# Daniel-Lin-S/decode_tonal_langauge

Measured on AMD Instinct MI355X. Metric: mel-frames/sec (train step) SynthesisModelCNN, 128ch x 400t batch256, higher is better.
Workload: dtype f32; 1 GPU; SynthesisModelCNN 128ch x 400t -> 80 mel, 4 tones x 2 syllables, L=5, global batch 256 (strong scaling: 256 windows on rank 0), dropout 0.5, NAdam, 1,376,768,720 params; per_gpu_batch=256, global_batch=256, parallelism=dp1, init=drawn on every rank

## Files before the change

decode_tonal_langauge_amd/_conv_stack.py:

```python
from __future__ import annotations

from typing import List

import torch

from . import _kernels, _lib
from ._launch import LaunchTimers, launch_nt, launch_tn, permute_reduce, r4
from ._lib import (EPI_C1WGRAD, EPI_GY, EPI_LRELU, EPI_MASK, EPI_MASKY, EPI_POOL, EPI_POOLV, LOAD_DIRECT, LOAD_UNPOOL, LOAD_V,
                   LOAD_Y, check, ptr)


class _Stage:

    def __init__(self, idx, cin, cout, k, pool, tin, tp_in):
        self.idx, self.cin, self.cout, self.k, self.pool = idx, cin, cout, k, pool
        self.tin, self.tp_in = tin, tp_in
        self.tc = tin - k + 1
        self.tout = self.tc // 2 if pool else self.tc
        self.tp_out = tp_in // 2 if pool else tp_in


class ConvStack(LaunchTimers):
    F63_CAPABLE = True

# ... 150 lines not shown
    def _v_hex_buffer(self, store, idx, rows, cin):
        nh = rows // 6
        nh_pad = (nh + 24 + 127) // 128 * 128
        V = store.get(idx)
        if V is None or V.shape[0] != nh_pad or V.shape[1] != 8 or V.shape[2] != cin:
            V = store[idx] = torch.zeros(nh_pad, 8, cin, dtype=torch.float32, device=self._dev)
        return V

    def _halo_buffer(self, key, ntm, cout):
        halo = self._vhalo.get(key)
        if halo is None or halo.shape[0] != ntm or halo.shape[2] != cout:
            halo = self._vhalo[key] = torch.zeros(ntm, 2, cout, dtype=torch.float32, device=self._dev)
        return halo

    def _pack_wino63(self, w, forward: bool):
        O, I = w.shape[0], w.shape[1]
        dst = torch.empty(8, O, I, dtype=torch.float32, device=w.device) if forward else \
            torch.empty(8, I, O, dtype=torch.float32, device=w.device)
        check(self.lib.tl_wino63_weights(ptr(w), ptr(dst) if forward else None, None if forward else ptr(dst), O, I, I, O,
                                         self._stream()), "tl_wino63_weights")
        return dst

    def f63_issue_factor(self, st) -> float:
        return (st.tp_in // 6) * 8.0 / (st.tc * 3.0)

    def _stage_forward63(self, st, w, bia) -> None:
        S = self.S
        wp = self._pack_wino63(w, True)
        V = self._v_ready[st.idx - 1]
        if st.idx == 2 and self.store_p1 and 2 not in self.P:
            self.P[2] = torch.zeros(S * st.tp_out, st.cout, dtype=torch.float32, device=self._dev)
        Pout = self.P.get(st.idx) if (st.idx != 2 or self.store_p1) else None
        kw = dict(A=ptr(V), A_rows=V.shape[0], lda=V.shape[2], loader=LOAD_V, Bw=ptr(wp), bias=ptr(bia), out=ptr(Pout),
                  M=S * st.tp_in, N=st.cout, K=st.cin, ldb=st.cin, ldo=Pout.shape[1] if Pout is not None else st.cout, J=3,
                  row_shift=0, Tp=st.tp_in, slope=self.slope, obits=ptr(self.bits[st.idx]), osign=ptr(self.sbits[st.idx]),
                  ld_obits=st.cout // 32, Tvalid=2 * st.tout)
        if st.idx == 2:
            rows_out = S * st.tp_out
            Vn = self._v_hex_buffer(self.V, 2, rows_out, st.cout)
            ntm = -(-(S * st.tp_in) // self._nt63_rows())
            halo = self._halo_buffer(2, ntm, st.cout)
            kw.update(epilogue=EPI_POOLV, vout=ptr(Vn), vhalo=ptr(halo), vout_quads=Vn.shape[0], ld_vout=Vn.shape[2])
            self._nt(tag="conv2_fwd", fn="tl_conv3_wino63v_nt", **kw)
            check(self.lib.tl_wino63_v_fixup(ptr(Vn), ptr(halo), rows_out // 6, ntm, st.tp_out, st.cout, Vn.shape[2],
                                             self._stream()), "tl_wino63_v_fixup")
            self._v_ready[2] = Vn
        else:
            if Pout is None:
                raise RuntimeError("F(6,3) stage 3 writes pooled rows: its output buffer was not allocated")
            kw.update(epilogue=EPI_POOL, out_tp=st.tp_out)
            self._nt(tag="conv3_fwd", fn="tl_conv3_wino63v_nt", **kw)

    def _stage_wgrad63(self, st, gw, gb) -> None:
        S = self.S
        f32 = dict(dtype=torch.float32, device=self._dev)
        rows_in = S * st.tp_in
        nd = st.cout
        ldg = nd
        V = self._v_ready[st.idx - 1]
        tiles = (st.cin // 64) * (nd // 64)
        sk = self._splitk(tiles, (rows_in + 35) // 36, 4096)
        slab = torch.empty(sk, 8 * st.cin, ldg, **f32)
        bias_part = torch.empty(sk, nd, **f32)
        if (st.idx == 3 and self.f63_yprod3 and self._y_ready.get(3) != self.generation):
            Gs = self.G[3]
            Y3 = self._v_hex_buffer(self.Yt, 3, rows_in, nd)
            Vd3 = self._v_hex_buffer(self.Vd, 3, rows_in, nd)
            ev = self._tick("conv3_yvd")
            check(self.lib.tl_wino63_unpool_yvd(ptr(Gs), ptr(self.bits[3]), ptr(Y3), ptr(Vd3), rows_in, Gs.shape[0], st.tp_in,
                                                st.tp_out, 2 * st.tout, nd, Gs.shape[1], st.cout // 32, nd, self._stream()),
                  "tl_wino63_unpool_yvd")
            if ev:
                ev[1].record()
            self._y_ready[3] = self.generation
            self._vd_ready[3] = self.generation
        if self._y_ready.get(st.idx) == self.generation:
            Y = self.Yt[st.idx]
            self._y_ready[st.idx] = -1
            self._tn(tag=f"conv{st.idx}_wgrad", fn="tl_conv3_wino63v_tn", A=ptr(V), B=ptr(Y), slab=ptr(slab), Krows=rows_in,
                     A_rows=V.shape[0], B_rows=Y.shape[0], Mdim=st.cin, Ndim=nd, lda=V.shape[2], ldb=Y.shape[2], ldc=ldg, J=3,
                     Tp=st.tp_in, splitk=sk, slab_stride=8 * st.cin * ldg, loader=LOAD_Y, Tvalid=2 * st.tout,
                     colsum=ptr(bias_part))
        else:
            Gs = self.G[st.idx]
            Vd = self._v_hex_buffer(self.Vd, st.idx, rows_in, nd)
            self._tn(tag=f"conv{st.idx}_wgrad", fn="tl_conv3_wino63v_tn", A=ptr(V), B=ptr(Gs), slab=ptr(slab), Krows=rows_in,
                     A_rows=V.shape[0], B_rows=Gs.shape[0], Mdim=st.cin, Ndim=nd, lda=V.shape[2], ldb=Gs.shape[1], ldc=ldg, J=3,
                     Tp=st.tp_in, splitk=sk, slab_stride=8 * st.cin * ldg, loader=LOAD_UNPOOL, bbits=ptr(self.bits[st.idx]),
                     ld_bbits=st.cout // 32, Tvalid=2 * st.tout, colsum=ptr(bias_part), vd=ptr(Vd), ld_vd=nd, g_tp=st.tp_out)
            self._vd_ready[st.idx] = self.generation
        self._wino_wgrad_tail(st, slab, bias_part, 8, "tl_wino63_wgrad_finalize", gw, gb)

    def _wino_wgrad_tail(self, st, slab, bias_part, taps, finalize, gw, gb) -> None:
        sk, rows, ldg = slab.shape
        if sk > 1:
            red = torch.empty(rows, ldg, dtype=torch.float32, device=self._dev)
            n = taps * st.cin * ldg
            self._permute(slab, red, (1, 1, 1, n), (0, 0, 0, 1), nz=sk, zs=n)
        else:
            red = slab
        check(getattr(self.lib, finalize)(ptr(red), ptr(gw), st.cout, st.cin, ldg, self._stream()), finalize)
        self._permute(bias_part, gb, (1, 1, 1, st.cout), (0, 0, 0, 1), nz=sk, zs=bias_part.shape[1])

    def _gy_stage(self, st) -> bool:
        return self.gy4 and st.idx == 4

    def _gy_applies(self) -> bool:
        if not (self.wino63 and self.f63_yprod3 and len(self.stages) >= 3):
            return False
        below, st = self.stages[1], self.stages[2]
        return (_kernels.get("conv4_dgrad") == "nt63" and st.k == 1 and st.pool and self._f63(below)
                and st.cout % 32 == 0 and st.cout >= 40 and st.cin % 32 == 0 and (below.tp_in // 2) % 3 == 0)

    def _stage_dgrad_gy(self, st, w):
        S = self.S
        below = self.stages[1]
        tpg = below.tp_in // 2
        rows = S * tpg
        f32 = dict(dtype=torch.float32, device=self._dev)
        nh = -(-rows // 6)
        nh_pad = (nh + 127) // 128 * 128
        A = self._gy_A
        if A is None or A.shape[0] != nh_pad or A.shape[2] != st.cout:
            A = self._gy_A = torch.zeros(nh_pad, 8, st.cout, **f32)
        Gs = self.G[st.idx]
        ev = self._tick(f"conv{st.idx}_dgrad")
        check(self.lib.tl_wino63_unpool_rows6(ptr(Gs), ptr(self.bits[st.idx]), ptr(A), rows, Gs.shape[0], tpg, st.tp_out,
                                              2 * st.tout, st.cout, Gs.shape[1], st.cout // 32, st.cout, 0, self._stream()),
              "tl_wino63_unpool_rows6")
        taps = torch.empty(st.cout // 8, 8, st.cin, 8, **f32)
        check(self.lib.tl_wino63_weights1(ptr(w), ptr(taps), st.cout, st.cin, st.cout, self._stream()), "tl_wino63_weights1")
        rows3 = S * below.tp_in
        Y3 = self._v_hex_buffer(self.Yt, below.idx, rows3, below.cout)
        Vd3 = self._v_hex_buffer(self.Vd, below.idx, rows3, below.cout)
        ntm = -(-rows // self._nt63_rows())
        halo = self._halo_buffer("d3", ntm, below.cout)
        self._nt(tag=None, fn="tl_conv1_wino63v_dgrad_nt", A=ptr(A), A_rows=A.shape[0], lda=A.shape[2], loader=LOAD_V,
                 Bw=ptr(taps), M=rows, N=st.cin, K=st.cout, ldb=st.cout, ldo=st.cin, J=1, row_shift=0, Tp=tpg, slope=self.slope,
                 auxbits=ptr(self.sbits[below.idx]), ld_auxbits=self.sbits[below.idx].shape[1], abits=ptr(self.bits[below.idx]),
                 ld_abits=below.cout // 32, out_tp=below.tp_out, Tvalid_in=2 * below.tout, epilogue=EPI_GY, out=None,
                 vout=ptr(Y3), vout2=ptr(Vd3), vhalo=ptr(halo), vout_quads=Y3.shape[0], ld_vout=Y3.shape[2])
        check(self.lib.tl_wino63_vd_fixup(ptr(Vd3), ptr(halo), rows // 3, ntm, below.tp_in // 6, below.cout, Vd3.shape[2],
                                          self._stream()), "tl_wino63_vd_fixup")
        if ev:
            ev[1].record()
        self._y_ready[below.idx] = self.generation
        self._vd_ready[below.idx] = self.generation
        return None

    def _stage_dgrad63(self, st, w):
        S = self.S
        rows_in = S * st.tp_in
        if self._vd_ready.get(st.idx) != self.generation:
            raise RuntimeError("F(6,3) input gradient: the stage's weight-gradient pass (which writes Vd) must run first")
        self._vd_ready[st.idx] = -1
        Vd = self.Vd[st.idx]
        wd = self._pack_wino63(w, False)
        kw = dict(A=ptr(Vd), A_rows=Vd.shape[0], lda=Vd.shape[2], loader=LOAD_V, Bw=ptr(wd), M=rows_in, N=st.cin,
                  K=st.cout, ldb=st.cout, ldo=st.cin, J=3, row_shift=-2, Tp=st.tp_in, slope=self.slope,
                  auxbits=ptr(self.sbits[st.idx - 1]), ld_auxbits=self.sbits[st.idx - 1].shape[1])
        if st.idx == 3 and self.f63_yprod:
            below = self.stages[0]
            rows2 = S * below.tp_in
            Y2 = self._v_hex_buffer(self.Yt, 2, rows2, below.cout)
            Vd2 = self._v_hex_buffer(self.Vd, 2, rows2, below.cout)
            ntm = -(-rows_in // self._nt63_rows())
            halo = self._halo_buffer("d2", ntm, below.cout)
            self._nt(tag="conv3_dgrad", fn="tl_conv3_wino63v_nt", epilogue=EPI_MASKY, out=None, vout=ptr(Y2), vout2=ptr(Vd2),
                     vhalo=ptr(halo), vout_quads=Y2.shape[0], ld_vout=Y2.shape[2], abits=ptr(self.bits[2]),
                     ld_abits=below.cout // 32, Tvalid_in=2 * below.tout, **kw)
            check(self.lib.tl_wino63_vd_fixup(ptr(Vd2), ptr(halo), rows_in // 3, ntm, below.tp_in // 6, below.cout, Vd2.shape[2],
                                              self._stream()), "tl_wino63_vd_fixup")
            self._y_ready[2] = self.generation
            self._vd_ready[2] = self.generation
            return None
        if st.idx == 3:
            self._nt(tag="conv3_dgrad", fn="tl_conv3_wino63v_nt", epilogue=EPI_MASK, out=ptr(self.G[2]), **kw)
            return None
        ntm = -(-rows_in // self._nt63_rows())
        part = torch.empty(ntm, (self.k1 + 1) * self.c1, dtype=torch.float32, device=self._dev)
        self._nt(tag="conv2_dgrad", fn="tl_conv3_wino63v_nt", epilogue=EPI_C1WGRAD, out=None, c1x=ptr(self._x),
                 c1bits=ptr(self.bits[1]), c1partial=ptr(part), c1T=self.T, c1kt=self.k1, Tvalid=self.tout1, **kw)
        return part

    def _c1_fusable(self) -> bool:
        return self.k1 <= 3 and self.T >= 2 * self.tout1 + 2

    def _v43(self, st) -> bool:
        return (self.wino43 and st.k == 3 and st.pool and st.cin % 64 == 0 and st.cout % 32 == 0 and st.tp_in % 4 == 0
                and r4(st.cout) % 16 == 0)

    def _tn_bm(self, st) -> int:
        wide = st.cin % 128 == 0
        dma8 = wide and r4(st.cout) % 64 == 0 and (st.cout // 32) % 2 == 0
        if self.tn_bm == 127:
            return 127 if wide else 64
        if self.tn_bm in (0, 128):
            return 128 if dma8 else 64
        return 64

    def _conv1_writes_v(self) -> bool:
        return (self._v43(self.stages[0]) and self.tp1 % 4 == 0 and self.c1 in (128, 256, 512, 1024)
                and (self.fuse_c1 and self._c1_fusable()))

    def _writes_v(self, st) -> bool:
        if not (self.wino_vout and st.pool and st.idx - 1 < len(self.stages)):
            return False
        nxt = self.stages[st.idx - 1]
        return self._v43(st) and self._v43(nxt) and st.tp_in % 8 == 0 and nxt.cin == st.cout

    def _pin(self, st):
        return self.P.get(st.idx - 1)

    def _v_buffer(self, idx, rows, cin, store=None):
        store = self.V if store is None else store
        nq = rows // 4
        nq_pad = (nq + 127) // 128 * 128
        V = store.get(idx)
        if V is None or V.shape[0] != nq_pad or V.shape[2] != cin:
            V = store[idx] = torch.zeros(nq_pad, 6, cin, dtype=torch.float32, device=self._dev)
        return V

    def _input_transform(self, st):
        src = self.P[st.idx - 1]
        V = self._v_buffer(st.idx - 1, src.shape[0], st.cin)
        ev = self._tick(f"conv{st.idx}_xform")
        check(self.lib.tl_wino43_input_transform(ptr(src), ptr(V), src.shape[0], st.tp_in, st.cin, src.shape[1], st.cin,
                                                 self._stream()), "tl_wino43_input_transform")
        if ev:
            ev[1].record()
        return V

    def wgrad_issue_factor(self, st) -> float:
        if self._f63(st):
            return self.f63_issue_factor(st)
        return 0.5 if self._v43(st) else 1.0

    def kernel_families(self):
        if self.wino63:
            self._fam_share = {}
            st2, st3 = self.stages[0], self.stages[1]
            f6 = "Winograd F(6,3) on pre-transformed operands, LDS-DMA"
            tn = "wino63v_tn4_kernel<true>" if st3.cin % 256 == 0 and st3.tp_in >= 12 else "wino63v_tn_kernel<true>"
            tn2 = "wino63v_tn4_kernel<true>" if st2.cin % 256 == 0 else "wino63v_tn_kernel<true>"
            fams = {f"wino63v_nt_kernel<POOLV> (conv2 forward, {f6}; writes V of its pooled output for conv3)": ["conv2_fwd"],
                    f"wino63v_nt_kernel<POOL> (conv3 forward, {f6})": ["conv3_fwd"],
                    f"wino63v_nt_kernel<C1WGRAD> (conv2 input gradient + conv1 weight gradient, {f6})": ["conv2_dgrad"],
                    }
            if self.f63_yprod3:
                gy = self.gy4
                src = "the epilogue of conv4's input gradient" if gy else "wino63_unpool_yvd_kernel"
                fams[f"wino63v_tn4y_kernel (conv3 weight gradient, {f6}: both operands by LDS-DMA, no transform in the kernel; Y3 / Vd3 "
                     f"from {src})"] = ["conv3_wgrad"]
            else:
                fams[f"{tn} (conv3 weight gradient, {f6}; also writes Vd)"] = ["conv3_wgrad"]
            if self.f63_yprod:
                fams[f"wino63v_nt_kernel<MASKY> (conv3 input gradient, {f6}; writes Y and Vd of conv2 instead of the gradient rows)"] = ["conv3_dgrad"]
                fams[f"wino63v_tn4y_kernel (conv2 weight gradient, {f6}: both operands by LDS-DMA, no transform in the kernel)"] = ["conv2_wgrad"]
            else:
                fams[f"wino63v_nt_kernel<MASK> (conv3 input gradient, {f6})"] = ["conv3_dgrad"]
                fams[f"{tn2} (conv2 weight gradient, {f6}; also writes Vd)"] = ["conv2_wgrad"]
            issued = {k: self.f63_issue_factor(st2 if "conv2" in k else st3) for k in fams}
            return fams, issued
        self._fam_share = {}
        if not all(self._v43(st) for st in self.stages[:2]):
            fams = {"nt_window_kernel<128,UNPOOL,MASK> (conv input-gradient)": ["conv2_dgrad", "conv3_dgrad", "conv4_dgrad"],
                    "nt_window_kernel<128,DIRECT,POOL> (conv forward)": ["conv2_fwd", "conv3_fwd", "conv4_fwd"],
                    "tn3_kernel<UNPOOL> (conv weight-gradient)": ["conv2_wgrad", "conv3_wgrad"]}
            return fams, {k: 1.0 for k in fams}
        form = "Winograd F(4,3) on pre-transformed operands, LDS-DMA"
        fused = self.fuse_c1 and self._c1_fusable()
        bm = self._tn_bm(self.stages[0])
        extra = {}
        if bm == 128:
            tn = f"wino43v_tn8_kernel<true> (conv2/conv3 weight gradient, {form}; also writes Vd for the input gradient)"
        else:
            ntm = (self.stages[0].cin + 63) // 64
            tn = f"wino43v_tn_kernel<false, 2> (conv2/conv3 weight gradient, C_in tiles 1..{ntm - 1} of {ntm}, {form})"
            vdn = f"wino43v_tn_kernel<true, 2> (conv2/conv3 weight gradient, C_in tile 0 of {ntm}, {form}, + writes Vd for the input gradient)"
            extra[vdn] = ["conv2_wgrad_vd", "conv3_wgrad_vd"]
            self._fam_share = {tn: (ntm - 1) / ntm, vdn: 1.0 / ntm}
        fams = {tn: ["conv2_wgrad", "conv3_wgrad"]}
        if self._writes_v(self.stages[0]):
            fams[f"wino43v_nt_kernel<POOLV> (conv2 forward, {form}; writes V of its pooled output for conv3 instead of the raw rows)"] = ["conv2_fwd"]
            fams[f"wino43v_nt_kernel<POOL> (conv3 forward, {form})"] = ["conv3_fwd"]
        else:
            fams[f"wino43v_nt_kernel<POOL> (conv2/conv3 forward, {form})"] = ["conv2_fwd", "conv3_fwd"]
        fams.update(extra)
        if fused:
            fams[f"wino43v_nt_kernel<UNPOOL,C1WGRAD> (conv2 input gradient + conv1 weight gradient, {form})"] = ["conv2_dgrad"]
            fams[f"wino43v_nt_kernel<UNPOOL,MASK> (conv3 input gradient, {form})"] = ["conv3_dgrad"]
        else:
            fams[f"wino43v_nt_kernel<UNPOOL,MASK> (conv2/conv3 input gradient, {form})"] = ["conv2_dgrad", "conv3_dgrad"]
        return fams, {k: 0.5 for k in fams}

    def _pack_wino43(self, w, forward: bool):
        O, I = w.shape[0], w.shape[1]
        dst = torch.empty(6, O, I, dtype=torch.float32, device=w.device) if forward else \
            torch.empty(6, I, O, dtype=torch.float32, device=w.device)
        check(self.lib.tl_wino43_weights(ptr(w), ptr(dst) if forward else None, None if forward else ptr(dst), O, I, I, O,
                                         self._stream()), "tl_wino43_weights")
        return dst

    def conv1_forward(self, x, w1, b1) -> None:
        lib, st_ = self.lib, self._stream()
        S, T, dev = self.S, self.T, self._dev
        self._x = x
        self._v_ready = {}
        w1 = w1.reshape(self.c1, self.k1).contiguous()
        sbits = ptr(self.sbits.get(1))
        if self.store_p1 and 1 not in self.P:
            self.P[1] = torch.zeros(S * self.tp1, self.c1, dtype=torch.float32, device=dev)
        P1 = ptr(self.P[1]) if self.store_p1 else None
        geom = (S, T, self.k1, self.c1, self.tp1, self.tout1, self.slope, st_)
        if self.wino63:
            V1 = self._v_hex_buffer(self.V, 1, S * self.tp1, self.c1)
            ev = self._tick("conv1_fwd")
            check(lib.tl_conv1_fwd_v6(ptr(x), ptr(w1), ptr(b1), P1, ptr(V1), ptr(self.bits[1]), sbits, *geom), "tl_conv1_fwd_v6")
            if ev:
                ev[1].record()
            self._v_ready[1] = V1
        elif self._conv1_writes_v():
            V1 = self._v_buffer(1, S * self.tp1, self.c1)
            check(lib.tl_conv1_fwd_v(ptr(x), ptr(w1), ptr(b1), P1, ptr(V1), ptr(self.bits[1]), sbits, *geom), "tl_conv1_fwd_v")
            self._v_ready[1] = V1
        else:
            check(lib.tl_conv1_fwd(ptr(x), ptr(w1), ptr(b1), ptr(self.P[1]), ptr(self.bits[1]), sbits, *geom), "tl_conv1_fwd")

    STAGE_NAMES = {2: "ecog_conv_block.3", 3: "ecog_conv_block.6", 4: "ecog_conv_block.9", 5: "ecog_conv_block.12"}

    def stage_forward(self, st: _Stage, w: torch.Tensor, bia: torch.Tensor) -> None:
        if self._f63(st):
            return self._stage_forward63(st, w, bia)
        S = self.S
        v43 = self._v43(st)
        wp = self._pack_wino43(w, True) if v43 else self._pack_conv(w, st.cin, False)
        src = self._pin(st)
        vout = self._writes_v(st)
        if vout and self.store_p1 and st.idx not in self.P:
            self.P[st.idx] = torch.zeros(S * st.tp_out, st.cout, dtype=torch.float32, device=self._dev)
        Pout = self.P.get(st.idx) if (not vout or self.store_p1) else None
        kw = dict(A=ptr(src), Bw=ptr(wp), bias=ptr(bia), out=ptr(Pout), M=S * st.tp_in,
                  A_rows=S * st.tp_in, N=st.cout, K=st.cin, lda=st.cin, ldb=st.cin,
                  ldo=Pout.shape[1] if Pout is not None else st.cout, J=st.k, row_shift=0, Tp=st.tp_in, slope=self.slope,
                  loader=LOAD_DIRECT)
        if st.pool:
            kw.update(epilogue=EPI_POOL, obits=ptr(self.bits[st.idx]), osign=ptr(self.sbits[st.idx]),
                      ld_obits=st.cout // 32, Tvalid=2 * st.tout)
        else:
            kw.update(epilogue=EPI_LRELU, Tvalid=st.tout)
        if not v43:
            self._nt(tag=f"conv{st.idx}_fwd", fn="tl_gemm_nt_window", **kw)
            return
        V = self._v_ready.get(st.idx - 1)
        if V is None:
            V = self._v_ready[st.idx - 1] = self._input_transform(st)
        kw.update(A=ptr(V), A_rows=V.shape[0], lda=V.shape[2], loader=LOAD_V)
        if vout:
            rows_out = S * st.tp_out
            Vn = self._v_buffer(st.idx, rows_out, st.cout)
            ntm = (S * st.tp_in + 511) // 512
            halo = self._halo_buffer(st.idx, ntm, st.cout)
            kw.update(epilogue=EPI_POOLV, vout=ptr(Vn), vhalo=ptr(halo), vout_quads=Vn.shape[0], ld_vout=Vn.shape[2])
            self._nt(tag=f"conv{st.idx}_fwd", fn="tl_conv3_wino43v_nt", **kw)
            check(self.lib.tl_wino43_v_fixup(ptr(Vn), ptr(halo), rows_out // 4, ntm, st.tp_out, st.cout, Vn.shape[2],
                                             self._stream()), "tl_wino43_v_fixup")
            self._v_ready[st.idx] = Vn
            return
        self._nt(tag=f"conv{st.idx}_fwd", fn="tl_conv3_wino43v_nt", **kw)

    def _colsum(self, Gm, rows, ncols, ld, Tp, Tvalid, dst):
        nc4 = r4(ncols)
        rpb = max(1, 256 // (nc4 // 4))
        nblk = int(min(2048, max(1, rows // (rpb * 16))))
        part = torch.empty(nblk, nc4, dtype=torch.float32, device=Gm.device)
        check(self.lib.tl_colsum(ptr(Gm), ptr(part), nblk, rows, nc4, ld, Tp, Tvalid, self._stream()), "tl_colsum")
        self._permute(part, dst, (1, 1, 1, ncols), (0, 0, 0, 1), nz=nblk, zs=nc4)

    def _reduce_c1_partials(self, part: torch.Tensor, gw: torch.Tensor, gb: torch.Tensor) -> None:
        f32 = dict(dtype=torch.float32, device=part.device)
        nblk = part.shape[0]
        zs = (self.k1 + 1) * self.c1
        if nblk >= 256 and zs % 4 == 0:
            red = torch.empty(zs, **f32)
            flat = part.view(-1)
            for c0 in range(0, zs, 1024):
                nc = min(1024, zs - c0)
                self._colsum(flat[c0:], nblk, nc, zs, 1, 1, red[c0:c0 + nc])
            self._permute(red, gw, (1, 1, self.c1, self.k1), (0, 0, 1, self.c1))
            self._permute(red, gb, (1, 1, 1, self.c1), (0, 0, 0, 1), src_off=self.k1 * self.c1)
        else:
            self._permute(part, gw, (1, 1, self.c1, self.k1), (0, 0, 1, self.c1), nz=nblk, zs=zs)
            self._permute(part, gb, (1, 1, 1, self.c1), (0, 0, 0, 1), nz=nblk, zs=zs, src_off=self.k1 * self.c1)

    def stage_wgrad(self, st: _Stage, gw: torch.Tensor, gb: torch.Tensor) -> None:
        if self._f63(st):
            return self._stage_wgrad63(st, gw, gb)
        S = self.S
        f32 = dict(dtype=torch.float32, device=self._dev)
        Xin = self._pin(st)
        Gs = self.G[st.idx]
        rows_in = S * st.tp_in
        ldg = Gs.shape[1]
        nd = r4(st.cout)
        if self._v43(st):
            tiles = ((st.cin + 63) // 64) * ((nd + 63) // 64)
            bm = self._tn_bm(st)
            sk = self._splitk(tiles, (rows_in + 31) // 32, 4096 if bm in (127, 128) else 8192)
            slab = torch.empty(sk, 6 * st.cin, ldg, **f32)
            bias_part = torch.empty(sk, nd, **f32)
# ... 87 lines not shown
```

decode_tonal_langauge_amd/_kernels.py:

```python
from __future__ import annotations

import os
from typing import Callable, Dict, Tuple, Union

_Allowed = Union[frozenset, Callable[[str], bool]]


def _int(lo: int, hi: int) -> Callable[[str], bool]:
    def ok(v: str) -> bool:
        try:
            return lo <= int(v) <= hi
        except ValueError:
            return False
    return ok


_B = frozenset({"0", "1"})
KEYS: Dict[str, Tuple[str, _Allowed, str, str]] = {
    "wino": ("TONAL_WINO", frozenset({"6", "4", "0"}), "6",
             "conv2 / conv3: 6 Winograd F(6,3) on pre-transformed operands (F(4,3) V form where the stack does not allow it), "
             "4 the F(4,3) V form, 0 direct MFMA kernels (also the fallback for every shape neither form covers)"),
    "f63_yprod": ("TONAL_F63_YPROD", _B, "1", "F(6,3): the backward operands Y / Vd of stages 2 and 3 come pre-transformed out of the "
                                              "input-gradient epilogue of the stage above (0: the weight-gradient kernels un-pool and "
                                              "transform the gradient rows themselves)"),
    "conv4_dgrad": ("TONAL_CONV4_DGRAD", frozenset({"nt63", "gemm"}), "nt63",
                    "F(6,3): the one-tap stage behind conv3 - nt63: its input gradient on the NT63 kernel, writing Y3 / Vd3 "
                    "(no gradient rows, no tl_wino63_unpool_yvd); gemm: one-tap GEMM + tl_wino63_unpool_yvd"),
    "store_p1": ("TONAL_STORE_P1", _B, "0", "keep the raw pooled rows of stages 1 / 2 beside V (tests)"),
    "conv7": ("TONAL_CONV7", frozenset({"wino63", "direct"}), "wino63", "the CNN-RNN classifier's 7-tap convolutions"),
    "whh_dh": ("TONAL_WHH_DH", _B, "1", "single process: the W_hh NAdam pass also produces the last BPTT product dh_1 = dgates_2 . W_hh "
                                        "(0: a W_hh stream of its own for it)"),
    "whh_stream": ("TONAL_WHH_STREAM", _B, "1", "label LSTM backward: dgates . W_hh as a pure stream of the weight (tl_lstm_gw; 0: the skinny "
                                                "MFMA GEMM with split-K slabs, also the form for more than 8 distinct label rows)"),
    "graph": ("TONAL_GRAPH", _B, "1", "SynthesisLite step replayed as a HIP graph"),
    "lstm_shard": ("TONAL_LSTM_SHARD", _B, "1", "data parallel: label LSTM sharded by gate rows"),
    "hilbert": ("TONAL_HILBERT", frozenset({"auto", "ols", "ols_full", "sym", "taps", "fft"}), "auto",
                "Hilbert bank: force a path (ols band-limited overlap-save, ols_full all 1024 bins per band, sym / taps the "
                "time-domain kernels with / without Hermitian symmetry, fft the DFT-domain form)"),
    "hilbert_f32": ("TONAL_HILBERT_F32", _B, "0", "float32 recordings: fp32 transforms end to end (default: fp64 math)"),
    "butter": ("TONAL_BUTTER", frozenset({"seq", "scan"}), "seq",
               "zero-phase Butterworth: seq the sequential recurrence (bit-identical to scipy's loop), scan the time-parallel "
               "block scan (2e-8 - 5e-8 from it: the size of the reference's own rounding; ~20 x faster)"),
}
_LEGACY = {v[0]: k for k, v in KEYS.items()}
_cache: Tuple[str, Dict[str, str]] = ("", {})


def _check(key: str, value: str) -> str:
    allowed = KEYS[key][1]
    ok = allowed(value) if callable(allowed) else value in allowed
    if not ok:
        what = "an integer in range" if callable(allowed) else "one of " + ", ".join(sorted(allowed))
        raise ValueError(f"TONAL_KERNELS: {key}={value!r} is not a value this switch takes ({what})")
    return value


def _parsed() -> Dict[str, str]:
    global _cache
    raw = os.environ.get("TONAL_KERNELS", "")
    if raw == _cache[0]:
        return _cache[1]
    out: Dict[str, str] = {}
    for item in raw.split(","):
        item = item.strip()
        if not item:
            continue
        key, sep, value = item.partition("=")
        key, value = key.strip(), value.strip()
        if not sep or key not in KEYS:
            raise ValueError(f"TONAL_KERNELS: unknown setting {item!r}; keys: " + ", ".join(sorted(KEYS)))
        out[key] = _check(key, value)
    _cache = (raw, out)
    return out


def get(key: str, default: str = None) -> str:
    legacy, _allowed, table_default, _doc = KEYS[key]
    spec = _parsed()
    if key in spec:
        return spec[key]
    if legacy in os.environ:
        if os.environ.get("TONAL_AB") != "1":
            raise RuntimeError(f"{legacy} is an A/B switch of the test suite and is ignored by the product: use "
                               f"TONAL_KERNELS={key}={os.environ[legacy]} (or set TONAL_AB=1 to run an A/B comparison)")
        return _check(key, os.environ[legacy])
    return table_default if default is None else default


def validate() -> None:
    _parsed()
    if os.environ.get("TONAL_AB") != "1":
        for legacy, key in _LEGACY.items():
            if legacy in os.environ:
                get(key)
```

decode_tonal_langauge_amd/_lib.py:

```python
from __future__ import annotations

import ctypes as C
import os
from typing import Optional

_HERE = os.path.dirname(os.path.abspath(__file__))
LIB_PATH = os.environ.get("TONAL_HIP_LIB", os.path.join(_HERE, "libtonal_hip.so"))

LOAD_DIRECT, LOAD_UNPOOL, LOAD_V = 0, 1, 2
EPI_STORE, EPI_LRELU, EPI_POOL, EPI_MASK, EPI_C1WGRAD, EPI_POOLV, EPI_MASKY, EPI_GY = 0, 1, 2, 3, 4, 5, 6, 7
LOAD_Y = 3


class NtParams(C.Structure):
    _fields_ = [
        ("A", C.c_void_p), ("abits", C.c_void_p), ("Bw", C.c_void_p), ("bias", C.c_void_p), ("aux", C.c_void_p),
        ("out", C.c_void_p), ("obits", C.c_void_p),
        ("M", C.c_int64), ("A_rows", C.c_int64),
        ("N", C.c_int), ("K", C.c_int),
        ("lda", C.c_int), ("ldb", C.c_int), ("ldo", C.c_int), ("ldaux", C.c_int), ("ld_abits", C.c_int),
        ("ld_obits", C.c_int),
        ("J", C.c_int), ("row_shift", C.c_int),
        ("Tp", C.c_int), ("Tvalid", C.c_int), ("Tvalid_in", C.c_int),
        ("slope", C.c_float),
        ("loader", C.c_int), ("epilogue", C.c_int),
        ("splitk", C.c_int), ("slab_stride", C.c_int64),
        ("bm", C.c_int),
        ("osign", C.c_void_p), ("auxbits", C.c_void_p), ("ld_auxbits", C.c_int),
        ("c1x", C.c_void_p), ("c1bits", C.c_void_p), ("c1partial", C.c_void_p), ("c1T", C.c_int), ("c1kt", C.c_int),
        ("vout", C.c_void_p), ("vhalo", C.c_void_p), ("vout_quads", C.c_int64), ("ld_vout", C.c_int),
        ("out_tp", C.c_int), ("vout2", C.c_void_p),
    ]


class TnParams(C.Structure):
    _fields_ = [
        ("A", C.c_void_p), ("B", C.c_void_p), ("bbits", C.c_void_p), ("slab", C.c_void_p),
        ("Krows", C.c_int64), ("A_rows", C.c_int64), ("B_rows", C.c_int64),
        ("Mdim", C.c_int), ("Ndim", C.c_int),
        ("lda", C.c_int), ("ldb", C.c_int), ("ldc", C.c_int), ("ld_bbits", C.c_int),
        ("J", C.c_int), ("Tp", C.c_int), ("Tvalid", C.c_int), ("loader", C.c_int),
        ("splitk", C.c_int), ("slab_stride", C.c_int64),
        ("colsum", C.c_void_p),
        ("vd", C.c_void_p), ("ld_vd", C.c_int), ("part", C.c_int), ("bm", C.c_int), ("g_tp", C.c_int),
    ]


_P = C.c_void_p
_I = C.c_int
_L = C.c_int64
_F = C.c_float
_D = C.c_double

SIGNATURES = {
    "tl_last_error": (C.c_char_p, []),
    "tl_version": (_I, []),
    "tl_device_count": (_I, []),
    "tl_gemm_nt_window": (_I, [C.POINTER(NtParams), _P]),
    "tl_gemm_tn_window": (_I, [C.POINTER(TnParams), _P]),
    "tl_wino43_weights": (_I, [_P, _P, _P, _I, _I, _I, _I, _P]),
    "tl_wino63_xform2": (_I, [_P, _P, _P, _L, _I, _I, _I, _I, _I, _P]),
    "tl_wino63_weights7": (_I, [_P, _P, _I, _I, _I, _P]),
    "tl_conv7_wino63v_nt": (_I, [C.POINTER(NtParams), _P]),
    "tl_wino63_unpool_rows6": (_I, [_P, _P, _P, _L, _L, _I, _I, _I, _I, _I, _I, _I, _I, _P]),
    "tl_wino63_weights1": (_I, [_P, _P, _I, _I, _I, _P]),
    "tl_conv1_wino63v_dgrad_nt": (_I, [C.POINTER(NtParams), _P]),
    "tl_comm_unique_id": (_I, [_P]),
    "tl_comm_init": (_I, [C.POINTER(C.c_void_p), _I, _I, _P]),
    "tl_comm_destroy": (_I, [_P]),
    "tl_allreduce": (_I, [_P, _P, _P, _L, _I, _P]),
    "tl_reduce_scatter": (_I, [_P, _P, _P, _L, _P]),
    "tl_all_gather": (_I, [_P, _P, _P, _L, _P]),
    "tl_wino43_wgrad_finalize": (_I, [_P, _P, _I, _I, _I, _P]),
    "tl_wino43_input_transform": (_I, [_P, _P, _L, _I, _I, _I, _I, _P]),
    "tl_conv3_wino43v_nt": (_I, [C.POINTER(NtParams), _P]),
    "tl_wino43_v_fixup": (_I, [_P, _P, _L, _L, _I, _I, _I, _P]),
    "tl_wino43_unpool_transform": (_I, [_P, _P, _P, _L, _L, _I, _I, _I, _I, _I, _I, _P]),
    "tl_conv3_wino43v_tn": (_I, [C.POINTER(TnParams), _P]),
    "tl_wino63_weights": (_I, [_P, _P, _P, _I, _I, _I, _I, _P]),
    "tl_conv3_wino63v_nt": (_I, [C.POINTER(NtParams), _P]),
    "tl_wino63_nt_tile_rows": (_I, []),
    "tl_wino63_v_fixup": (_I, [_P, _P, _L, _L, _I, _I, _I, _P]),
    "tl_conv3_wino63v_tn": (_I, [C.POINTER(TnParams), _P]),
    "tl_wino63_wgrad_finalize": (_I, [_P, _P, _I, _I, _I, _P]),
    "tl_wino63_vd_fixup": (_I, [_P, _P, _L, _L, _I, _I, _I, _P]),
    "tl_wino63_unpool_yvd": (_I, [_P, _P, _P, _P, _L, _L, _I, _I, _I, _I, _I, _I, _I, _P]),
    "tl_conv1_fwd_v6": (_I, [_P, _P, _P, _P, _P, _P, _P, _L, _I, _I, _I, _I, _I, _F, _P]),
    "tl_sizeof_nt_params": (_I, []),
    "tl_sizeof_tn_params": (_I, []),
    "tl_conv1_fwd": (_I, [_P, _P, _P, _P, _P, _P, _L, _I, _I, _I, _I, _I, _F, _P]),
    "tl_conv1_fwd_v": (_I, [_P, _P, _P, _P, _P, _P, _P, _L, _I, _I, _I, _I, _I, _F, _P]),
    "tl_dropout_scale": (_I, [_P, _L, _F, C.c_uint64, _P]),
    "tl_dropout_scale_at": (_I, [_P, _L, _F, C.c_uint64, _L, _P]),
    "tl_conv1_wgrad": (_I, [_P, _P, _P, _P, _I, _L, _I, _I, _I, _I, _I, _P]),
    "tl_permute_reduce": (_I, [_P, _P, C.POINTER(_L), C.POINTER(_L), C.POINTER(_L), _I, _L, _P, _P]),
    "tl_colsum": (_I, [_P, _P, _I, _L, _I, _I, _I, _I, _P]),
    "tl_lstm_cell_fwd": (_I, [_P, _P, _P, _P, _P, _P, _P, _P, _P, _I, _I, _I, _I, _P]),
    "tl_lstm_gw": (_I, [_P, _P, _P, _I, _L, _I, _L, _L, _I, _P]),
    "tl_lstm_infer_seq_fused": (_I, [_P, _L, _P, _P, _P, _P, _I, _I, _I, C.POINTER(C.c_int), _P]),
    "tl_lstm_cell_bwd": (_I, [_P, _P, _P, _P, _P, _P, _P, _P, _P, _I, _I, _I, _P]),
    "tl_lstm_ih_grad": (_I, [_P, _P, _P, _P, _P, _I, _I, _I, _I, _P]),
    "tl_concat_pack": (_I, [_P, _P, _P, _P, _I, _I, _I, _I, _I, _I, _I, _I, _I, _F, C.c_uint64, _L, _P]),
    "tl_concat_unpack_bwd": (_I, [_P, _P, _P, _P, _P, _P, _I, _I, _I, _I, _I, _I, _I, _I, _I, _I, _F, _F,
                                  C.c_uint64, _L, _P]),
    "tl_l1_mcd": (_I, [_P, _P, _P, _P, _I, _I, _I, _I, _F, _P]),
    "tl_nadam": (_I, [_P, _P, _P, _P, _L, _F, _F, _F, _F, _F, _F, _F, _F, _P]),
    "tl_nadam_multi": (_I, [_P, _I, _L, _F, _F, _F, _F, _F, _F, _F, _F, _P]),
    "tl_nadam_multi_chunk": (_I, []),
    "tl_sum_slabs2": (_I, [_P, _P, _L, _P, _P, _L, _I, _P]),
    "tl_set_step_scalars": (_I, [_P, _P, _F, _F, _F, C.c_uint64, _P]),
    "tl_stage_step": (_I, [_P, _P, _F, _F, _F, C.c_uint64, _P, _P, _P, _I, _P]),
    "tl_nadam_multi_dev": (_I, [_P, _I, _L, _P, _F, _F, _F, _F, _F, _P]),
    "tl_nadam_lowrank": (_I, [_P, _P, _P, _P, _P, _I, _I, _I, _I, _I, _F, _F, _F, _F, _F, _F, _F, _F, _P]),
    "tl_nadam_lowrank_dh": (_I, [_P, _P, _P, _P, _P, _I, _I, _I, _I, _I, _F, _F, _F, _F, _F, _F, _F, _F, _P, _I, _I, _P]),
    "tl_tone_dynamics": (_I, [_P, _P, _P, _P, _P, _I, _I, _I, _P]),
    "tl_splitk_bias_lrelu": (_I, [_P, _P, _P, _I, _L, _I, _F, _P]),
    "tl_labels_from_scores": (_I, [_P, _P, _P, _P, _P, _P, _P, _P, _I, _I, _I, _I, _I, _I, _P]),
    "tl_ce_loss": (_I, [_P, _P, _P, _P, _P, _P, _P, _P, _P, _I, _I, _I, _I, _F, _P]),
    "tl_ce_scores_loss": (_I, [_P, _P, _P, _P, _P, _P, _P, _P, _P, _I, _I, _I, _I, _F, _P]),
    "tl_head_bwd": (_I, [_P, _P, _P, _P, _P, _P, _I, _I, _I, _I, _I, _F, _P]),
    "tl_lstm_train_seq": (_I, [_P, _L, _L, _P, _P, _P, _P, _I, _I, _I, _P]),
    "tl_lstm_bptt_seq": (_I, [_P, _P, _P, _P, _P, _P, _P, _L, _I, _I, _I, _P]),
    "tl_pool3_fwd": (_I, [_P, _P, _I, _I, _I, _I, _I, _I, _I, _L, _L, _F, C.c_uint64, _P]),
    "tl_pool3_bwd": (_I, [_P, _P, _P, _I, _I, _I, _I, _I, _I, _I, _I, _L, _L, _F, C.c_uint64, _F, _P]),
    "tl_pool3_fwd_shard": (_I, [_P, _P, _I, _I, _I, _I, _I, _I, _I, _L, _L, _F, C.c_uint64, _I, _I, _P]),
    "tl_pool3_bwd_shard": (_I, [_P, _P, _P, _I, _I, _I, _I, _I, _I, _I, _I, _L, _L, _F, C.c_uint64, _F, _I, _I, _P]),
    "tl_conv1_dgrad": (_I, [_P, _P, _P, _P, _L, _I, _I, _I, _I, _I, _I, _L, _L, _L, _P]),
    "tl_lite_conv_fwd": (_I, [_P, _P, _P, _P, _P, _I, _I, _I, _I, _I, _I, _P]),
    "tl_lite_bn_finalize": (_I, [_P, _P, _P, _P, _P, _I, _I, _L, _I, _F, _F, _I, _P, _P]),
    "tl_lite_bn_act_pool_fwd": (_I, [_P, _P, _P, _P, _P, _P, _I, _I, _I, _F, _P]),
    "tl_lite_bn_act_pool_bwd": (_I, [_P, _P, _P, _P, _P, _P, _P, _P, _P, _P, _I, _I, _I, _F, _I, _P]),
    "tl_lite_conv_bwd": (_I, [_P, _P, _P, _P, _P, _P, _I, _I, _I, _I, _I, _I, _P]),
    "tl_lite_lstm_fwd": (_I, [_P, _P, _P, _P, _P, _P, _P, _P, _I, _I, _I, _I, _P]),
    "tl_lite_lstm_bwd": (_I, [_P, _P, _P, _P, _P, _I, _I, _I, _I, _P]),
    "tl_lite_cat": (_I, [_P, _P, _P, _I, _I, _I, _I, _I, _F, C.c_uint64, _P]),
    "tl_lite_uncat": (_I, [_P, _P, _P, _I, _I, _I, _I, _F, C.c_uint64, _P]),
    "tl_lite_cat_dev": (_I, [_P, _P, _P, _I, _I, _I, _I, _I, _F, _P, _P]),
    "tl_lite_uncat_dev": (_I, [_P, _P, _P, _I, _I, _I, _I, _F, _P, _P]),
    "tl_row_zscore": (_I, [_P, _I, _P, _P, _I, _L, _L, _L, _I, _P]),
    "tl_car": (_I, [_P, _I, _P, _P, _I, _L, _I, _P]),
    "tl_rolling_zscore": (_I, [_P, _I, _P, _I, _L, _I, _I, _P]),
    "tl_fft_resample": (_I, [_P, _I, _P, _I, _L, _L, _P, _P, _P, _I, _P, _P, _P, _I, _P, _P]),
    "tl_gauss_envelope": (_I, [_P, _I, _P, _P, _I, _L, _I, _I, _I, _I, _P]),
    "tl_gauss_envelope_sym": (_I, [_P, _I, _P, _P, _I, _L, _I, _I, _I, _P]),
    "tl_linear_rows": (_I, [_P, _P, _P, _P, _I, _I, _I, _L, _I, _P]),
    "tl_hilbert_ols": (_I, [_P, _I, _P, _P, _P, _I, _L, _I, _I, _I, _I, _P]),
    "tl_hilbert_ols_bl": (_I, [_P, _I, _P, _P, _P, _P, _I, _L, _I, _I, _I, _I, _P]),
    "tl_hilbert_fft": (_I, [_P, _I, _P, _I, _L, _P, _I, _P, _P, _P, _I, _I, _P, _P]),
    "tl_filtfilt_f64": (_I, [_P, _I, _P, _P, _P, _P, _P, _I, _L, _I, _P]),
    "tl_filtfilt_scan_f64": (_I, [_P, _I, _P, _P, _P, _P, _I, _P, _P, _P, _I, _L, _I, _I, _P]),
    "tl_sosfilt_f64": (_I, [_P, _I, _P, _P, _I, _L, _I, _P]),
    "tl_fir_bank": (_I, [_P, _I, _P, _P, _I, _I, _L, _I, _I, _P]),
    "tl_fir_bank_ols": (_I, [_P, _I, _P, _P, _P, _I, _I, _L, _I, _I, _P]),
    "tl_group_moments": (_I, [_P, _I, _L, _L, _P, _I, _P, _I, _P, _P, _P]),
    "tl_anova_finalize": (_I, [_P, _P, C.POINTER(C.c_int32), _I, _I, _L, _P, _P, _P]),
    "tl_max_run_below": (_I, [_P, _I, _L, C.c_double, _P, _P, _P]),
    "tl_mel_power": (_I, [_P, _I, _L, _P, _P, _P, _P, _I, _P, _P, _I, _L, _I, _I, _I, _I, _I, _I, _L, _P]),
    "tl_mel_finish": (_I, [_P, _P, _P, _I, _I, _L, _I, _P]),
    "tl_mel_invert": (_I, [_P, _P, _P, _I, _P, _P, _P, _P, _I, _I, _I, _L, _I, _D, _I, _P]),
    "tl_gl_synth": (_I, [_P, _P, _I, _P, _P, _P, _I, _I, _L, _P]),
    "tl_gl_analyse": (_I, [_P, _P, _P, _P, _P, _P, _I, _I, _I, _I, _L, _L, _D, _I, _P]),
    "tl_gl_overlap_add": (_I, [_P, _P, _P, _I, _I, _I, _I, _L, _L, _P]),
}

_lib: Optional[C.CDLL] = None


def load() -> C.CDLL:
    global _lib
    if _lib is not None:
        return _lib
    import torch
    if not os.path.exists(LIB_PATH):
        raise RuntimeError(
            f"{LIB_PATH} not found: build it with `python -c 'import __graft_entry__ as g; g.build()'` "
            "(or `make -C decode_tonal_langauge_amd/csrc`). This package has no CPU fallback.")
    lib = C.CDLL(LIB_PATH)
    for name, (res, args) in SIGNATURES.items():
        fn = getattr(lib, name)
        fn.restype = res
        fn.argtypes = args
    if lib.tl_sizeof_nt_params() != C.sizeof(NtParams) or lib.tl_sizeof_tn_params() != C.sizeof(TnParams):
        raise RuntimeError("libtonal_hip.so parameter structs do not match the ctypes binding; rebuild the library")
    _lib = lib
    return lib


def check(rc: int, what: str) -> None:
    if rc != 0:
        msg = load().tl_last_error()
        raise RuntimeError(f"{what} failed (code {rc}): {msg.decode() if msg else '?'}")


def ptr(t) -> Optional[int]:
    return None if t is None else t.data_ptr()


def stream_ptr() -> int:
    import torch
    return torch.cuda.current_stream().cuda_stream


def require_gpu(t, what: str) -> None:
    if not t.is_cuda:
        raise RuntimeError(
            f"{what}: tensor is on '{t.device}'. The MI355X path runs HIP kernels only and has no CPU "
            "fallback; move the model and its inputs to a 'cuda' device.")
```

decode_tonal_langauge_amd/csrc/tonal_wino63.hip:

```cpp
#include "tonal_common.h"
#include "tonal_wino43_epi.h"
#include "tonal_wino43v_epi.h"
#include "tonal_wino63_epi.h"
#include "tonal_wino63_kloop.h"
#include <type_traits>

namespace tl {

typedef __attribute__((address_space(3))) void lds_void6_t;
__device__ __forceinline__ void dma16h(__amdgpu_buffer_rsrc_t rs, char* lds_dst, unsigned voff, unsigned soff) {
  __builtin_amdgcn_raw_ptr_buffer_load_lds(rs, (lds_void6_t*)lds_dst, 16, voff, soff, 0, 0);
}

typedef int v6_i32x4 __attribute__((ext_vector_type(4)));
__device__ __forceinline__ v6_i32x4 v6_rsrc_words(const void* base, long long bytes) {
  const unsigned long long a = (unsigned long long)base;
  const long long n = bytes < 0 ? 0 : (bytes < 0x7fffffffLL ? bytes : 0x7fffffffLL);
  return v6_i32x4{(int)(unsigned)a, (int)(unsigned)((a >> 32) & 0xffffu), (int)n, 0x00020000};
}

__device__ __forceinline__ long long v6_at(long long hex, int i, int c, int kc8) {
  return ((((hex >> 1) * kc8 + (c >> 3)) * 8 + i) * 2 + (hex & 1)) * 8 + (c & 7);
}

__global__ void wino63_weights_kernel(const float* __restrict__ w, float* __restrict__ fwd, float* __restrict__ dgr, int O,
                                      int I, int ld_f, int ld_d) {
  const long long n_f = (long long)O * ld_f, n_d = (long long)I * ld_d;
  const long long idx = (long long)blockIdx.x * blockDim.x + threadIdx.x;
  auto emit = [](float* dst, int R, int r, int k, float g0, float g1, float g2) {
    float* d0 = dst + (((long long)(k >> 3) * 8) * R + r) * 8 + (k & 7);
    const long long n = (long long)R * 8;
    const float s = g0 + g2;
    d0[0] = -g0;
    d0[n] = (-2.f / 9.f) * (s + g1);
    d0[2 * n] = (-2.f / 9.f) * (s - g1);
    const float a = fmaf(4.f, g2, g0), b = 2.f * g1;
    d0[3 * n] = (1.f / 90.f) * (a + b);
    d0[4 * n] = (1.f / 90.f) * (a - b);
    const float c = fmaf(4.f, g0, g2), d = 2.f * g1;
    d0[5 * n] = (8.f / 45.f) * (c + d);
    d0[6 * n] = (8.f / 45.f) * (c - d);
    d0[7 * n] = g2;
  };
  if (fwd != nullptr && idx < n_f) {
    const int o = (int)(idx / ld_f), i = (int)(idx % ld_f);
    float g0 = 0.f, g1 = 0.f, g2 = 0.f;
    if (i < I) {
      const float* s = w + ((long long)o * I + i) * 3;
      g0 = s[0], g1 = s[1], g2 = s[2];
    }
    emit(fwd, O, o, i, g0, g1, g2);
  }
  if (dgr != nullptr && idx < n_d) {
    const int i = (int)(idx / ld_d), o = (int)(idx % ld_d);
    float g0 = 0.f, g1 = 0.f, g2 = 0.f;
    if (o < O) {
      const float* s = w + ((long long)o * I + i) * 3;
      g0 = s[2], g1 = s[1], g2 = s[0];
    }
    emit(dgr, I, i, o, g0, g1, g2);
  }
}

__global__ void wino63_wgrad_finalize_kernel(const float* __restrict__ red, float* __restrict__ gw, int O, int I, int ld) {
  const long long idx = (long long)blockIdx.x * blockDim.x + threadIdx.x;
  if (idx >= (long long)O * I) return;
  const int i = (int)(idx / O), o = (int)(idx % O);
  const long long plane = (long long)I * ld;
  const float* s = red + (long long)i * ld + o;
  float m[8];
#pragma unroll
  for (int t = 0; t < 8; ++t) m[t] = s[t * plane];
  const float a12 = m[1] + m[2], s12 = m[1] - m[2], a34 = m[3] + m[4], s34 = m[3] - m[4], a56 = m[5] + m[6], s56 = m[5] - m[6];
  float* d = gw + ((long long)o * I + i) * 3;
  d[0] = -m[0] - (2.f / 9.f) * a12 + (1.f / 90.f) * a34 + (32.f / 45.f) * a56;
  d[1] = -(2.f / 9.f) * s12 + (1.f / 45.f) * s34 + (16.f / 45.f) * s56;
  d[2] = -(2.f / 9.f) * a12 + (2.f / 45.f) * a34 + (8.f / 45.f) * a56 + m[7];
}

__global__ void wino63_weights7_kernel(const float* __restrict__ w, float* __restrict__ fwd, int O, int I, int taps) {
  const long long idx = (long long)blockIdx.x * blockDim.x + threadIdx.x;
  if (idx >= 3LL * O * I) return;
  const int k = (int)(idx % (3LL * I)), o = (int)(idx / (3LL * I));
  const int seg = k / I, i = k - seg * I;
  const float* s = w + ((long long)o * I + i) * taps + 3 * seg;
  const float g0 = 3 * seg < taps ? s[0] : 0.f, g1 = 3 * seg + 1 < taps ? s[1] : 0.f, g2 = 3 * seg + 2 < taps ? s[2] : 0.f;
  float* d0 = fwd + (((long long)(k >> 3) * 8) * O + o) * 8 + (k & 7);
  const long long n = (long long)O * 8;
  const float sm = g0 + g2;
  d0[0] = -g0;
  d0[n] = (-2.f / 9.f) * (sm + g1);
  d0[2 * n] = (-2.f / 9.f) * (sm - g1);
  const float a = fmaf(4.f, g2, g0), b = 2.f * g1;
  d0[3 * n] = (1.f / 90.f) * (a + b);
  d0[4 * n] = (1.f / 90.f) * (a - b);
  const float c = fmaf(4.f, g0, g2), d = 2.f * g1;
  d0[5 * n] = (8.f / 45.f) * (c + d);
  d0[6 * n] = (8.f / 45.f) * (c - d);
  d0[7 * n] = g2;
}

__global__ __launch_bounds__(256, 4) void wino63_xform2_kernel(const float* __restrict__ P, float* __restrict__ V0, float* __restrict__ V1,
                                                             long long nhex, int hps, int Tp, int Tvalid, int C, int ldp, int ldv) {
  const int tpp = C >> 1;
  const long long idx = (long long)blockIdx.x * blockDim.x + threadIdx.x;
  const long long pair = idx / tpp;
  const int tl_ = (int)(idx - pair * tpp);
  const int half = tl_ & 1, hpar = (tl_ >> 1) & 1, kc = tl_ >> 2;
  const int c = 8 * kc + 4 * half;
  const long long hg = 2 * pair + hpar;
  if (hg >= nhex) return;
  const long long seq = hg / hps;
  const int hs = (int)(hg - seq * hps);
  const float* src = P + (seq * Tp + 6LL * hs) * (long long)ldp + c;
  f32x4 d[11];
#pragma unroll
  for (int j = 0; j < 11; ++j) {
    d[j] = f32x4{0.f, 0.f, 0.f, 0.f};
    if (6 * hs + j < Tvalid) d[j] = *reinterpret_cast<const f32x4*>(src + (long long)j * ldp);
  }
  f32x4 o0[8], o1[8];
#pragma unroll
  for (int k = 0; k < 4; ++k) {
    float a[8], b[8], va[8], vb[8];
#pragma unroll
    for (int j = 0; j < 8; ++j) {
      a[j] = d[j][k];
      b[j] = d[j + 3][k];
    }
    wino63_bt(a, va);
    wino63_bt(b, vb);
#pragma unroll
    for (int j = 0; j < 8; ++j) {
      o0[j][k] = va[j];
      o1[j][k] = vb[j];
    }
  }
  const long long at = v6_at(hg, 0, c, ldv >> 3);
#pragma unroll
  for (int j = 0; j < 8; ++j) *reinterpret_cast<f32x4*>(V0 + at + 16 * j) = o0[j];
#pragma unroll
  for (int j = 0; j < 8; ++j) *reinterpret_cast<f32x4*>(V1 + at + 16 * j) = o1[j];
}

__global__ __launch_bounds__(256, 4) void wino63_v_fixup_kernel(float* __restrict__ V, const float* __restrict__ halo, long long hexes,
                                                              long long tiles, int Tq, int C, int ldv) {
  const int c4n = C >> 2;
  const long long idx = (long long)blockIdx.x * blockDim.x + threadIdx.x;
  if (idx >= tiles * c4n) return;
  const long long t = idx / c4n;
  const int c = (int)(idx - t * c4n) * 4;
  const long long q = t * 64 + 63;
  if (q >= hexes) return;
  float* v = V + v6_at(q, 0, c, ldv >> 3);
  f32x4 d[8];
#pragma unroll
  for (int j = 0; j < 6; ++j) d[j] = *reinterpret_cast<const f32x4*>(v + 16 * j);
  const int tq = (int)((6 * q) % Tq);
  if (tq + 6 < Tq && t + 1 < tiles) {
    d[6] = *reinterpret_cast<const f32x4*>(halo + ((t + 1) * 2) * (long long)C + c);
    d[7] = *reinterpret_cast<const f32x4*>(halo + ((t + 1) * 2 + 1) * (long long)C + c);
  } else {
    d[6] = d[7] = f32x4{0.f, 0.f, 0.f, 0.f};
  }
  f32x4 o[8];
#pragma unroll
  for (int k = 0; k < 4; ++k) {
    float dd[8], vv[8];
#pragma unroll
    for (int j = 0; j < 8; ++j) dd[j] = d[j][k];
    wino63_bt(dd, vv);
#pragma unroll
    for (int j = 0; j < 8; ++j) o[j][k] = vv[j];
  }
#pragma unroll
  for (int j = 0; j < 8; ++j) *reinterpret_cast<f32x4*>(v + 16 * j) = o[j];
}

constexpr int V6_BH = 128, V6_BN = 64, V6_BK = 8;
constexpr int V6_ROWB = V6_BK * 4;
constexpr int V6_A_BYTES = 8 * V6_BH * V6_ROWB;
constexpr int V6_B_BYTES = 8 * V6_BN * V6_ROWB;
constexpr int V6_STAGE = V6_A_BYTES + V6_B_BYTES;
constexpr int V6_ROWS = 6 * V6_BH;

template <int EPI>
__global__ __launch_bounds__(512, 2) void wino63v_nt_kernel(const tl_nt_params p) {
  __shared__ __attribute__((aligned(1024))) char lds[3 * V6_STAGE + ((EPI == W_EPI_POOLV || EPI == W_EPI_MASKY || EPI == W_EPI_GY) ? 4096 : EPI == W_EPI_C1W ? 16384 : 0)];
  const int tid = threadIdx.x;
  const int lane = tid & 63;
  const int wave = __builtin_amdgcn_readfirstlane(tid >> 6);
  const int wm = wave >> 1, wn = wave & 1;
  const int lr = lane & 31, lh = lane >> 5;

  const int ntn = (p.N + V6_BN - 1) / V6_BN;
  const long long ntm = (p.M + V6_ROWS - 1) / V6_ROWS;
  const long long nwg = ntm * ntn;
  constexpr bool SEG3 = EPI == W_EPI_LRELU;
  constexpr bool SIX = EPI == W_EPI_GY;
  const int kseg = p.K / V6_BK;
  const int nsteps = SEG3 ? 3 * kseg : kseg;
  f32x16 acc[8];
  f32x4 faL[4], fbL[4], faH[4], fbH[4];

  const int prow = lane >> 1;
  const int src_chunk = (lane & 1) ^ ((lane >> 4) & 1);
  const v6_i32x4 rsB = v6_rsrc_words(p.Bw, (SIX && wave >= 6) ? 0 : 8LL * p.N * p.ldb * 4);
  const unsigned lds0 = (unsigned)(unsigned long long)(lds_void6_t*)lds;
  const unsigned dst_a0 = lds0 + (unsigned)(wave * V6_BH * V6_ROWB);
  const unsigned dst_b0 = lds0 + (unsigned)(V6_A_BYTES + wave * V6_BN * V6_ROWB);
  const int hex_of_row = (prow & 3) | ((prow >> 3) << 2) | (((prow >> 2) & 1) << 4);
  const int kc8 = p.lda >> 3;
  unsigned avoff[4], bv_lane[2];
#pragma unroll
  for (int t = 0; t < 4; ++t) avoff[t] = (unsigned)(v6_at(t * 32 + hex_of_row, wave, src_chunk * 4, kc8) * 4);
  unsigned avoff1[4];
#pragma unroll
  for (int t = 0; t < 4; ++t) avoff1[t] = SEG3 ? (unsigned)(v6_at(t * 32 + hex_of_row + 1, wave, src_chunk * 4, kc8) * 4) : avoff[t];
#pragma unroll
  for (int t = 0; t < 2; ++t) bv_lane[t] = (unsigned)((((long long)wave * p.N + t * 32 + prow) * 8 + src_chunk * 4) * 4);
  const unsigned b_step = (unsigned)p.N * 256u;

  struct tile_t {
    long long tm, R0;
    int n0;
    v6_i32x4 rsA, rsA1;
    unsigned bvoff[2];
  };
  const long long a_tile_bytes = (long long)V6_BH * 8 * p.lda * 4, a_total_bytes = p.A_rows * 8LL * p.lda * 4;
  auto place = [&](tile_t& t, long long tm, int tn) {
    t.tm = tm;
    t.R0 = tm * V6_ROWS;
    t.n0 = tn * V6_BN;
    const long long ab = tm * a_tile_bytes;
    t.rsA = v6_rsrc_words(reinterpret_cast<const char*>(p.A) + ab, (SIX && wave >= 6) ? 0 : a_total_bytes - ab);
    t.rsA1 = SEG3 ? v6_rsrc_words(reinterpret_cast<const char*>(p.aux) + ab, a_total_bytes - ab) : t.rsA;
    if (t.n0 + V6_BN <= p.N) {
      const unsigned nb4 = (unsigned)t.n0 * 32u;
#pragma unroll
      for (int k = 0; k < 2; ++k) t.bvoff[k] = bv_lane[k] + nb4;
    } else {
#pragma unroll
      for (int k = 0; k < 2; ++k) {
        int n = t.n0 + k * 32 + prow;
        if (n > p.N - 1) n = p.N - 1;
        t.bvoff[k] = (unsigned)((((long long)wave * p.N + n) * 8 + src_chunk * 4) * 4);
      }
    }
  };
  tile_t cur;
  {
    long long bid = blockIdx.x;
    const long long q = nwg / 8, r = nwg % 8, x = bid % 8, i = bid / 8;
    bid = (x < r ? x * (q + 1) : r * (q + 1) + (x - r) * q) + i;
    place(cur, bid / ntn, (int)(bid % ntn));
  }
  const int walk = (int)(gridDim.x >> 3), walk_q = walk / ntn, walk_r = walk - walk_q * ntn;
  auto advance = [&](const tile_t& c) -> tile_t {
    tile_t t = c;
    int tn = c.n0 / V6_BN + walk_r;
    long long tm = c.tm + walk_q;
    if (tn >= ntn) {
      tn -= ntn;
      ++tm;
    }
    place(t, tm, tn);
    return t;
  };
  auto next3 = [](int s) { return s == 2 ? 0 : s + 1; };

  const int cphys = (lh ^ ((lr >> 3) & 1)) << 4;
  const unsigned a_row = lds0 + (unsigned)((wm * 32 + lr) * V6_ROWB + cphys);
  const unsigned b_row = lds0 + (unsigned)((wn * 32 + lr) * V6_ROWB + cphys);
  int stg = 0;

  struct dma_src {
    v6_i32x4 ra;
    unsigned va[4], vb[2], sa, sb;
  };
  auto src_of = [&](const tile_t& t, int step) {
    dma_src d;
    int ks = step;
    if constexpr (SEG3) {
      const int seg = (step >= kseg ? 1 : 0) + (step >= 2 * kseg ? 1 : 0);
      ks = step - seg * kseg;
#pragma unroll
      for (int k = 0; k < 4; ++k) {
        d.ra[k] = seg == 1 ? t.rsA1[k] : t.rsA[k];
        d.va[k] = seg == 2 ? avoff1[k] : avoff[k];
      }
    } else {
      d.ra = t.rsA;
#pragma unroll
      for (int k = 0; k < 4; ++k) d.va[k] = avoff[k];
    }
    d.vb[0] = t.bvoff[0];
    d.vb[1] = t.bvoff[1];
#pragma unroll
    for (int k = 0; k < 4; ++k) d.ra[k] = __builtin_amdgcn_readfirstlane(d.ra[k]);
    d.sa = (unsigned)__builtin_amdgcn_readfirstlane(ks * 512);
    d.sb = (unsigned)__builtin_amdgcn_readfirstlane((int)((unsigned)step * b_step));
    return d;
  };
#define V6K_INPUTS(src, dst, wimm)                                                                                             \
  [a] "v"(a_row + (unsigned)stg * (unsigned)V6_STAGE), [b] "v"(b_row + (unsigned)stg * (unsigned)V6_STAGE),                    \
      [va0] "v"((src).va[0]), [va1] "v"((src).va[1]), [va2] "v"((src).va[2]), [va3] "v"((src).va[3]), [vb0] "v"((src).vb[0]), \
      [vb1] "v"((src).vb[1]), [ra] "s"((src).ra), [rb] "s"(rsB), [m0a] "s"(dst_a0 + (unsigned)(dst) * (unsigned)V6_STAGE),     \
      [m0b] "s"(dst_b0 + (unsigned)(dst) * (unsigned)V6_STAGE), [sa] "s"((src).sa), [sb] "s"((src).sb), [w] "n"(wimm)
#pragma clang diagnostic ignored "-Winline-asm"
#define V6K_STMT_R(REGS, TEXT, tl_, step, dst, wimm)                                                                     \
  do {                                                                                                                   \
    const dma_src src_ = src_of(tl_, step);                                                                              \
    asm volatile(TEXT : REGS(acc, faL, fbL, faH, fbH) : V6K_INPUTS(src_, dst, wimm) : "memory", "scc", "m0");                  \
  } while (0)
#define V6K_STMT(TEXT, tl_, step, dst, wimm) V6K_STMT_R(V6K_REGS, TEXT, tl_, step, dst, wimm)
  auto issue = [&](const tile_t& tl_, int step, int dst) {
    const dma_src src_ = src_of(tl_, step);
    asm volatile(V6K_ISSUE : : V6K_INPUTS(src_, dst, 0) : "memory", "scc", "m0");
  };
  constexpr bool early = EPI == W_EPI_POOLV || EPI == W_EPI_C1W;
  constexpr int NST = v6_stores<EPI>();
  constexpr int first_n = NST + 6 > 63 ? 63 : NST + 6;
  constexpr int first_wait = (first_n & 15) | (7 << 4) | (0 << 8) | ((first_n >> 4) << 14);

  issue(cur, 0, 0);
  issue(cur, 1, 1);
  __builtin_amdgcn_s_waitcnt(0x0f70);
  for (long long vb = blockIdx.x; vb < nwg; vb += gridDim.x) {
    __builtin_amdgcn_s_barrier();
    asm volatile("" ::: "memory");
    auto prefetch = [&] {
      if constexpr (EPI == W_EPI_POOL || EPI == W_EPI_POOLV || EPI == W_EPI_LRELU) return v5_prefetch_pool(p, cur.n0, wn, lr);
      else if constexpr (EPI == W_EPI_MASK) return v6_prefetch_mask(p, cur.R0, cur.n0, wm, wn, lr, lh);
      else if constexpr (EPI == W_EPI_MASKY) return v6_prefetch_masky(p, cur.R0, cur.n0, wm, wn, lr, lh);
      else if constexpr (EPI == W_EPI_GY) return v6_prefetch_masky<true>(p, cur.R0, cur.n0, wm, wn, lr, lh);
      else return v6_prefetch_c1w(p, cur.R0, cur.n0, wm, wn, lr, lh);
    };
    decltype(prefetch()) pre;
#define V6K_RUN(KIND, RSFX, tl_, step, dst, wimm)                                                                              \
  do {                                                                                                                         \
    if constexpr (SIX) V6K_STMT_R(V6K6_REGS##RSFX, V6K6_##KIND##_L, tl_, step, dst, wimm);                                     \
    else if constexpr (early) V6K_STMT_R(V6K_REGS##RSFX, V6K_##KIND##_E, tl_, step, dst, wimm);                                \
    else V6K_STMT_R(V6K_REGS##RSFX, V6K_##KIND##_L, tl_, step, dst, wimm);                                                     \
  } while (0)
    if constexpr (SIX) V6K_STMT_R(V6K6_REGS_FIRST, V6K6_FIRST, cur, 2, stg == 0 ? 2 : stg - 1, first_wait);
    else V6K_STMT_R(V6K_REGS_FIRST, V6K_FIRST, cur, 2, stg == 0 ? 2 : stg - 1, first_wait);
    stg = next3(stg);
    V6K_RUN(STEP1, _STEP1, cur, 3, stg == 0 ? 2 : stg - 1, 0);
    stg = next3(stg);
    {
      int s = 2;
      do {
        V6K_RUN(NORM, , cur, s + 2, stg == 0 ? 2 : stg - 1, 0);
        stg = next3(stg);
      } while (++s + 2 < nsteps);
    }
    V6K_RUN(PRELAST, , cur, 0, 0, 0);
    stg = next3(stg);
    pre = prefetch();
    V6K_RUN(LAST, , cur, 0, 0, 0);
    stg = next3(stg);
#undef V6K_RUN

    const tile_t done = cur;
    const long long nb = vb + gridDim.x;
    const int last_stage = stg == 0 ? 2 : stg - 1;
    __builtin_amdgcn_s_waitcnt(0x0f70);
    if (nb < nwg) {
      cur = advance(cur);
      issue(cur, 0, stg);
      issue(cur, 1, next3(stg));
    }
    __builtin_amdgcn_sched_barrier(0);
    float* scratch = reinterpret_cast<float*>(lds + last_stage * V6_STAGE);
    (void)scratch;
    const bool full = done.R0 + V6_ROWS <= p.M && done.n0 + V6_BN <= p.N;
    if constexpr (EPI == W_EPI_POOL) {
      if (full) v6_epilogue_pool<false, true>(p, acc, pre, nullptr, done.R0, done.n0, wm, wn, lr, lh, done.tm);
      else v6_epilogue_pool<false, false>(p, acc, pre, nullptr, done.R0, done.n0, wm, wn, lr, lh, done.tm);
    } else if constexpr (EPI == W_EPI_POOLV) {
      float* xch = reinterpret_cast<float*>(lds + 3 * V6_STAGE);
      if (full) v6_epilogue_pool<true, true>(p, acc, pre, xch, done.R0, done.n0, wm, wn, lr, lh, done.tm);
      else v6_epilogue_pool<true, false>(p, acc, pre, xch, done.R0, done.n0, wm, wn, lr, lh, done.tm);
    } else if constexpr (EPI == W_EPI_LRELU) {
      if (full) v6_epilogue_lrelu<true>(p, acc, pre, done.R0, done.n0, wm, wn, lr, lh);
      else v6_epilogue_lrelu<false>(p, acc, pre, done.R0, done.n0, wm, wn, lr, lh);
    } else if constexpr (EPI == W_EPI_MASK) {
      if (full) v6_epilogue_mask<true>(p, acc, pre, done.R0, done.n0, wm, wn, lr, lh);
      else v6_epilogue_mask<false>(p, acc, pre, done.R0, done.n0, wm, wn, lr, lh);
    } else if constexpr (EPI == W_EPI_MASKY) {
      float* xch = reinterpret_cast<float*>(lds + 3 * V6_STAGE);
      if (full) v6_epilogue_masky<true>(p, acc, pre, xch, done.R0, done.n0, wm, wn, lr, lh, done.tm);
      else v6_epilogue_masky<false>(p, acc, pre, xch, done.R0, done.n0, wm, wn, lr, lh, done.tm);
    } else if constexpr (EPI == W_EPI_GY) {
      float* xch = reinterpret_cast<float*>(lds + 3 * V6_STAGE);
      if (full) v6_epilogue_masky<true, true>(p, acc, pre, xch, done.R0, done.n0, wm, wn, lr, lh, done.tm);
      else v6_epilogue_masky<false, true>(p, acc, pre, xch, done.R0, done.n0, wm, wn, lr, lh, done.tm);
    } else {
      v6_epilogue_c1w(p, acc, pre, reinterpret_cast<float*>(lds + 3 * V6_STAGE) + wave * 512, scratch, done.R0, done.n0, wm, wn,
                      lr, lh, done.tm);
    }
    {
      constexpr int n = NST + 6 > 63 ? 63 : NST + 6;
      __builtin_amdgcn_s_waitcnt((n & 15) | (7 << 4) | (15 << 8) | ((n >> 4) << 14));
    }
  }
}



constexpr int T6_BN = 64, T6_H = 6;
constexpr int T6_PLANE = T6_H * 64;
constexpr int T6_TILE = 8 * T6_PLANE;
constexpr int T6_NA = 4, T6_NG = 6;
constexpr int T6_GW = T6_H * 4 * 64;
constexpr int T6_GT = T6_GW + 64;

template <bool WVD>
__global__ __launch_bounds__(512, 1) void wino63v_tn_kernel(const tl_tn_params p, int mtn) {
  constexpr int NA = T6_NA, NG = T6_NG, GW = T6_GW, GT = T6_GT;
  __shared__ __attribute__((aligned(1024))) float lds[(NA * 2 + 2) * T6_TILE + NG * GT];
  float* As = lds;
  float* Bs = lds + NA * 2 * T6_TILE;
  float* Gs = Bs + 2 * T6_TILE;
  const int tid = threadIdx.x, lane = tid & 63;
  const int wave = __builtin_amdgcn_readfirstlane(tid >> 6);
  const int wm = wave >> 1, wn = wave & 1, lr = lane & 31, lh = lane >> 5;
  const int ntn = p.Ndim / T6_BN;
  const long long tiles = (long long)mtn * ntn;
  const long long nwg = tiles * p.splitk;
  long long bid = (long long)blockIdx.y * gridDim.x + blockIdx.x;
  {
    const long long q = nwg / 8, r = nwg % 8, x = bid % 8, i = bid / 8;
    bid = (x < r ? x * (q + 1) : r * (q + 1) + (x - r) * q) + i;
  }
  const int z = __builtin_amdgcn_readfirstlane((int)(bid / tiles));
  const int tt = __builtin_amdgcn_readfirstlane((int)(bid % tiles));
  const int mi = __builtin_amdgcn_readfirstlane(tt / ntn);
  const int m0 = mi * 128, n0 = __builtin_amdgcn_readfirstlane((tt % ntn) * T6_BN);

  const long long hexes_all = p.Krows / 6;
  const long long ksteps_all = (hexes_all + T6_H - 1) / T6_H;
  const long long per = __builtin_amdgcn_readfirstlane((int)((ksteps_all + p.splitk - 1) / p.splitk));
  const long long ks_begin = z * per;
  long long ks_end = ks_begin + per;
  if (ks_end > ksteps_all) ks_end = ksteps_all;
  const int nsteps = ks_end > ks_begin ? (int)(ks_end - ks_begin) : 0;

  f32x16 acc[8];
#pragma unroll
  for (int i = 0; i < 8; ++i)
#pragma unroll
    for (int e = 0; e < 16; ++e) acc[i][e] = 0.f;

  const long long v_h0 = ks_begin * T6_H;
  const int kc8 = p.lda >> 3;
  const __amdgpu_buffer_rsrc_t rsV = __builtin_amdgcn_make_buffer_rsrc(
      (void*)(p.A + v_h0 * 8 * (long long)p.lda), 0, clip31((p.A_rows - v_h0) * 8 * (long long)p.lda * 4), 0x00020000);
  unsigned vvoff[3], vdst[3];
#pragma unroll
  for (int t = 0; t < 3; ++t) {
    const int half = (wave * 3 + t) / 12, pc = (wave * 3 + t) % 12;
    const int rho = 4 * pc + (lane >> 4), i = rho / 6, hx = rho % 6;
    const int chunk = (lane & 15) ^ ((hx & 1) << 3);
    vvoff[t] = (unsigned)(v6_at(hx, i, m0 + half * 64 + chunk * 4, kc8) * 4);
    vdst[t] = (unsigned)((half * T6_TILE + pc * 256) * 4);
  }
  const unsigned v_step = (unsigned)(T6_H * 8 * p.lda * 4);
  auto issue_v = [&](int step) {
    char* base = reinterpret_cast<char*>(As) + (step & (NA - 1)) * (2 * T6_TILE * 4);
    const unsigned soff = (unsigned)step * v_step;
#pragma unroll
    for (int t = 0; t < 3; ++t) dma16h(rsV, base + vdst[t], vvoff[t] + soff, 0u);
  };
  const int Tq = p.Tp >> 1, hps = p.Tp / 6;
  const int g_tp = p.g_tp > 0 ? p.g_tp : Tq;
  const bool wpiece = wave >= 6;
  const int myhex = wpiece ? (lane >> 3) : wave;
  const long long seq0 = v_h0 / hps;
  const int hs0 = (int)(v_h0 - seq0 * hps);
  const long long g_r0 = seq0 * g_tp + 3LL * hs0;
  int g_hs = hs0 + myhex, g_off = 3 * myhex;
  while (g_hs >= hps) {
    g_hs -= hps;
    g_off += g_tp - Tq;
  }
  const int ldw4 = p.ld_bbits * 4;
  const __amdgpu_buffer_rsrc_t rsG = __builtin_amdgcn_make_buffer_rsrc(
      wpiece ? (void*)(p.bbits + g_r0 * (long long)p.ld_bbits + (n0 >> 5)) : (void*)(p.B + g_r0 * (long long)p.ldb + n0), 0,
      wpiece ? clip31((p.B_rows - g_r0) * (long long)ldw4 - (long long)(n0 >> 5) * 4)
             : clip31((p.B_rows - g_r0) * (long long)p.ldb * 4 - (long long)n0 * 4),
      0x00020000);
  const unsigned g_lane = wpiece ? (unsigned)(((lane >> 1) & 3) * ldw4 + (lane & 1) * 4)
                                 : (unsigned)(((lane >> 4) * (long long)p.ldb + (lane & 15) * 4) * 4);
  const unsigned g_row4 = wpiece ? (unsigned)ldw4 : (unsigned)(p.ldb * 4);
  const unsigned gdst = wpiece ? (unsigned)(GW * 4) : (unsigned)(wave * 256 * 4);
  const bool g_live = !wpiece || lane < 48;
  auto issue_g = [&](int slot) {
    const unsigned voff = g_live ? (unsigned)g_off * g_row4 + g_lane : 0xfffffff0u;
    if (wpiece) __builtin_amdgcn_raw_ptr_buffer_load_lds(rsG, (lds_void6_t*)(reinterpret_cast<char*>(Gs) + slot * (GT * 4) + gdst), 4, voff, 0u, 0, 0);
    else dma16h(rsG, reinterpret_cast<char*>(Gs) + slot * (GT * 4) + gdst, voff, 0u);
    g_hs += T6_H;
    g_off += 3 * T6_H;
    while (g_hs >= hps) {
      g_hs -= hps;
      g_off += g_tp - Tq;
    }
  };
  auto next6 = [](int v) { return v == NG - 1 ? 0 : v + 1; };

  constexpr bool write_vd = WVD;
  const bool ywave = wave < T6_H;
  const int sw = lane ^ ((wave & 1) << 5);
  int tq = __builtin_amdgcn_readfirstlane((int)((6 * (v_h0 + (ywave ? wave : 0))) % p.Tp));
  const int dstep = __builtin_amdgcn_readfirstlane((6 * T6_H) % p.Tp);
  float bsum = 0.f;
  const int kcd = write_vd ? (p.ld_vd >> 3) : 1;
  const unsigned vd_pstride = (unsigned)(16 * p.ld_vd * 4);
  const long long vd_hexes = ((hexes_all + 1) >> 1) << 1;
  const __amdgpu_buffer_rsrc_t rsVd = __builtin_amdgcn_make_buffer_rsrc(
      write_vd ? (void*)(p.vd + v_h0 * 8 * (long long)p.ld_vd) : (void*)p.slab, 0,
      write_vd ? clip31((vd_hexes - v_h0) * 8 * (long long)p.ld_vd * 4) : 0, 0x00020000);
  const unsigned vdA_lane = (unsigned)(v6_at(0, lane & 3, n0 + (lane & ~3), kcd) * 4);
  const unsigned vdB_lane = vdA_lane + 4u * 64u;
  const int nhex = (int)hexes_all, h_first = (int)v_h0;
  const int h_end = h_first + nsteps * T6_H;
  const int hs_lim = nhex < h_end ? nhex : h_end;
  struct y_in {
    float g[3];
    unsigned long long mo[3], me[3];
    int tq;
  };
  struct y_out {
    float d[6];
  };
  auto uni = [](unsigned long long v) -> unsigned long long {
    return (unsigned long long)(unsigned)__builtin_amdgcn_readfirstlane((int)(unsigned)v) |
           ((unsigned long long)(unsigned)__builtin_amdgcn_readfirstlane((int)(unsigned)(v >> 32)) << 32);
  };
  const int wy = ywave ? wave : 0;
  auto fetch_y = [&](int sd, int slot, y_in& y) {
    const int h = h_first + sd * T6_H + wy;
    const int live = ywave & (h < hs_lim);
    const float* gs = Gs + slot * GT;
    const unsigned long long* ws = reinterpret_cast<const unsigned long long*>(gs + GW) + wy * 4;
#pragma unroll
    for (int r = 0; r < 3; ++r) {
      y.g[r] = gs[wy * 256 + r * 64 + lane];
      const unsigned long long w = uni(ws[r]);
      const int v = live & (tq + 2 * r < p.Tvalid);
      y.mo[r] = v ? w : 0ull;
      y.me[r] = v ? ~w : 0ull;
    }
// ... 792 lines not shown
                                                                   long long g_rows, int Tp, int g_tp, int Tvalid, int C, int ldg,
                                                                   int ld_bits, int lda, int pad) {
  const int tpp = C >> 1;
  const long long idx = (long long)blockIdx.x * blockDim.x + threadIdx.x;
  const long long pair = idx / tpp;
  const int tl_ = (int)(idx - pair * tpp);
  const int half = tl_ & 1, hpar = (tl_ >> 1) & 1, kc = tl_ >> 2;
  const int c = 8 * kc + 4 * half;
  const long long hg = 2 * pair + hpar;
  if (hg >= nhex) return;
  float* dst = A + v6_at(hg, 0, c, lda >> 3);
  const f32x4 zero = {0.f, 0.f, 0.f, 0.f};
#pragma unroll
  for (int i = 0; i < 6; ++i) {
    const long long R = 6 * hg + i;
    f32x4 v = zero;
    if (R < rows) {
      const long long seq = R / Tp;
      const int t = (int)(R - seq * Tp);
      const long long row = seq * g_tp + (t >> 1);
      if (t < Tvalid && row < g_rows) {
        const f32x4 g = *reinterpret_cast<const f32x4*>(G + row * (long long)ldg + c);
        const uint32_t w = bits[row * (long long)ld_bits + (c >> 5)] >> (c & 31);
#pragma unroll
        for (int k = 0; k < 4; ++k) v[k] = (int)((w >> k) & 1u) == (t & 1) ? g[k] : 0.f;
      }
    }
    *reinterpret_cast<f32x4*>(dst + 16 * i) = v;
  }
  if (pad) {
    *reinterpret_cast<f32x4*>(dst + 16 * 6) = zero;
    *reinterpret_cast<f32x4*>(dst + 16 * 7) = zero;
  }
}

__global__ void wino63_weights1_kernel(const float* __restrict__ w, float* __restrict__ out, int O, int I, int ldb) {
  const long long n_all = (long long)ldb * 8 * I;
  const long long idx = (long long)blockIdx.x * blockDim.x + threadIdx.x;
  if (idx >= n_all) return;
  const int k8 = (int)(idx & 7);
  const long long q = idx >> 3;
  const int n = (int)(q % I);
  const long long q2 = q / I;
  const int t = (int)(q2 & 7);
  const int o = (int)(q2 >> 3) * 8 + k8;
  out[idx] = (t < 6 && o < O) ? w[(long long)o * I + n] : 0.f;
}

constexpr int C1_MAXKT = 8;
template <int KT>
__global__ __launch_bounds__(256) void conv1_fwd_vh_kernel(const float* __restrict__ x, const float* __restrict__ w,
                                                           const float* __restrict__ b, float* __restrict__ P,
                                                           float* __restrict__ V, uint32_t* __restrict__ bits,
                                                           uint32_t* __restrict__ sign, long long S, int T, int C1,
                                                           int Tp, int Tout, float slope) {
  constexpr int kt = KT;
  extern __shared__ __attribute__((aligned(16))) float xs[];
  const long long seq = blockIdx.x;
  for (int i = threadIdx.x; i < T; i += blockDim.x) xs[i] = x[seq * T + i];
  __syncthreads();
  const int tpp = C1 >> 1;
  const int ppp = 256 / tpp;
  const int tl_ = threadIdx.x % tpp, psub = threadIdx.x / tpp;
  const int half = tl_ & 1, hpar = (tl_ >> 1) & 1, kc = tl_ >> 2;
  const int o = 8 * kc + 4 * half;
  float wv[4][KT], bv[4];
#pragma unroll
  for (int c = 0; c < 4; ++c) {
    bv[c] = b[o + c];
#pragma unroll
    for (int j = 0; j < KT; ++j) wv[c][j] = w[(o + c) * kt + j];
  }
  const int sh = 4 * (2 * (kc & 3) + half);
  const int Th = Tp / 6;
  auto row = [&](int pr, bool live, f32x4& out, uint32_t& wb, uint32_t& ws) {
    out = f32x4{0.f, 0.f, 0.f, 0.f};
    uint32_t nib = 0, nsg = 0;
    if (live && pr < Tout) {
#pragma unroll
      for (int c = 0; c < 4; ++c) {
        float z0 = 0.f, z1 = 0.f;
#pragma unroll
        for (int jj = 0; jj < KT; ++jj) {
          z0 = fmaf(wv[c][jj], xs[2 * pr + jj], z0);
          z1 = fmaf(wv[c][jj], xs[2 * pr + 1 + jj], z1);
        }
        const float y0 = lrelu(z0 + bv[c], slope), y1 = lrelu(z1 + bv[c], slope);
        const bool sel = y1 > y0;
        const float v = sel ? y1 : y0;
        out[c] = v;
        nib |= (sel ? 1u : 0u) << c;
        nsg |= (v > 0.f ? 1u : 0u) << c;
      }
    }
    auto or8 = [](uint32_t v) {
      v |= (uint32_t)__builtin_amdgcn_update_dpp(0, (int)v, 0xB1, 0xf, 0xf, false);
      v |= (uint32_t)__builtin_amdgcn_update_dpp(0, (int)v, 0x124, 0xf, 0xf, false);
      v |= (uint32_t)__builtin_amdgcn_update_dpp(0, (int)v, 0x128, 0xf, 0xf, false);
      return v;
    };
    wb = or8(nib << sh);
    ws = or8(nsg << sh);
  };
  const long long h0 = seq * Th;
  const int q0 = (int)((hpar - h0) & 1) + 2 * psub;
  const int trips = (Th + 2 * ppp - 1) / (2 * ppp) + 1;
  const bool word_writer = sh == 0;
  for (int i = 0; i < trips; ++i) {
    const int q = q0 + 2 * ppp * i;
    const bool live = q < Th;
    f32x4 d[8];
    uint32_t wb[8], ws[8];
#pragma unroll
    for (int j = 0; j < 8; ++j) row(6 * q + j, live && 6 * q + j < Tp, d[j], wb[j], ws[j]);
    if (live) {
      const long long row0 = seq * Tp + 6 * q;
#pragma unroll
      for (int j = 0; j < 6; ++j) {
        if (P != nullptr) *reinterpret_cast<f32x4*>(P + (row0 + j) * C1 + o) = d[j];
        if (word_writer) {
          bits[(row0 + j) * (C1 >> 5) + (o >> 5)] = wb[j];
          if (sign != nullptr) sign[(row0 + j) * (C1 >> 5) + (o >> 5)] = ws[j];
        }
      }
      f32x4 ov[8];
#pragma unroll
      for (int k = 0; k < 4; ++k) {
        float dd[8], vv[8];
#pragma unroll
        for (int j = 0; j < 8; ++j) dd[j] = d[j][k];
        wino63_bt(dd, vv);
#pragma unroll
        for (int j = 0; j < 8; ++j) ov[j][k] = vv[j];
      }
      float* dst = V + v6_at(h0 + q, 0, o, C1 >> 3);
#pragma unroll
      for (int j = 0; j < 8; ++j) *reinterpret_cast<f32x4*>(dst + 16 * j) = ov[j];
    }
  }
}

}

extern "C" int tl_wino63_weights(const float* w, float* fwd, float* dgr, int O, int I, int ld_f, int ld_d, void* stream) {
  using namespace tl;
  TL_REQUIRE(w != nullptr && (fwd != nullptr || dgr != nullptr), "wino63_weights: null pointer");
  TL_REQUIRE(O > 0 && I > 0, "wino63_weights: bad sizes");
  TL_REQUIRE((fwd == nullptr || (ld_f >= I && ld_f % 8 == 0)) && (dgr == nullptr || (ld_d >= O && ld_d % 8 == 0)),
             "wino63_weights: leading dimensions must cover the reduction length and be multiples of 8");
  const long long nf = (long long)O * ld_f, nd = (long long)I * ld_d;
  const long long n = nf > nd ? nf : nd;
  TL_REQUIRE((n + 255) / 256 < (1LL << 31), "wino63_weights: too large");
  hipLaunchKernelGGL(wino63_weights_kernel, dim3((unsigned)((n + 255) / 256)), dim3(256), 0, (hipStream_t)stream, w, fwd, dgr, O,
                     I, ld_f, ld_d);
  return check_launch("wino63_weights");
}

extern "C" int tl_wino63_wgrad_finalize(const float* red, float* gw, int O, int I, int ld, void* stream) {
  using namespace tl;
  TL_REQUIRE(red && gw && O > 0 && I > 0 && ld >= O, "wino63_wgrad_finalize: bad arguments");
  const long long n = (long long)O * I;
  hipLaunchKernelGGL(wino63_wgrad_finalize_kernel, dim3((unsigned)((n + 255) / 256)), dim3(256), 0, (hipStream_t)stream, red, gw,
                     O, I, ld);
  return check_launch("wino63_wgrad_finalize");
}

extern "C" int tl_wino63_v_fixup(float* V, const float* vhalo, int64_t hexes, int64_t tiles, int Tq, int C, int ldv, void* stream) {
  using namespace tl;
  TL_REQUIRE(V && vhalo, "wino63_v_fixup: null pointer");
  TL_REQUIRE(hexes > 0 && tiles > 0 && Tq > 0 && Tq % 6 == 0, "wino63_v_fixup: hexes, tiles > 0 and Tq %% 6 == 0 needed");
  TL_REQUIRE(C > 0 && C % 4 == 0 && ldv >= C && ldv % 8 == 0, "wino63_v_fixup: C %% 4 and ldv %% 8 needed");
  const long long n = (long long)tiles * (C / 4);
  TL_REQUIRE((n + 255) / 256 < (1LL << 31), "wino63_v_fixup: grid too large");
  hipLaunchKernelGGL(wino63_v_fixup_kernel, dim3((unsigned)((n + 255) / 256)), dim3(256), 0, (hipStream_t)stream, V, vhalo,
                     (long long)hexes, (long long)tiles, Tq, C, ldv);
  return check_launch("wino63_v_fixup");
}

extern "C" int tl_wino63_vd_fixup(float* Vd, const float* vhalo, int64_t hexes, int64_t tiles, int hexes_per_seq, int C, int ldv,
                                  void* stream) {
  using namespace tl;
  TL_REQUIRE(Vd && vhalo, "wino63_vd_fixup: null pointer");
  TL_REQUIRE(hexes > 0 && tiles > 0 && hexes_per_seq > 0, "wino63_vd_fixup: hexes, tiles, hexes per sequence > 0 needed");
  TL_REQUIRE(C > 0 && C % 4 == 0 && ldv >= C && ldv % 8 == 0, "wino63_vd_fixup: C %% 4 and ldv %% 8 needed");
  const long long n = (long long)tiles * (C / 4);
  TL_REQUIRE((n + 255) / 256 < (1LL << 31), "wino63_vd_fixup: grid too large");
  hipLaunchKernelGGL(wino63_vd_fixup_kernel, dim3((unsigned)((n + 255) / 256)), dim3(256), 0, (hipStream_t)stream, Vd, vhalo,
                     (long long)hexes, (long long)tiles, hexes_per_seq, C, ldv);
  return check_launch("wino63_vd_fixup");
}

extern "C" int tl_wino63_unpool_yvd(const float* G, const uint32_t* bits, float* Y, float* Vd, int64_t conv_rows, int64_t g_rows,
                                    int Tp, int g_tp, int Tvalid, int C, int ldg, int ld_bits, int ldv, void* stream) {
  using namespace tl;
  TL_REQUIRE(G && bits && Y && Vd, "wino63_unpool_yvd: null pointer");
  TL_REQUIRE(Tp > 0 && Tp % 6 == 0 && conv_rows > 0 && conv_rows % Tp == 0 && Tvalid % 2 == 0 && Tvalid <= Tp,
             "wino63_unpool_yvd: Tp %% 6 == 0, whole sequences, an even Tvalid <= Tp needed");
  TL_REQUIRE(g_tp > 0 && 2 * g_tp >= Tvalid && g_rows >= (conv_rows / Tp) * (long long)g_tp, "wino63_unpool_yvd: G holds fewer rows than sequences x g_tp");
  TL_REQUIRE(C > 0 && C % 8 == 0 && ldg >= C && ldg % 4 == 0 && ldv >= C && ldv % 8 == 0 && ld_bits * 32 >= C,
             "wino63_unpool_yvd: C %% 8, ldg %% 4, ldv %% 8 needed, bits row must cover C");
  const long long nhex = conv_rows / 6;
  const long long n = ((nhex + 1) / 2) * (C / 2);
  TL_REQUIRE((n + 255) / 256 < (1LL << 31), "wino63_unpool_yvd: grid too large");
  hipLaunchKernelGGL(wino63_unpool_yvd_kernel, dim3((unsigned)((n + 255) / 256)), dim3(256), 0, (hipStream_t)stream, G, bits, Y, Vd,
                     nhex, (long long)g_rows, Tp / 6, g_tp, Tvalid, C, ldg, ld_bits, ldv);
  return check_launch("wino63_unpool_yvd");
}

extern "C" int tl_wino63_weights7(const float* w, float* fwd, int O, int I, int taps, void* stream) {
  using namespace tl;
  TL_REQUIRE(w && fwd && O > 0 && I > 0 && I % 8 == 0 && taps >= 7 && taps <= 9, "wino63_weights7: I %% 8 == 0 and 7..9 taps needed");
  const long long n = 3LL * O * I;
  TL_REQUIRE((n + 255) / 256 < (1LL << 31), "wino63_weights7: grid too large");
  hipLaunchKernelGGL(wino63_weights7_kernel, dim3((unsigned)((n + 255) / 256)), dim3(256), 0, (hipStream_t)stream, w, fwd, O, I, taps);
  return check_launch("wino63_weights7");
}

extern "C" int tl_wino63_xform2(const float* P, float* V0, float* V1, int64_t rows, int Tp, int Tvalid, int C, int ldp, int ldv,
                                void* stream) {
  using namespace tl;
  TL_REQUIRE(P && V0 && V1, "wino63_xform2: null pointer");
  TL_REQUIRE(Tp > 0 && Tp % 6 == 0 && rows > 0 && rows % Tp == 0 && Tvalid >= 0 && Tvalid <= Tp, "wino63_xform2: Tp %% 6 == 0, whole sequences, Tvalid <= Tp needed");
  TL_REQUIRE(C > 0 && C % 8 == 0 && ldp >= C && ldp % 4 == 0 && ldv >= C && ldv % 8 == 0, "wino63_xform2: C %% 8, ldp %% 4, ldv %% 8 needed");
  const long long nhex = rows / 6;
  const long long n = ((nhex + 1) / 2) * (C / 2);
  TL_REQUIRE((n + 255) / 256 < (1LL << 31), "wino63_xform2: grid too large");
  hipLaunchKernelGGL(wino63_xform2_kernel, dim3((unsigned)((n + 255) / 256)), dim3(256), 0, (hipStream_t)stream, P, V0, V1, nhex,
                     Tp / 6, Tp, Tvalid, C, ldp, ldv);
  return check_launch("wino63_xform2");
}

extern "C" int tl_conv7_wino63v_nt(const tl_nt_params* pp, void* stream) {
  using namespace tl;
  TL_REQUIRE(pp != nullptr, "conv7_wino63: null params");
  const tl_nt_params& p = *pp;
  TL_REQUIRE(p.A && p.aux && p.Bw && p.out, "conv7_wino63: null V0 (A) / V1 (aux) / Bw / out");
  TL_REQUIRE(p.loader == W_LOAD_V && p.epilogue == W_EPI_LRELU && p.row_shift == 0 && p.splitk <= 1,
             "conv7_wino63: loader 2 (pre-transformed operands), LRELU epilogue, row_shift 0, no split-K");
  TL_REQUIRE(p.J >= 7 && p.J <= 9, "conv7_wino63: 7..9 taps (three segments)");
  TL_REQUIRE(p.M > 0 && p.M % 6 == 0 && p.N > 0 && p.N % 32 == 0 && p.K >= 16 && p.K % 8 == 0, "conv7_wino63: M %% 6, N %% 32, K %% 8, K >= 16 needed");
  TL_REQUIRE(p.lda >= p.K && p.lda % 8 == 0 && p.ldb >= 3 * p.K && p.ldb % 8 == 0 && p.ldo >= p.N, "conv7_wino63: bad leading dimensions");
  TL_REQUIRE(p.A_rows % 2 == 0 && p.Tp > 0 && p.Tp % 6 == 0 && p.M % p.Tp == 0, "conv7_wino63: V holds hex pairs; Tp %% 6, whole sequences");
  TL_REQUIRE(8LL * p.N * p.ldb * 4 < (1LL << 31), "conv7_wino63: tap set larger than a buffer resource");
  TL_REQUIRE(128LL * 8 * p.lda * 4 + 4LL * p.K < (1LL << 31) && p.M + V6_ROWS < (1LL << 31), "conv7_wino63: tile span / M too large");
  TL_REQUIRE(p.slope >= 0.f && p.slope <= 1.f, "conv7_wino63: LeakyReLU slope must lie in [0, 1]");
  const long long ntm = (p.M + V6_ROWS - 1) / V6_ROWS;
  const long long nwg = ntm * ((p.N + V6_BN - 1) / V6_BN);
  TL_REQUIRE(nwg < (1LL << 31), "conv7_wino63: grid too large");
  TL_REQUIRE(p.A_rows >= ntm * V6_BH, "conv7_wino63: V0 / V1 must hold whole 128-hex tiles (pad them with zero hexes)");
  const long long ngrid = nwg < 256 ? nwg : 256;
  hipLaunchKernelGGL((wino63v_nt_kernel<W_EPI_LRELU>), dim3((unsigned)ngrid), dim3(512), 0, (hipStream_t)stream, p);
  return check_launch("conv7_wino63");
}

extern "C" int tl_wino63_nt_tile_rows(void) { return tl::V6_ROWS; }

extern "C" int tl_conv3_wino63v_nt(const tl_nt_params* pp, void* stream) {
  using namespace tl;
  TL_REQUIRE(pp != nullptr, "wino63v_nt: null params");
  const tl_nt_params& p = *pp;
  TL_REQUIRE(p.A && p.Bw && (p.out || p.epilogue == W_EPI_C1W || p.epilogue == W_EPI_POOLV || p.epilogue == W_EPI_MASKY), "wino63v_nt: null V/Bw/out");
  TL_REQUIRE(p.loader == W_LOAD_V, "wino63v_nt: loader 2 (pre-transformed operand) only");
  TL_REQUIRE(p.J == 3 && p.splitk <= 1, "wino63v_nt: 3 taps, no split-K");
  TL_REQUIRE(p.M > 0 && p.M % 6 == 0 && p.N > 0 && p.K >= 40 && p.K % 8 == 0, "wino63v_nt: M %% 6, K %% 8, K >= 40 needed");
  TL_REQUIRE(p.lda >= p.K && p.ldb >= p.K && p.lda % 8 == 0 && p.ldb % 8 == 0, "wino63v_nt: bad leading dimensions (multiples of 8)");
  TL_REQUIRE(p.A_rows % 2 == 0, "wino63v_nt: V holds hex pairs");
  TL_REQUIRE(p.Tp > 0 && p.Tp % 6 == 0 && p.M % p.Tp == 0, "wino63v_nt: Tp must be a positive multiple of 6, M whole sequences");
  TL_REQUIRE(8LL * p.N * p.ldb * 4 < (1LL << 31), "wino63v_nt: tap set larger than a buffer resource");
  TL_REQUIRE(128LL * 8 * p.lda * 4 + 4LL * p.K < (1LL << 31), "wino63v_nt: tile span too large");
  const long long ntm = (p.M + V6_ROWS - 1) / V6_ROWS;
  const long long nwg = ntm * ((p.N + V6_BN - 1) / V6_BN);
  TL_REQUIRE(nwg < (1LL << 31), "wino63v_nt: grid too large");
  TL_REQUIRE(p.N % 32 == 0 && p.M + V6_ROWS < (1LL << 31), "wino63v_nt: N %% 32 == 0 and M < 2^31 - 768 needed");
  TL_REQUIRE(p.slope >= 0.f && p.slope <= 1.f, "wino63v_nt: LeakyReLU slope must lie in [0, 1]");
  TL_REQUIRE(p.A_rows >= ntm * V6_BH, "wino63v_nt: V must hold whole 128-hex tiles (pad it with zero hexes)");
  hipStream_t st = (hipStream_t)stream;
  const long long ngrid = nwg < 256 ? nwg : 256;
  if (p.epilogue == W_EPI_POOL) {
    TL_REQUIRE(p.row_shift == 0 && p.out && p.ldo >= p.N, "wino63v_nt: forward needs row_shift 0 and an output");
    TL_REQUIRE(p.obits != nullptr && p.Tvalid % 2 == 0 && p.Tvalid <= p.Tp, "wino63v_nt: POOL needs obits and an even Tvalid");
    TL_REQUIRE(p.ld_obits * 32 >= p.N, "wino63v_nt: POOL: ld_obits too small");
    TL_REQUIRE(p.out_tp >= 0 && (p.out_tp == 0 || 2 * p.out_tp >= p.Tvalid), "wino63v_nt: out_tp must cover the valid pooled rows");
    const long long orows = (p.M / p.Tp) * (long long)(p.out_tp > 0 ? p.out_tp : p.Tp / 2);
    TL_REQUIRE(orows * (long long)p.ldo * 4 < (1LL << 40), "wino63v_nt: output too large");
    hipLaunchKernelGGL((wino63v_nt_kernel<W_EPI_POOL>), dim3((unsigned)ngrid), dim3(512), 0, st, p);
  } else if (p.epilogue == W_EPI_POOLV) {
    TL_REQUIRE(p.row_shift == 0 && (p.out == nullptr || p.ldo >= p.N), "wino63v_nt: forward needs row_shift 0");
    TL_REQUIRE(p.obits != nullptr && p.Tvalid % 2 == 0 && p.Tvalid <= p.Tp, "wino63v_nt: POOLV needs obits and an even Tvalid");
    TL_REQUIRE(p.ld_obits * 32 >= p.N && p.Tp % 12 == 0, "wino63v_nt: POOLV needs Tp %% 12 == 0 (output hexes inside one sequence)");
    TL_REQUIRE(p.vout && p.vhalo && p.ld_vout >= p.N && p.ld_vout % 8 == 0 && p.vout_quads >= p.M / 12 && p.vout_quads % 2 == 0,
               "wino63v_nt: POOLV needs vout (>= M / 12 hexes, whole pairs, ld_vout %% 8 == 0) and vhalo");
    TL_REQUIRE(64LL * 8 * p.ld_vout * 4 < (1LL << 31), "wino63v_nt: ld_vout too large");
    hipLaunchKernelGGL((wino63v_nt_kernel<W_EPI_POOLV>), dim3((unsigned)ngrid), dim3(512), 0, st, p);
  } else if (p.epilogue == W_EPI_MASK) {
    TL_REQUIRE(p.row_shift == -2 && p.ldo >= p.N, "wino63v_nt: input gradient needs row_shift -2");
    TL_REQUIRE(p.auxbits != nullptr, "wino63v_nt: MASK needs auxbits (the sign bits of the stage input)");
    hipLaunchKernelGGL((wino63v_nt_kernel<W_EPI_MASK>), dim3((unsigned)ngrid), dim3(512), 0, st, p);
  } else if (p.epilogue == W_EPI_MASKY) {
    TL_REQUIRE(p.row_shift == -2 && p.auxbits != nullptr && p.abits != nullptr, "wino63v_nt: epilogue 6 needs row_shift -2, auxbits and abits");
    TL_REQUIRE(p.ld_abits * 32 >= p.N && p.Tvalid_in % 2 == 0 && p.Tvalid_in <= 2 * p.Tp, "wino63v_nt: epilogue 6: bad abits / Tvalid_in");
    TL_REQUIRE(p.vout && p.vout2 && p.vhalo && p.ld_vout >= p.N && p.ld_vout % 8 == 0 && p.vout_quads >= p.M / 3 && p.vout_quads % 2 == 0,
               "wino63v_nt: epilogue 6 needs vout / vout2 (>= M / 3 hexes, whole pairs, ld_vout %% 8 == 0) and vhalo");
    TL_REQUIRE(128LL * 8 * p.ld_vout * 4 < (1LL << 31), "wino63v_nt: ld_vout too large");
    hipLaunchKernelGGL((wino63v_nt_kernel<W_EPI_MASKY>), dim3((unsigned)ngrid), dim3(512), 0, st, p);
  } else if (p.epilogue == W_EPI_C1W) {
    TL_REQUIRE(p.row_shift == -2, "wino63v_nt: input gradient needs row_shift -2");
    TL_REQUIRE(p.auxbits && p.c1x && p.c1bits && p.c1partial, "wino63v_nt: epilogue 4 needs auxbits, c1x, c1bits, c1partial");
    TL_REQUIRE(p.c1kt >= 1 && p.c1kt <= 3 && p.c1T >= 2 * p.Tvalid + 2, "wino63v_nt: epilogue 4: 1..3 taps, c1T >= 2*Tvalid + 2");
    hipLaunchKernelGGL((wino63v_nt_kernel<W_EPI_C1W>), dim3((unsigned)ngrid), dim3(512), 0, st, p);
  } else {
    set_error("wino63v_nt: unsupported epilogue %d", p.epilogue);
    return TL_EINVAL;
  }
  return check_launch("wino63v_nt");
}

extern "C" int tl_wino63_unpool_rows6(const float* G, const uint32_t* bits, float* A, int64_t rows, int64_t g_rows, int Tp, int g_tp,
                                      int Tvalid, int C, int ldg, int ld_bits, int lda, int pad, void* stream) {
  using namespace tl;
  TL_REQUIRE(G && bits && A, "wino63_unpool_rows6: null pointer");
  TL_REQUIRE(rows > 0 && Tp > 0 && rows % Tp == 0 && Tvalid > 0 && Tvalid <= Tp, "wino63_unpool_rows6: whole sequences of Tp rows, 0 < Tvalid <= Tp needed");
  TL_REQUIRE(g_tp > 0 && 2 * g_tp >= Tvalid && g_rows >= (rows / Tp) * (long long)g_tp, "wino63_unpool_rows6: G holds fewer rows than sequences x g_tp");
  TL_REQUIRE(C > 0 && C % 8 == 0 && ldg >= C && ldg % 4 == 0 && lda >= C && lda % 8 == 0 && ld_bits * 32 >= C,
             "wino63_unpool_rows6: C %% 8, ldg %% 4, lda %% 8 needed, bits row must cover C");
  const long long nhex = (rows + 5) / 6;
  const long long n = (nhex + 1) / 2 * (C >> 1);
  TL_REQUIRE((n + 255) / 256 < (1LL << 31), "wino63_unpool_rows6: grid too large");
  hipLaunchKernelGGL(wino63_unpool_rows6_kernel, dim3((unsigned)((n + 255) / 256)), dim3(256), 0, (hipStream_t)stream, G, bits, A,
                     nhex, (long long)rows, (long long)g_rows, Tp, g_tp, Tvalid, C, ldg, ld_bits, lda, pad);
  return check_launch("wino63_unpool_rows6");
}

extern "C" int tl_wino63_weights1(const float* w, float* taps, int O, int I, int ldb, void* stream) {
  using namespace tl;
  TL_REQUIRE(w && taps && O > 0 && I > 0 && ldb >= O && ldb % 8 == 0, "wino63_weights1: w, taps, O, I > 0 and ldb %% 8 == 0, ldb >= O needed");
  const long long n = (long long)ldb * 8 * I;
  TL_REQUIRE((n + 255) / 256 < (1LL << 31), "wino63_weights1: too large");
  hipLaunchKernelGGL(wino63_weights1_kernel, dim3((unsigned)((n + 255) / 256)), dim3(256), 0, (hipStream_t)stream, w, taps, O, I, ldb);
  return check_launch("wino63_weights1");
}

extern "C" int tl_conv1_wino63v_dgrad_nt(const tl_nt_params* pp, void* stream) {
  using namespace tl;
  TL_REQUIRE(pp != nullptr, "conv1_wino63v_dgrad_nt: null params");
  const tl_nt_params& p = *pp;
  TL_REQUIRE(p.A && p.Bw, "conv1_wino63v_dgrad_nt: null A / taps");
  TL_REQUIRE(p.loader == W_LOAD_V && p.epilogue == W_EPI_GY && p.J == 1 && p.row_shift == 0 && p.splitk <= 1,
             "conv1_wino63v_dgrad_nt: loader 2, epilogue 7, one tap, row_shift 0, no split-K");
  TL_REQUIRE(p.M > 0 && p.N > 0 && p.K >= 40 && p.K % 8 == 0, "conv1_wino63v_dgrad_nt: K %% 8, K >= 40 needed");
  TL_REQUIRE(p.Tp > 0 && p.Tp % 3 == 0 && p.M % p.Tp == 0, "conv1_wino63v_dgrad_nt: Tp (rows per sequence) must be a multiple of 3, M whole sequences");
  TL_REQUIRE(p.lda >= p.K && p.ldb >= p.K && p.lda % 8 == 0 && p.ldb % 8 == 0, "conv1_wino63v_dgrad_nt: bad leading dimensions (multiples of 8)");
  TL_REQUIRE(p.A_rows % 2 == 0, "conv1_wino63v_dgrad_nt: A holds hex pairs");
  TL_REQUIRE(8LL * p.N * p.ldb * 4 < (1LL << 31), "conv1_wino63v_dgrad_nt: tap set larger than a buffer resource");
  TL_REQUIRE(128LL * 8 * p.lda * 4 + 4LL * p.K < (1LL << 31), "conv1_wino63v_dgrad_nt: tile span too large");
  const long long ntm = (p.M + V6_ROWS - 1) / V6_ROWS;
  const long long nwg = ntm * ((p.N + V6_BN - 1) / V6_BN);
  TL_REQUIRE(nwg < (1LL << 31), "conv1_wino63v_dgrad_nt: grid too large");
  TL_REQUIRE(p.N % 32 == 0 && p.M + V6_ROWS < (1LL << 31), "conv1_wino63v_dgrad_nt: N %% 32 == 0 and M < 2^31 - 768 needed");
  TL_REQUIRE(p.slope >= 0.f && p.slope <= 1.f, "conv1_wino63v_dgrad_nt: LeakyReLU slope must lie in [0, 1]");
  TL_REQUIRE(p.A_rows >= ntm * V6_BH, "conv1_wino63v_dgrad_nt: A must hold whole 128-hex tiles (pad it with zero hexes)");
  TL_REQUIRE(p.auxbits != nullptr && p.abits != nullptr, "conv1_wino63v_dgrad_nt: needs auxbits (sign) and abits (arg-max) of the stage below");
  TL_REQUIRE(p.out_tp > 0 && p.out_tp <= p.Tp && 2 * p.out_tp >= p.Tvalid_in, "conv1_wino63v_dgrad_nt: out_tp = rows per sequence of the bit arrays (0 < out_tp <= Tp, covering Tvalid_in / 2)");
  TL_REQUIRE(p.ld_abits * 32 >= p.N && p.ld_auxbits * 32 >= p.N && p.Tvalid_in % 2 == 0 && p.Tvalid_in <= 2 * p.Tp, "conv1_wino63v_dgrad_nt: bad abits / auxbits / Tvalid_in");
  TL_REQUIRE(p.vout && p.vout2 && p.vhalo && p.ld_vout >= p.N && p.ld_vout % 8 == 0 && p.vout_quads >= p.M / 3 && p.vout_quads % 2 == 0,
             "conv1_wino63v_dgrad_nt: needs vout / vout2 (>= M / 3 hexes, whole pairs, ld_vout %% 8 == 0) and vhalo");
  TL_REQUIRE(128LL * 8 * p.ld_vout * 4 < (1LL << 31), "conv1_wino63v_dgrad_nt: ld_vout too large");
  const long long ngrid = nwg < 256 ? nwg : 256;
  hipLaunchKernelGGL((wino63v_nt_kernel<W_EPI_GY>), dim3((unsigned)ngrid), dim3(512), 0, (hipStream_t)stream, p);
  return check_launch("conv1_wino63v_dgrad_nt");
}

extern "C" int tl_conv3_wino63v_tn(const tl_tn_params* pp, void* stream) {
  using namespace tl;
  TL_REQUIRE(pp != nullptr, "wino63v_tn: null params");
  tl_tn_params p = *pp;
  if (p.splitk < 1) p.splitk = 1;
  if (p.loader == 3) {
    TL_REQUIRE(p.A && p.B && p.slab, "wino63v_tn: null V/Y/slab");
    TL_REQUIRE(p.J == 3 && p.Tp > 0 && p.Tp % 6 == 0 && p.Krows > 0 && p.Krows % p.Tp == 0, "wino63v_tn: loader 3: bad Tp / Krows");
    TL_REQUIRE(p.Krows + 64 < (1LL << 31), "wino63v_tn: more than 2^31 reduction rows");
    TL_REQUIRE(p.Mdim % 256 == 0 && p.Ndim % 64 == 0 && p.lda % 8 == 0 && p.ldb % 8 == 0 && p.lda >= p.Mdim && p.ldb >= p.Ndim &&
               p.ldc >= p.Ndim, "wino63v_tn: loader 3 needs Mdim %% 256, Ndim %% 64, lda / ldb %% 8");
    TL_REQUIRE(p.A_rows % 2 == 0 && p.B_rows % 2 == 0 && p.vd == nullptr, "wino63v_tn: loader 3: whole hex pairs in V and Y, no Vd");
    TL_REQUIRE(p.splitk <= 65535 && (p.splitk == 1 || p.slab_stride >= 8LL * p.Mdim * p.ldc), "wino63v_tn: bad splitk / slab_stride");
    const long long ks = (p.Krows / 6 + T6_H - 1) / T6_H;
    TL_REQUIRE(p.A_rows >= ks * T6_H && p.B_rows >= ks * T6_H, "wino63v_tn: V and Y must hold whole 6-hex K-steps (pad with zero hexes)");
    const long long per3 = (ks + p.splitk - 1) / p.splitk;
    TL_REQUIRE((per3 + 4) * (long long)T6_H * 8 * p.lda * 4 < (1LL << 31) && (per3 + 4) * (long long)T6_H * 8 * p.ldb * 4 < (1LL << 31),
               "wino63v_tn: a reduction split spans more than 2 GB of V or Y: raise splitk");
    const int ntm3 = p.Mdim / 256;
    hipLaunchKernelGGL(wino63v_tn4y_kernel, dim3((unsigned)(2 * ntm3 * (p.Ndim / T6_BN)), (unsigned)p.splitk, 1), dim3(512), 0,
                       (hipStream_t)stream, p, ntm3);
    return check_launch("wino63v_tn (both operands pre-transformed)");
  }
  TL_REQUIRE(p.A && p.B && p.slab && p.bbits, "wino63v_tn: null V/B/bbits/slab");
  TL_REQUIRE(p.J == 3 && p.loader == 1, "wino63v_tn: 3 taps, UNPOOL loader (1) or pre-transformed Y (3)");
  TL_REQUIRE(p.Tp > 0 && p.Tp % 6 == 0 && p.Tvalid % 2 == 0 && p.Tvalid <= p.Tp, "wino63v_tn: Tp %% 6 == 0 and an even Tvalid <= Tp needed");
  TL_REQUIRE(p.Krows > 0 && p.Krows % p.Tp == 0 && p.Mdim > 0 && p.Ndim > 0, "wino63v_tn: bad sizes (Krows must be whole sequences)");
  TL_REQUIRE(p.Krows + 64 < (1LL << 31), "wino63v_tn: more than 2^31 reduction rows");
  TL_REQUIRE(p.Mdim % 128 == 0 && p.Ndim % 64 == 0 && p.lda % 8 == 0 && p.ldb % 4 == 0 && p.A_rows % 2 == 0,
             "wino63v_tn: Mdim %% 128, Ndim %% 64, lda %% 8, ldb %% 4, whole hex pairs in V needed");
  TL_REQUIRE(p.lda >= p.Mdim && p.ldb >= p.Ndim && p.ldc >= p.Ndim, "wino63v_tn: leading dimension too small");
  TL_REQUIRE(p.ld_bbits * 32 >= p.Ndim && p.ld_bbits % 2 == 0, "wino63v_tn: bbits row too short / odd");
  TL_REQUIRE(p.splitk <= 65535, "wino63v_tn: splitk too large");
  TL_REQUIRE(p.splitk == 1 || p.slab_stride >= 8LL * p.Mdim * p.ldc, "wino63v_tn: slab_stride smaller than 8*Mdim*ldc");
  const int g_tp = p.g_tp > 0 ? p.g_tp : p.Tp / 2;
  TL_REQUIRE(2 * g_tp >= p.Tvalid, "wino63v_tn: g_tp must cover the valid pooled rows");
  TL_REQUIRE(p.B_rows >= (p.Krows / p.Tp) * (long long)g_tp && p.B_rows < (1LL << 30), "wino63v_tn: G holds fewer rows than sequences x g_tp");
  const long long ksteps_all = (p.Krows / 6 + T6_H - 1) / T6_H;
  TL_REQUIRE(p.A_rows >= (ksteps_all + 3) * T6_H, "wino63v_tn: V must hold whole 6-hex K-steps and three more (pad it with zero hexes)");
  const long long per = (ksteps_all + p.splitk - 1) / p.splitk;
  TL_REQUIRE((per + 4) * (long long)T6_H * 8 * p.lda * 4 < (1LL << 31), "wino63v_tn: a reduction split spans more than 2 GB of V: raise splitk");
  TL_REQUIRE((per + 6) * 3LL * T6_H * p.ldb * 4 < (1LL << 31), "wino63v_tn: a reduction split spans more than 2 GB of G: raise splitk");
  TL_REQUIRE(p.vd == nullptr || (p.ld_vd >= p.Ndim && p.ld_vd % 8 == 0), "wino63v_tn: ld_vd must cover Ndim (multiple of 8)");
  TL_REQUIRE(p.vd == nullptr || (per + 4) * (long long)T6_H * 8 * p.ld_vd * 4 < (1LL << 31), "wino63v_tn: a reduction split spans more than 2 GB of Vd: raise splitk");
  const int ntn = p.Ndim / T6_BN;
  hipStream_t st = (hipStream_t)stream;
  TL_REQUIRE(p.bm == 0 || p.bm == 128 || (p.bm == 256 && p.Mdim % 256 == 0 && p.Tp >= 12),
             "wino63v_tn: bm must be 0, 128, or 256 with Mdim %% 256 == 0 and Tp >= 12");
  if (p.bm == 256 || (p.bm == 0 && p.Mdim % 256 == 0 && p.Tp >= 12)) {
    const int ntm = p.Mdim / 256;
    const dim3 grid((unsigned)(2 * ntm * ntn), (unsigned)p.splitk, 1);
    if (p.vd != nullptr) hipLaunchKernelGGL((wino63v_tn4_kernel<true>), grid, dim3(512), 0, st, p, ntm);
    else hipLaunchKernelGGL((wino63v_tn4_kernel<false>), grid, dim3(512), 0, st, p, ntm);
    return check_launch("wino63v_tn (4 transforms per workgroup)");
  }
  const int ntm = p.Mdim / 128;
  const dim3 grid((unsigned)(ntm * ntn), (unsigned)p.splitk, 1);
  if (p.vd != nullptr) hipLaunchKernelGGL((wino63v_tn_kernel<true>), grid, dim3(512), 0, st, p, ntm);
  else hipLaunchKernelGGL((wino63v_tn_kernel<false>), grid, dim3(512), 0, st, p, ntm);
  return check_launch("wino63v_tn");
}

extern "C" int tl_conv1_fwd_v6(const float* x, const float* w, const float* b, float* P, float* V, uint32_t* bits, uint32_t* sign,
                               int64_t S, int T, int ktaps, int C1, int Tp, int Tout, float slope, void* stream) {
  using namespace tl;
  TL_REQUIRE(x && w && b && V && bits, "conv1_fwd_v6: null pointer");
  TL_REQUIRE(S > 0 && S < (1LL << 31) && T > 0, "conv1_fwd_v6: bad sizes");
  TL_REQUIRE(ktaps >= 1 && ktaps <= C1_MAXKT, "conv1_fwd_v6: ktaps must be 1..%d", C1_MAXKT);
  TL_REQUIRE(C1 % 128 == 0 && C1 <= 1024 && (C1 & (C1 - 1)) == 0, "conv1_fwd_v6: C1 must be 128, 256, 512 or 1024");
  TL_REQUIRE(Tp > 0 && Tp % 6 == 0, "conv1_fwd_v6: Tp must be a multiple of 6");
  TL_REQUIRE(Tout >= 0 && Tout <= Tp && 2 * Tout + ktaps - 1 <= T, "conv1_fwd_v6: Tout/Tp/T inconsistent (%d,%d,%d)", Tout, Tp, T);
  TL_REQUIRE((size_t)T * 4 <= 64 * 1024, "conv1_fwd_v6: T too large for the LDS window");
#define TL_C1V_LAUNCH(KT_)                                                                                                   \
  case KT_:                                                                                                                  \
    hipLaunchKernelGGL(conv1_fwd_vh_kernel<KT_>, dim3((unsigned)S), dim3(256), (size_t)T * 4, (hipStream_t)stream, x, w, b, P, V, \
                       bits, sign, (long long)S, T, C1, Tp, Tout, slope);                                                    \
    break;
  switch (ktaps) {
    TL_C1V_LAUNCH(1) TL_C1V_LAUNCH(2) TL_C1V_LAUNCH(3) TL_C1V_LAUNCH(4) TL_C1V_LAUNCH(5) TL_C1V_LAUNCH(6) TL_C1V_LAUNCH(7)
    TL_C1V_LAUNCH(8)
  }
#undef TL_C1V_LAUNCH
  return check_launch("conv1_fwd_v6");
}
```

decode_tonal_langauge_amd/csrc/tonal_wino63_epi.h:

```cpp
#pragma once
#include "tonal_common.h"
#include "tonal_wino43_epi.h"
#include "tonal_wino43v_epi.h"

namespace tl {

constexpr unsigned V6_DROP = 0x80000000u;
constexpr unsigned long long V6_HI = 0xffffffff00000000ull;

template <bool IMM>
__device__ __forceinline__ void v6_store_at(float x, __amdgpu_buffer_rsrc_t rs, unsigned vo, unsigned so, unsigned k) {
  if constexpr (IMM) __builtin_amdgcn_raw_buffer_store_b32(__builtin_bit_cast(unsigned, x), rs, vo + k, so, 0);
  else __builtin_amdgcn_raw_buffer_store_b32(__builtin_bit_cast(unsigned, x), rs, vo, so + k, 0);
}

__device__ __forceinline__ void v6_pair_swap(float& a, float& b) {
  const auto r = __builtin_amdgcn_permlane32_swap(__float_as_uint(a), __float_as_uint(b), false, false);
  a = __uint_as_float(r[0]);
  b = __uint_as_float(r[1]);
}

template <bool IMM>
__device__ __forceinline__ void v6_store_hex_pair(float (&ha)[8], float (&hb)[8], __amdgpu_buffer_rsrc_t rs, unsigned voAP, unsigned voAQ,
                                                  unsigned voBP, unsigned voBQ, unsigned so) {
#pragma unroll
  for (int i = 0; i < 8; ++i) v6_pair_swap(ha[i], hb[i]);
#pragma unroll
  for (int t = 0; t < 8; t += 2) {
    {
      const auto r = __builtin_amdgcn_permlane16_swap(__float_as_uint(ha[t]), __float_as_uint(ha[t + 1]), false, false);
      v6_store_at<IMM>(__uint_as_float(r[0]), rs, voAP, so, (unsigned)(t * 64));
      v6_store_at<IMM>(__uint_as_float(r[1]), rs, voAQ, so, (unsigned)(t * 64));
    }
    {
      const auto r = __builtin_amdgcn_permlane16_swap(__float_as_uint(hb[t]), __float_as_uint(hb[t + 1]), false, false);
      v6_store_at<IMM>(__uint_as_float(r[0]), rs, voBP, so, (unsigned)(t * 64));
      v6_store_at<IMM>(__uint_as_float(r[1]), rs, voBQ, so, (unsigned)(t * 64));
    }
  }
}
__device__ __forceinline__ unsigned v6_pair_offset(int colbase, int lr, int lh) {
  return (unsigned)((colbase >> 3) + ((lr >> 3) & 1)) * 512u + (unsigned)((lr >> 4) & 1) * 64u + (unsigned)lh * 32u + (unsigned)(lr & 7) * 4u;
}

__device__ __forceinline__ void wino63_rows(const f32x16 (&acc)[8], int e, float (&y)[6]) {
  const float m1 = acc[1][e], m2 = acc[2][e], m3 = acc[3][e], m4 = acc[4][e], m5 = acc[5][e], m6 = acc[6][e];
  const float a12 = m1 + m2, s12 = m1 - m2, a34 = m3 + m4, s34 = m3 - m4, a56 = m5 + m6, s56 = m5 - m6;
  y[0] = ((acc[0][e] + a12) + a34) + a56;
  y[1] = fmaf(0.5f, s56, fmaf(2.f, s34, s12));
  y[2] = fmaf(0.25f, a56, fmaf(4.f, a34, a12));
  y[3] = fmaf(0.125f, s56, fmaf(8.f, s34, s12));
  y[4] = fmaf(0.0625f, a56, fmaf(16.f, a34, a12));
  y[5] = fmaf(0.03125f, s56, fmaf(32.f, s34, s12)) + acc[7][e];
}
__device__ __forceinline__ void wino63_bt(const float (&d)[8], float (&v)[8]) {
  v[0] = fmaf(5.25f, d[2] - d[4], d[6] - d[0]);
  const float e1 = fmaf(-4.25f, d[4], d[2] + d[6]), o1 = fmaf(-4.25f, d[3], d[1] + d[5]);
  v[1] = e1 + o1;
  v[2] = e1 - o1;
  const float e2 = fmaf(0.25f, d[2], fmaf(-1.25f, d[4], d[6])), o2 = fmaf(0.5f, d[1], fmaf(-2.5f, d[3], 2.f * d[5]));
  v[3] = e2 + o2;
  v[4] = e2 - o2;
  const float e3 = fmaf(4.f, d[2], fmaf(-5.f, d[4], d[6])), o3 = fmaf(2.f, d[1], fmaf(-2.5f, d[3], 0.5f * d[5]));
  v[5] = e3 + o3;
  v[6] = e3 - o3;
  v[7] = fmaf(5.25f, d[3] - d[5], d[7] - d[1]);
}

__device__ __forceinline__ float selbit(uint32_t w, int j, float a, float b) {
  const uint32_t m = (uint32_t)__builtin_amdgcn_sbfe((int)w, j, 1);
  return __uint_as_float((__float_as_uint(a) & m) | (__float_as_uint(b) & ~m));
}

struct v6_rows {
  int tA, tB;
  long long seqA, seqB;
};
__device__ __forceinline__ v6_rows v6_rows_of(long long Hw, int Tp) {
  v6_rows r;
  const unsigned R = (unsigned)(6 * Hw);
  const unsigned s = R / (unsigned)Tp;
  r.seqA = (long long)(unsigned)__builtin_amdgcn_readfirstlane((int)s);
  r.tA = __builtin_amdgcn_readfirstlane((int)(R - s * (unsigned)Tp));
  r.tB = r.tA + 96;
  r.seqB = r.seqA;
  while (r.tB >= Tp) {
    r.tB -= Tp;
    ++r.seqB;
  }
  return r;
}
struct bits96 {
  unsigned long long lo;
  uint32_t hi;
};
__device__ __forceinline__ unsigned long long mask96(const bits96& a, const bits96& b, int j) {
  return j < 64 ? mask2l(a.lo, b.lo, j) : mask2(a.hi, b.hi, j - 64);
}
__device__ __forceinline__ bits96 v6_in_bits96(long long R0h, long long M) {
  bits96 r;
  r.lo = v5_in_bits<64, 1>(R0h, M);
  r.hi = (uint32_t)v5_in_bits<32, 1>(R0h + 64, M);
  return r;
}
__device__ __forceinline__ bits96 v6_valid_bits96(int t0, int Tp, int tlim, long long R0h, long long M) {
  bits96 r;
  r.lo = v5_valid_bits<64, 1>(t0, Tp, tlim, R0h, M);
  int t1 = t0 + 64;
  while (t1 >= Tp) t1 -= Tp;
  r.hi = (uint32_t)v5_valid_bits<32, 1>(t1, Tp, tlim, R0h + 64, M);
  return r;
}

template <bool VOUT, bool FULL>
__device__ __forceinline__ void v6_epilogue_pool(const tl_nt_params& p, const f32x16 (&acc)[8], const v5_pre_pool& pre, float* xch,
                                                 long long R0, int n0, int wm, int wn, int lr_in, int lh, long long tm) {
  int lr = lr_in;
  asm volatile("" : "+v"(lr));
  const int colbase = n0 + wn * 32;
  const bool colok = colbase < p.N;
  const int col = colbase + lr;
  const long long Hw = tm * 128 + wm * 32;
  const int Tp = p.Tp, Tq = Tp >> 1;
  const v6_rows rw = v6_rows_of(Hw, Tp);
  const unsigned long long vA = v5_valid_bits<48, 2>(rw.tA, Tp, p.Tvalid, 6 * Hw, p.M);
  const unsigned long long vB = v5_valid_bits<48, 2>(rw.tB, Tp, p.Tvalid, 6 * Hw + 96, p.M);
  const float bv = pre.bv;
  const long long P0 = 3 * Hw;
  const long long prows = p.M >> 1;
  const int out_tp = (!VOUT && p.out_tp > 0) ? p.out_tp : Tq;
  const int tqa0 = rw.tA >> 1, tqb0 = rw.tB >> 1;
  const unsigned long long kA = v5_valid_bits<48, 1>(tqa0, Tq, out_tp, P0, prows);
  const unsigned long long kB = v5_valid_bits<48, 1>(tqb0, Tq, out_tp, P0 + 48, prows);
  const long long nseq = p.M / Tp;
  const long long obase = rw.seqA * out_tp;
  const __amdgpu_buffer_rsrc_t rsO = rsrc_of(!VOUT ? p.out + obase * (long long)p.ldo : nullptr,
                                            !VOUT ? (nseq * out_tp - obase) * (long long)p.ldo * 4 : 0);
  const unsigned ldo4 = (unsigned)p.ldo * 4u;
  const unsigned col4 = colok ? (unsigned)col * 4u : V6_DROP;
  int ta = tqa0, tb = tqb0;
  unsigned ra = (unsigned)tqa0 * ldo4, rb = ((unsigned)(rw.seqB - rw.seqA) * (unsigned)out_tp + (unsigned)tqb0) * ldo4;
  const unsigned seq_step = (unsigned)(out_tp - Tq) * ldo4;
  float pv[48];
  uint32_t wb0 = 0, wb1 = 0, ws0 = 0, ws1 = 0;
  static_for<0, 16>([&](auto E) {
    constexpr int e = decltype(E)::value;
    float y[6];
    wino63_rows(acc, e, y);
    unsigned vo_e = 0;
    if constexpr (!VOUT) vo_e = selmu(V6_HI, rb, ra) + col4;
    static_for<0, 3>([&](auto H) {
      constexpr int h = decltype(H)::value, j = 3 * e + h;
      const float y0 = lrelu01(y[2 * h] + bv, p.slope), y1 = lrelu01(y[2 * h + 1] + bv, p.slope);
      const bool valid = __builtin_amdgcn_inverse_ballot_w64(mask2l(vA, vB, j));
      const bool gt = (y1 > y0) && valid;
      const float o = valid ? (gt ? y1 : y0) : 0.f;
      pv[j] = o;
      if constexpr (j < 32) {
        wb0 = wb0 + wb0 + (uint32_t)gt;
        ws0 = ws0 + ws0 + (uint32_t)(o > 0.f);
      } else {
        wb1 = wb1 + wb1 + (uint32_t)gt;
        ws1 = ws1 + ws1 + (uint32_t)(o > 0.f);
      }
      if constexpr (!VOUT) {
        const unsigned vo = selmu(mask2l(kA, kB, j), vo_e, V5_OOB);
        __builtin_amdgcn_raw_buffer_store_b32(__builtin_bit_cast(unsigned, o), rsO, vo, (unsigned)h * ldo4, 0);
      }
    });
    if constexpr (!VOUT) {
      ta += 3;
      ra += 3u * ldo4;
      const bool wa = ta >= Tq;
      ta -= wa ? Tq : 0;
      ra += wa ? seq_step : 0u;
      tb += 3;
      rb += 3u * ldo4;
      const bool wbb = tb >= Tq;
      tb -= wbb ? Tq : 0;
      rb += wbb ? seq_step : 0u;
    }
  });
  {
    wb0 = bit_transpose32(__builtin_bitreverse32(wb0), lr);
    ws0 = bit_transpose32(__builtin_bitreverse32(ws0), lr);
    wb1 = bit_transpose32(__builtin_bitreverse32(wb1) >> 16, lr);
    ws1 = bit_transpose32(__builtin_bitreverse32(ws1) >> 16, lr);
    const long long wleft = (nseq * out_tp - obase) * (long long)p.ld_obits * 4;
    const long long wbase = obase * (long long)p.ld_obits + (colbase >> 5);
    const __amdgpu_buffer_rsrc_t rsB = rsrc_of(p.obits + wbase, wleft - (long long)(colbase >> 5) * 4);
    const __amdgpu_buffer_rsrc_t rsS = rsrc_of(p.osign ? p.osign + wbase : nullptr, p.osign ? wleft - (long long)(colbase >> 5) * 4 : 0);
    const unsigned t0h = (unsigned)(lh ? tqb0 : tqa0);
    const unsigned s0h = lh ? (unsigned)(rw.seqB - rw.seqA) : 0u;
#pragma unroll
    for (int b = 0; b < 2; ++b) {
      const unsigned r = 32u * b + (unsigned)lr;
      unsigned t = t0h + r;
      const unsigned c = t / (unsigned)Tq;
      t -= c * (unsigned)Tq;
      const bool keep = colok && r < 48u && t < (unsigned)out_tp && (P0 + 48 * lh + r) < prows;
      const unsigned wo = keep ? ((s0h + c) * (unsigned)out_tp + t) * (unsigned)p.ld_obits * 4u : V5_OOB;
      __builtin_amdgcn_raw_buffer_store_b32(b ? wb1 : wb0, rsB, wo, 0u, 0);
      __builtin_amdgcn_raw_buffer_store_b32(b ? ws1 : ws0, rsS, wo, 0u, 0);
    }
  }
  if constexpr (VOUT) {
    if (p.out != nullptr) {
      const __amdgpu_buffer_rsrc_t rsP = rsrc_of(p.out + P0 * (long long)p.ldo, (prows - P0) * (long long)p.ldo * 4);
      const unsigned pvoff = colok ? ((unsigned)(48 * lh) * (unsigned)p.ldo + (unsigned)col) * 4u : V5_OOB;
#pragma unroll
      for (int j = 0; j < 48; ++j) {
        const unsigned vo = selmu(mask2l(kA, kB, j), pvoff, V5_OOB);
        __builtin_amdgcn_raw_buffer_store_b32(__builtin_bit_cast(unsigned, pv[j]), rsP, vo, (unsigned)j * (unsigned)p.ldo * 4u, 0);
      }
    }
    const int slot = wm * 2 + lh;
    {
      float2 v2 = {pv[0], pv[1]};
      *reinterpret_cast<float2*>(xch + (slot * 64 + wn * 32 + lr) * 2) = v2;
    }
    __builtin_amdgcn_s_waitcnt(0xc07f);
    __builtin_amdgcn_s_barrier();
    asm volatile("" ::: "memory");
    float nb0 = 0.f, nb1 = 0.f;
    if (slot < 7) {
      const float2 v2 = *reinterpret_cast<const float2*>(xch + ((slot + 1) * 64 + wn * 32 + lr) * 2);
      nb0 = v2.x;
      nb1 = v2.y;
    }
    uint32_t seA = 0, seB = 0, nvA = 0, nvB = 0;
    {
      int t_a = tqa0, t_b = tqb0;
      const long long qa = (Hw >> 1), qb = (Hw >> 1) + 8;
      for (int k = 0; k < 8; ++k) {
        seA |= (uint32_t)(t_a == Tq - 6) << k;
        seB |= (uint32_t)(t_b == Tq - 6) << k;
        nvA |= (uint32_t)(FULL || qa + k < p.vout_quads) << k;
        nvB |= (uint32_t)(FULL || qb + k < p.vout_quads) << k;
        t_a += 6;
        if (t_a >= Tq) t_a -= Tq;
        t_b += 6;
        if (t_b >= Tq) t_b -= Tq;
      }
    }
    const long long Hn = Hw >> 1;
    const __amdgpu_buffer_rsrc_t rsV = rsrc_of(p.vout + Hn * 8 * (long long)p.ld_vout,
                                              (p.vout_quads - Hn) * 8 * (long long)p.ld_vout * 4);
    const unsigned pair4 = (unsigned)p.ld_vout * 64u;
    const unsigned offP = v6_pair_offset(colbase, lr, lh);
    const unsigned vvA = colok ? offP : V6_DROP, vvB = colok ? 4u * pair4 + offP : V6_DROP;
    const unsigned long long mraw = wm == 3 ? V6_HI : 0ull;
#pragma unroll
    for (int qp = 0; qp < 4; ++qp) {
      float vv[2][8];
#pragma unroll
      for (int hq = 0; hq < 2; ++hq) {
        const int q = 2 * qp + hq;
        const unsigned long long mend = mask2(seA, seB, q);
        float d[8];
#pragma unroll
        for (int k = 0; k < 6; ++k) d[k] = pv[6 * q + k];
        d[6] = selm(mend, 0.f, q < 7 ? pv[(6 * q + 6) % 48] : nb0);
        d[7] = selm(mend, 0.f, q < 7 ? pv[(6 * q + 7) % 48] : nb1);
        wino63_bt(d, vv[hq]);
        if (q == 7) {
#pragma unroll
          for (int k = 0; k < 6; ++k) vv[hq][k] = selm(mraw, d[k], vv[hq][k]);
        }
      }
      const int q = 2 * qp;
      const unsigned voA = selmu(mask2(nvA, nvA >> 1, q), vvA, V6_DROP), voB = selmu(mask2(nvB, nvB >> 1, q), vvB, V6_DROP);
      v6_store_hex_pair<FULL>(vv[0], vv[1], rsV, voA, voA + 1024u, voB, voB + 1024u, (unsigned)qp * pair4);
    }
    {
      const bool hw = wm == 0 && p.vhalo != nullptr;
      const __amdgpu_buffer_rsrc_t rsH = rsrc_of(hw ? p.vhalo + tm * 2 * (long long)p.N : nullptr, hw ? 2LL * p.N * 4 : 0);
      const unsigned ho = (colok && lh == 0) ? (unsigned)col * 4u : V5_OOB;
      __builtin_amdgcn_raw_buffer_store_b32(__builtin_bit_cast(unsigned, pv[0]), rsH, ho, 0u, 0);
      __builtin_amdgcn_raw_buffer_store_b32(__builtin_bit_cast(unsigned, pv[1]), rsH, ho, (unsigned)p.N * 4u, 0);
    }
  }
}

template <int EPI>
constexpr int v6_stores() {
  return EPI == W_EPI_POOL ? 52 : EPI == W_EPI_POOLV ? 70 : (EPI == W_EPI_MASK || EPI == W_EPI_LRELU) ? 96 : (EPI == W_EPI_MASKY || EPI == W_EPI_GY) ? 63 : 0;
}

struct v6_pre_mask {
  uint32_t s[3];
};
__device__ __forceinline__ v6_pre_mask v6_prefetch_mask(const tl_nt_params& p, long long R0, int n0, int wm, int wn, int lr, int lh) {
  const int colbase = n0 + wn * 32;
  const long long ra = R0 + wm * 192 + 96 * lh + lr;
  v6_pre_mask r = {{0u, 0u, 0u}};
#pragma unroll
  for (int k = 0; k < 3; ++k)
    if (colbase < p.N && ra + 32 * k < p.M) r.s[k] = p.auxbits[(ra + 32 * k) * (long long)p.ld_auxbits + (colbase >> 5)];
  return r;
}
template <bool FULL>
__device__ __forceinline__ void v6_epilogue_mask(const tl_nt_params& p, const f32x16 (&acc)[8], const v6_pre_mask& pre, long long R0,
                                                 int n0, int wm, int wn, int lr_in, int lh) {
  int lr = lr_in;
  asm volatile("" : "+v"(lr));
  const int colbase = n0 + wn * 32;
  const bool colok = colbase < p.N;
  const int col = colbase + lr;
  const long long Rw = R0 + wm * 192;
  const __amdgpu_buffer_rsrc_t rsO = rsrc_of(p.out + Rw * (long long)p.ldo, (p.M - Rw) * (long long)p.ldo * 4);
  const unsigned ovoff = colok ? ((unsigned)(96 * lh) * (unsigned)p.ldo + (unsigned)col) * 4u : V5_OOB;
  const unsigned ldo4 = (unsigned)p.ldo * 4u;
  bits96 inA = {~0ull, ~0u}, inB = inA;
  if (!FULL) {
    inA = v6_in_bits96(Rw, p.M);
    inB = v6_in_bits96(Rw + 96, p.M);
  }
  uint32_t sT[3];
#pragma unroll
  for (int k = 0; k < 3; ++k) sT[k] = bit_transpose32(pre.s[k], lr);
#pragma unroll
  for (int e = 0; e < 16; ++e) {
    float y[6];
    wino63_rows(acc, e, y);
#pragma unroll
    for (int h = 0; h < 6; ++h) {
      const int r = 6 * e + h;
      const float o = y[h] * selbit(sT[r >> 5], r & 31, 1.f, p.slope);
      const unsigned vo = FULL ? ovoff : selmu(mask96(inA, inB, r), ovoff, V5_OOB);
      __builtin_amdgcn_raw_buffer_store_b32(__builtin_bit_cast(unsigned, o), rsO, vo, (unsigned)r * ldo4, 0);
    }
  }
}

template <bool FULL>
__device__ __forceinline__ void v6_epilogue_lrelu(const tl_nt_params& p, const f32x16 (&acc)[8], const v5_pre_pool& pre, long long R0,
                                                  int n0, int wm, int wn, int lr_in, int lh) {
  int lr = lr_in;
  asm volatile("" : "+v"(lr));
  const int colbase = n0 + wn * 32;
  const bool colok = colbase < p.N;
  const int col = colbase + lr;
  const long long Rw = R0 + wm * 192;
  const __amdgpu_buffer_rsrc_t rsO = rsrc_of(p.out + Rw * (long long)p.ldo, (p.M - Rw) * (long long)p.ldo * 4);
  const unsigned ovoff = colok ? ((unsigned)(96 * lh) * (unsigned)p.ldo + (unsigned)col) * 4u : V5_OOB;
  const unsigned ldo4 = (unsigned)p.ldo * 4u;
  bits96 inA = {~0ull, ~0u}, inB = inA;
  if (!FULL) {
    inA = v6_in_bits96(Rw, p.M);
    inB = v6_in_bits96(Rw + 96, p.M);
  }
  const float bv = pre.bv;
#pragma unroll
  for (int e = 0; e < 16; ++e) {
    float y[6];
    wino63_rows(acc, e, y);
#pragma unroll
    for (int h = 0; h < 6; ++h) {
      const int r = 6 * e + h;
      const float o = lrelu01(y[h] + bv, p.slope);
      const unsigned vo = FULL ? ovoff : selmu(mask96(inA, inB, r), ovoff, V5_OOB);
      __builtin_amdgcn_raw_buffer_store_b32(__builtin_bit_cast(unsigned, o), rsO, vo, (unsigned)r * ldo4, 0);
    }
  }
}

struct v6_pre_masky {
  uint32_t s[3], a[3];
};
template <bool GTP = false>
__device__ __forceinline__ v6_pre_masky v6_prefetch_masky(const tl_nt_params& p, long long R0, int n0, int wm, int wn, int lr, int lh) {
  const int colbase = n0 + wn * 32;
  const long long ra = R0 + wm * 192 + 96 * lh + lr;
  v6_pre_masky r;
#pragma unroll
  for (int k = 0; k < 3; ++k) {
    r.s[k] = r.a[k] = 0u;
    if (colbase < p.N && ra + 32 * k < p.M) {
      long long row = ra + 32 * k;
      bool have = true;
      if constexpr (GTP) {
        const unsigned R = (unsigned)row, sq = R / (unsigned)p.Tp, t = R - sq * (unsigned)p.Tp;
        have = t < (unsigned)p.out_tp;
        row = (long long)sq * p.out_tp + t;
      }
      if (have) {
        r.s[k] = p.auxbits[row * (long long)p.ld_auxbits + (colbase >> 5)];
        r.a[k] = p.abits[row * (long long)p.ld_abits + (colbase >> 5)];
      }
    }
  }
  return r;
}
template <bool FULL, bool DIRECT = false>
__device__ __forceinline__ void v6_epilogue_masky(const tl_nt_params& p, const f32x16 (&acc)[8], const v6_pre_masky& pre, float* xch,
                                                  long long R0, int n0, int wm, int wn, int lr_in, int lh, long long tm) {
  int lr = lr_in;
  asm volatile("" : "+v"(lr));
  const int colbase = n0 + wn * 32;
  const bool colok = colbase < p.N;
  const int col = colbase + lr;
  const long long Rw = R0 + wm * 192;
  const int Tp = p.Tp, hps = Tp / 3;
  const v6_rows rw = v6_rows_of(tm * 128 + wm * 32, Tp);
  uint32_t we[3], wo[3], sT[3], firstw = 0;
  {
    const bits96 okA = v6_valid_bits96(rw.tA, Tp, p.Tvalid_in >> 1, Rw, p.M);
    const bits96 okB = v6_valid_bits96(rw.tB, Tp, p.Tvalid_in >> 1, Rw + 96, p.M);
    const uint32_t okw[3] = {lh ? (uint32_t)okB.lo : (uint32_t)okA.lo, lh ? (uint32_t)(okB.lo >> 32) : (uint32_t)(okA.lo >> 32),
                             lh ? okB.hi : okA.hi};
    uint32_t fA = 0, fB = 0;
    int ha = rw.tA / 3, hb = rw.tB / 3;
    for (int k = 0; k < 32; ++k) {
      fA |= (uint32_t)(ha == 0) << k;
      fB |= (uint32_t)(hb == 0) << k;
      ha = ha + 1 == hps ? 0 : ha + 1;
      hb = hb + 1 == hps ? 0 : hb + 1;
    }
    firstw = lh ? fB : fA;
#pragma unroll
    for (int k = 0; k < 3; ++k) {
      sT[k] = bit_transpose32(pre.s[k], lr);
      const uint32_t aT = bit_transpose32(pre.a[k], lr);
      we[k] = okw[k] & ~aT;
      wo[k] = okw[k] & aT;
    }
  }
  const long long Hb = Rw / 3;
  const unsigned pair4 = (unsigned)p.ld_vout * 64u;
  const __amdgpu_buffer_rsrc_t rsY = rsrc_of(p.vout + Hb * 8 * (long long)p.ld_vout, (p.vout_quads - Hb) * 8 * (long long)p.ld_vout * 4);
  const __amdgpu_buffer_rsrc_t rsD = rsrc_of(p.vout2 + Hb * 8 * (long long)p.ld_vout, (p.vout_quads - Hb) * 8 * (long long)p.ld_vout * 4);
  const unsigned offP = v6_pair_offset(colbase, lr, lh);
  const unsigned vvA = colok ? offP : V6_DROP, vvB = colok ? 16u * pair4 + offP : V6_DROP;
  const int nexA = (int)(p.M / 3 - Hb < 64 ? p.M / 3 - Hb : 64) - lh, nexB = nexA - 32;
  float pe = 0.f, po = 0.f;
  float first_d[6], v1keep[8];
#pragma unroll
  for (int k = 0; k < 6; ++k) first_d[k] = 0.f;
#pragma unroll
  for (int k = 0; k < 8; ++k) v1keep[k] = 0.f;
  auto andf = [](float x, uint32_t m) { return __uint_as_float(__float_as_uint(x) & m); };
#pragma unroll
  for (int e = 0; e < 16; ++e) {
    float y[6];
    if constexpr (DIRECT) {
#pragma unroll
      for (int h = 0; h < 6; ++h) y[h] = acc[h][e];
    } else {
      wino63_rows(acc, e, y);
    }
    float dzr[12];
#pragma unroll
    for (int h = 0; h < 6; ++h) {
      const int r = 6 * e + h;
      const float t = y[h] * selbit(sT[r >> 5], r & 31, 1.f, p.slope);
      dzr[2 * h] = andf(t, (uint32_t)__builtin_amdgcn_sbfe((int)we[r >> 5], r & 31, 1));
      dzr[2 * h + 1] = andf(t, (uint32_t)__builtin_amdgcn_sbfe((int)wo[r >> 5], r & 31, 1));
    }
    float Yp[2][8], Vp[2][8];
#pragma unroll
    for (int hh = 0; hh < 2; ++hh) {
      const int j = 2 * e + hh;
      const float* d6 = dzr + 6 * hh;
      const float ev1 = (d6[0] + d6[2]) + d6[4], od1 = (d6[1] + d6[3]) + d6[5];
      const float ev2 = fmaf(16.f, d6[4], fmaf(4.f, d6[2], d6[0])), od2 = fmaf(32.f, d6[5], fmaf(8.f, d6[3], 2.f * d6[1]));
      const float ev3 = fmaf(0.0625f, d6[4], fmaf(0.25f, d6[2], d6[0])), od3 = fmaf(0.03125f, d6[5], fmaf(0.125f, d6[3], 0.5f * d6[1]));
      Yp[hh][0] = d6[0];
      Yp[hh][1] = ev1 + od1;
      Yp[hh][2] = ev1 - od1;
      Yp[hh][3] = ev2 + od2;
      Yp[hh][4] = ev2 - od2;
      Yp[hh][5] = ev3 + od3;
      Yp[hh][6] = ev3 - od3;
      Yp[hh][7] = d6[5];
      if (j == 0) {
#pragma unroll
        for (int k = 0; k < 6; ++k) first_d[k] = d6[k];
      } else {
        const uint32_t keep = ~(uint32_t)__builtin_amdgcn_sbfe((int)firstw, j, 1);
        float d[8];
        d[0] = andf(pe, keep);
        d[1] = andf(po, keep);
#pragma unroll
        for (int k = 0; k < 6; ++k) d[2 + k] = d6[k];
        wino63_bt(d, Vp[hh]);
      }
      pe = d6[4];
      po = d6[5];
    }
    {
      const int j = 2 * e;
      const unsigned so = (unsigned)e * pair4;
      const unsigned voA = FULL ? vvA : (j < nexA ? vvA : V6_DROP), voB = FULL ? vvB : (j < nexB ? vvB : V6_DROP);
      v6_store_hex_pair<FULL>(Yp[0], Yp[1], rsY, voA, voA + 1024u, voB, voB + 1024u, so);
      if (e == 0) {
#pragma unroll
        for (int i = 0; i < 8; ++i) v1keep[i] = Vp[1][i];
      } else {
        v6_store_hex_pair<FULL>(Vp[0], Vp[1], rsD, voA, voA + 1024u, voB, voB + 1024u, so);
      }
    }
    __builtin_amdgcn_sched_barrier(0);
  }
  const int slot = wm * 2 + lh;
  {
    float2 v2 = {pe, po};
    *reinterpret_cast<float2*>(xch + (slot * 64 + wn * 32 + lr) * 2) = v2;
  }
  __builtin_amdgcn_s_waitcnt(0xc07f);
  __builtin_amdgcn_s_barrier();
  asm volatile("" ::: "memory");
  {
    float fe = 0.f, fo = 0.f;
    if (slot > 0) {
      const float2 v2 = *reinterpret_cast<const float2*>(xch + ((slot - 1) * 64 + wn * 32 + lr) * 2);
      fe = v2.x;
      fo = v2.y;
    }
    const uint32_t keep = ~(uint32_t)__builtin_amdgcn_sbfe((int)firstw, 0, 1);
    float d[8], v[8];
    d[0] = andf(fe, keep);
    d[1] = andf(fo, keep);
#pragma unroll
    for (int k = 0; k < 6; ++k) d[2 + k] = first_d[k];
    wino63_bt(d, v);
    const bool raw = slot == 0;
#pragma unroll
    for (int k = 0; k < 8; ++k) v[k] = raw ? (k < 2 ? 0.f : d[k]) : v[k];
    const unsigned voA = FULL ? vvA : (0 < nexA ? vvA : V6_DROP), voB = FULL ? vvB : (0 < nexB ? vvB : V6_DROP);
    v6_store_hex_pair<FULL>(v, v1keep, rsD, voA, voA + 1024u, voB, voB + 1024u, 0u);
  }
  {
    const bool hw = wm == 3 && p.vhalo != nullptr;
    const __amdgpu_buffer_rsrc_t rsH = rsrc_of(hw ? p.vhalo + tm * 2 * (long long)p.N : nullptr, hw ? 2LL * p.N * 4 : 0);
    const unsigned ho = (colok && lh == 1) ? (unsigned)col * 4u : V5_OOB;
    __builtin_amdgcn_raw_buffer_store_b32(__builtin_bit_cast(unsigned, pe), rsH, ho, 0u, 0);
    __builtin_amdgcn_raw_buffer_store_b32(__builtin_bit_cast(unsigned, po), rsH, ho, (unsigned)p.N * 4u, 0);
  }
}

struct v6_pre_c1w {
  uint32_t s[3], c[3];
  f32x4 x[2];
};
__device__ __forceinline__ v6_pre_c1w v6_prefetch_c1w(const tl_nt_params& p, long long R0, int n0, int wm, int wn, int lr, int lh) {
  const int colbase = n0 + wn * 32;
  const long long rh = R0 + wm * 192 + 96 * lh;
  v6_pre_c1w r;
  const int Tp = p.Tp;
  const long long nseq = p.M / Tp;
  const unsigned s0 = (unsigned)(R0 / Tp);
  const __amdgpu_buffer_rsrc_t rsX = rsrc_of(p.c1x + (long long)s0 * p.c1T, (nseq - s0) * (long long)p.c1T * 4);
  typedef unsigned v4u __attribute__((ext_vector_type(4)));
#pragma unroll
  for (int k = 0; k < 3; ++k) {
    r.s[k] = r.c[k] = 0u;
    const long long rk = rh + lr + 32 * k;
    if (colbase < p.N && rk < p.M) {
      r.s[k] = p.auxbits[rk * (long long)p.ld_auxbits + (colbase >> 5)];
      r.c[k] = p.c1bits[rk * (long long)p.ld_auxbits + (colbase >> 5)];
    }
  }
  const unsigned Rx = (unsigned)(rh + 3 * lr), sx = Rx / (unsigned)Tp, tx = Rx - sx * (unsigned)Tp;
  const unsigned xo = ((sx - s0) * (unsigned)p.c1T + 2u * tx) * 4u;
  r.x[0] = __builtin_bit_cast(f32x4, (v4u)__builtin_amdgcn_raw_buffer_load_b128(rsX, xo, 0u, 0));
  r.x[1] = __builtin_bit_cast(f32x4, (v4u)__builtin_amdgcn_raw_buffer_load_b128(rsX, xo + 16u, 0u, 0));
  return r;
}
__device__ __forceinline__ void v6_epilogue_c1w(const tl_nt_params& p, const f32x16 (&acc)[8], const v6_pre_c1w& pre, float* xw,
                                                float* red, long long R0, int n0, int wm, int wn, int lr_in, int lh, long long tm) {
  int lr = lr_in;
  asm volatile("" : "+v"(lr));
  const int colbase = n0 + wn * 32;
  const bool colok = colbase < p.N;
  const int col = colbase + lr;
  const long long Hw = tm * 128 + wm * 32;
  const long long Rw = 6 * Hw;
  const int Tp = p.Tp;
  const v6_rows rw = v6_rows_of(Hw, Tp);
  const bits96 okA = v6_valid_bits96(rw.tA, Tp, p.Tvalid, Rw, p.M);
  const bits96 okB = v6_valid_bits96(rw.tB, Tp, p.Tvalid, Rw + 96, p.M);
  float* xh = xw + lh * 256;
  *reinterpret_cast<f32x4*>(xh + 8 * lr) = pre.x[0];
  *reinterpret_cast<f32x4*>(xh + 8 * lr + 4) = pre.x[1];
  c1w_acc ca;
  ca.clear();
  uint32_t sT[3], cT[3];
#pragma unroll
  for (int k = 0; k < 3; ++k) {
    sT[k] = bit_transpose32(pre.s[k], lr);
    cT[k] = bit_transpose32(pre.c[k], lr);
  }
  asm volatile("" ::: "memory");
#pragma unroll
  for (int e = 0; e < 16; ++e) {
    float y[6];
    wino63_rows(acc, e, y);
#pragma unroll
    for (int h = 0; h < 6; ++h) {
      const int r = 6 * e + h;
      const float2 xa = *reinterpret_cast<const float2*>(xh + 8 * (r / 3) + 2 * (r % 3));
      const float2 xb = *reinterpret_cast<const float2*>(xh + 8 * (r / 3) + 2 * (r % 3) + 2);
      const float dz = selm0(mask96(okA, okB, r), y[h] * selbit(sT[r >> 5], r & 31, 1.f, p.slope));
      const uint32_t am = (uint32_t)__builtin_amdgcn_sbfe((int)cT[r >> 5], r & 31, 1);
      auto pick = [am](float a, float b) { return __uint_as_float((__float_as_uint(a) & am) | (__float_as_uint(b) & ~am)); };
      ca.s[0] = fmaf(dz, pick(xa.y, xa.x), ca.s[0]);
      ca.s[1] = fmaf(dz, pick(xb.x, xa.y), ca.s[1]);
      ca.s[2] = fmaf(dz, pick(xb.y, xb.x), ca.s[2]);
      ca.b += dz;
    }
    __builtin_amdgcn_sched_barrier(0);
  }
  __syncthreads();
  c1w_reduce_store<4, 64>(p, red, ca, wm, wn * 32 + lr, lh, tm, col, colok);
}

}
```

include/tonal_hip.h:

```cpp
#ifndef TONAL_HIP_H
#define TONAL_HIP_H
#include <stdint.h>

#ifdef __cplusplus
extern "C" {
#endif

#define TL_OK 0
#define TL_EINVAL (-1)
#define TL_ELAUNCH (-2)
#define TL_ENODEV (-3)

const char* tl_last_error(void);
int tl_version(void);
int tl_device_count(void);

typedef struct {
  const float* A; const uint32_t* abits; const float* Bw; const float* bias; const float* aux;
  float* out; uint32_t* obits;
  int64_t M;
  int64_t A_rows;
  int N, K;
  int lda, ldb, ldo, ldaux, ld_abits, ld_obits;
  int J;
  int row_shift;
  int Tp, Tvalid, Tvalid_in;
  float slope;
  int loader, epilogue;
  int splitk; int64_t slab_stride;
  int bm;
  uint32_t* osign; const uint32_t* auxbits; int ld_auxbits;
  const float* c1x; const uint32_t* c1bits; float* c1partial; int c1T, c1kt;
  float* vout; float* vhalo; int64_t vout_quads; int ld_vout;
  int out_tp;
  float* vout2;
} tl_nt_params;
int tl_gemm_nt_window(const tl_nt_params* p, void* stream);

typedef struct {
  const float* A; const float* B; const uint32_t* bbits; float* slab;
  int64_t Krows;
  int64_t A_rows, B_rows;
  int Mdim, Ndim;
  int lda, ldb, ldc, ld_bbits;
  int J;
  int Tp, Tvalid;
  int loader;
  int splitk; int64_t slab_stride;
  float* colsum;
  float* vd; int ld_vd;
  int part;
  int bm;
  int g_tp;
} tl_tn_params;
int tl_gemm_tn_window(const tl_tn_params* p, void* stream);

int tl_wino43_weights(const float* w, float* fwd, float* dgr, int O, int I, int ld_f, int ld_d, void* stream);
int tl_wino43_wgrad_finalize(const float* red, float* gw, int O, int I, int ld, void* stream);
int tl_wino43_input_transform(const float* P, float* V, int64_t rows, int Tp, int C, int ldp, int ldv, void* stream);
int tl_conv3_wino43v_nt(const tl_nt_params* p, void* stream);
int tl_wino43_v_fixup(float* V, const float* vhalo, int64_t quads, int64_t tiles, int Tq, int C, int ldv, void* stream);
int tl_wino43_unpool_transform(const float* G, const uint32_t* bits, float* V, int64_t conv_rows, int64_t g_rows, int Tp,
                               int Tvalid, int C, int ldg, int ld_bits, int ldv, void* stream);
int tl_conv3_wino43v_tn(const tl_tn_params* p, void* stream);
int tl_wino63_weights(const float* w, float* fwd, float* dgr, int O, int I, int ld_f, int ld_d, void* stream);
int tl_conv3_wino63v_nt(const tl_nt_params* p, void* stream);
int tl_wino63_nt_tile_rows(void);
int tl_wino63_v_fixup(float* V, const float* vhalo, int64_t hexes, int64_t tiles, int Tq, int C, int ldv, void* stream);
int tl_conv3_wino63v_tn(const tl_tn_params* p, void* stream);
int tl_wino63_wgrad_finalize(const float* red, float* gw, int O, int I, int ld, void* stream);
int tl_wino63_vd_fixup(float* Vd, const float* vhalo, int64_t hexes, int64_t tiles, int hexes_per_seq, int C, int ldv, void* stream);
int tl_wino63_unpool_yvd(const float* G, const uint32_t* bits, float* Y, float* Vd, int64_t conv_rows, int64_t g_rows, int Tp,
                         int g_tp, int Tvalid, int C, int ldg, int ld_bits, int ldv, void* stream);
int tl_conv1_fwd_v6(const float* x, const float* w, const float* b, float* P, float* V, uint32_t* bits, uint32_t* sign,
                    int64_t S, int T, int ktaps, int C1, int Tp, int Tout, float slope, void* stream);
int tl_wino63_xform2(const float* P, float* V0, float* V1, int64_t rows, int Tp, int Tvalid, int C, int ldp, int ldv, void* stream);
int tl_wino63_weights7(const float* w, float* fwd, int O, int I, int taps, void* stream);
int tl_conv7_wino63v_nt(const tl_nt_params* p, void* stream);
int tl_wino63_unpool_rows6(const float* G, const uint32_t* bits, float* A, int64_t rows, int64_t g_rows, int Tp, int g_tp, int Tvalid,
                           int C, int ldg, int ld_bits, int lda, int pad, void* stream);
int tl_wino63_weights1(const float* w, float* taps, int O, int I, int ldb, void* stream);
int tl_conv1_wino63v_dgrad_nt(const tl_nt_params* p, void* stream);
int tl_comm_unique_id(void* id128);
int tl_comm_init(void** comm, int rank, int nranks, const void* id128);
int tl_comm_destroy(void* comm);
int tl_allreduce(void* comm, const float* send, float* recv, int64_t count, int op, void* stream);
int tl_reduce_scatter(void* comm, const float* send, float* recv, int64_t recv_count, void* stream);
int tl_all_gather(void* comm, const float* send, float* recv, int64_t send_count, void* stream);
int tl_sizeof_nt_params(void);
int tl_sizeof_tn_params(void);

int tl_conv1_fwd(const float* x, const float* w, const float* b, float* P, uint32_t* bits, uint32_t* sign,
                 int64_t S, int T, int ktaps, int C1, int Tp, int Tout, float slope, void* stream);
int tl_conv1_fwd_v(const float* x, const float* w, const float* b, float* P, float* V, uint32_t* bits, uint32_t* sign,
                   int64_t S, int T, int ktaps, int C1, int Tp, int Tout, float slope, void* stream);
int tl_conv1_wgrad(const float* x, const float* G, const uint32_t* bits, float* partial,
                   int nblk, int64_t S, int T, int ktaps, int C1, int Tp, int Tout, void* stream);

int tl_dropout_scale(float* x, int64_t n, float p, uint64_t seed, void* stream);
int tl_dropout_scale_at(float* x, int64_t n, float p, uint64_t seed, int64_t index0, void* stream);

int tl_permute_reduce(const float* src, float* dst, const int64_t dims[4], const int64_t strides[4],
                      const int64_t lims[4], int nz, int64_t zs, const float* bias_last, void* stream);
int tl_colsum(const float* G, float* partial, int nblk, int64_t rows, int ncols, int ld,
              int Tp, int Tvalid, void* stream);

int tl_lstm_cell_fwd(const float* hh, const float* x_t, const float* w_ih, const float* b_ih,
                     const float* b_hh, const float* c_prev, float* act, float* c, float* h,
                     int U, int H, int in_dim, int ld_hh, void* stream);
int tl_lstm_gw(const float* g, const float* W, float* slab, int U, int64_t N, int K, int64_t ldg, int64_t ldw, int rows_per_block,
               void* stream);
int tl_lstm_infer_seq_fused(const float* xp, int64_t xp_row_stride, const float* wp, float* h_a, float* h_b, float* c,
                            int B, int H, int T, int* last_in_b, void* stream);
int tl_lstm_cell_bwd(const float* dh, const float* dh_rec, const float* dc_next, const float* act,
                     const float* c, const float* c_prev, float* dgates, float* dgates_t, float* dc_prev,
                     int U, int H, int ldt, void* stream);
int tl_lstm_ih_grad(const float* dgates, const float* x, float* dw_ih, float* db, float* db2 ,
                    int L, int U, int H, int in_dim, void* stream);

int tl_concat_pack(const float* O5, const float* h, const int32_t* uid, float* Xc,
                   int B, int C, int Tp, int lat, int Cc, int Lc, int ld5, int ldh, int ldx,
                   float p_drop, uint64_t seed, int64_t drop_row0, void* stream);
int tl_concat_unpack_bwd(const float* dXc, const float* O5, const int32_t* members, const int32_t* offsets,
                         float* G5, float* dh, int B, int U, int C, int Tp, int lat, int Cc, int Lc,
                         int ld5, int ldh, int ldx, float slope, float p_drop, uint64_t seed, int64_t drop_row0,
                         void* stream);

int tl_l1_mcd(const float* out, const float* targets, float* dout, float* stats,
              int B, int D, int ldd, int trunc_targets, float grad_scale, void* stream);

int tl_nadam(float* p, const float* g, float* m, float* v, int64_t n, float coef_grad, float coef_mom,
             float beta1, float beta2, float bias_corr2, float eps, float weight_decay, float grad_scale,
             void* stream);
typedef struct { float* p; const float* g; float* m; float* v; int64_t n; int64_t block0; } tl_nadam_entry;
int tl_nadam_multi(const tl_nadam_entry* entries_dev, int count, int64_t total_blocks, float coef_grad, float coef_mom,
                   float beta1, float beta2, float bias_corr2, float eps, float weight_decay, float grad_scale,
                   void* stream);
int tl_nadam_multi_chunk(void);
int tl_set_step_scalars(float* scalars_dev, uint64_t* seed_dev, float coef_grad, float coef_mom, float bias_corr2,
                        uint64_t seed, void* stream);
int tl_sum_slabs2(const float* srcA, float* dstA, int64_t nA, const float* srcB, float* dstB, int64_t nB, int nz, void* stream);
int tl_stage_step(float* scalars_dev, uint64_t* seed_dev, float coef_grad, float coef_mom, float bias_corr2, uint64_t seed,
                  const void* const* src, void* const* dst, const int64_t* nbytes, int n, void* stream);
int tl_nadam_multi_dev(const tl_nadam_entry* entries_dev, int count, int64_t total_blocks, const float* scalars_dev,
                       float beta1, float beta2, float eps, float weight_decay, float grad_scale, void* stream);
int tl_nadam_lowrank(float* p, float* m, float* v, const float* fa, const float* fb, int kr, int rows, int cols,
                     int ldfa, int ldfb, float coef_grad, float coef_mom, float beta1, float beta2,
                     float bias_corr2, float eps, float weight_decay, float grad_scale, void* stream);
int tl_nadam_lowrank_dh(float* p, float* m, float* v, const float* fa, const float* fb, int kr, int rows, int cols,
                        int ldfa, int ldfb, float coef_grad, float coef_mom, float beta1, float beta2,
                        float bias_corr2, float eps, float weight_decay, float grad_scale, float* dh_slab, int U,
                        int row_tiles, void* stream);

int tl_tone_dynamics(const int64_t* tone, const int64_t* syl, const float* table, float* labels,
                     int32_t* err, int B, int n_tones, int L, void* stream);
int tl_splitk_bias_lrelu(const float* slab, const float* bias, float* out, int nz, int64_t n, int ncols, float slope, void* stream);
int tl_linear_rows(const float* x, const float* w, const float* bias, float* out, int B, int K, int N, int64_t ldx, int act,
                   void* stream);
int tl_labels_from_scores(const float* tone_scores, const float* syl_scores, const float* table, float* labels, int64_t* tone,
                          int64_t* syl, int32_t* pair, int32_t* err, int B, int n_tone_cls, int n_syl_cls, int n_rows, int n_syl,
                          int L, void* stream);

int tl_ce_loss(const float* logits, const int64_t* labels, float* dlogits, float* dbias, int64_t* pred, double* loss_sum,
               int64_t* count, int64_t* confusion, int32_t* err, int B, int N, int ldl, int ldd, float grad_scale, void* stream);
int tl_ce_scores_loss(const float* scores, const int64_t* labels, float* dlogits, float* dbias, int64_t* pred, double* loss_sum,
                      int64_t* count, int64_t* confusion, int32_t* err, int B, int N, int ldl, int ldd, float grad_scale,
                      void* stream);
int tl_head_bwd(const float* dlogits, const float* h, const float* W, float* dh, float* dbias_h, float* dw, int B, int K, int N,
                int ldd, int act, float slope, void* stream);

int tl_lstm_train_seq(const float* xp, int64_t xp_row_stride, int64_t xp_step_stride, const float* wp, float* hs, float* cs,
                      float* act, int B, int H, int T, void* stream);
int tl_lstm_bptt_seq(const float* whT, const float* dh_last, const float* act, const float* cs, float* dc, float* dgates,
                     float* dgates_t, int64_t ldt, int B, int H, int T, void* stream);
int tl_pool3_fwd(const float* Y, float* X, int B, int w1, int Cn, int C, int Tp, int tq, int ldy, int64_t rs_b, int64_t rs_t, float p,
                 uint64_t seed, void* stream);
int tl_pool3_bwd(const float* Y, const float* dX, float* dZ, int B, int w1, int Cn, int C, int Tp, int tq, int ldy, int lddz,
                 int64_t rs_b, int64_t rs_t, float p, uint64_t seed, float slope, void* stream);
int tl_pool3_fwd_shard(const float* Y, float* X, int B, int w1, int Cn, int C, int Tp, int tq, int ldy, int64_t rs_b, int64_t rs_t,
                       float p, uint64_t seed, int b0, int B_global, void* stream);
int tl_pool3_bwd_shard(const float* Y, const float* dX, float* dZ, int B, int w1, int Cn, int C, int Tp, int tq, int ldy, int lddz,
                       int64_t rs_b, int64_t rs_t, float p, uint64_t seed, float slope, int b0, int B_global, void* stream);
int tl_conv1_dgrad(const float* G, const uint32_t* bits, const float* w, float* dx, int64_t S, int T, int ktaps, int C1, int Tp,
                   int Tout, int n_inner, int64_t stride_outer, int64_t stride_t, int64_t stride_inner, void* stream);

int tl_lite_conv_fwd(const float* x, const float* w, const float* bias, float* z, float* part,
                     int B, int Cin, int Cout, int T, int k, int pad, void* stream);
int tl_lite_bn_finalize(const float* part, float* mean, float* rstd, float* run_mean, float* run_var,
                        int nparts, int C, int64_t count , int T, float momentum, float eps, int training,
                        int64_t* tracked , void* stream);
int tl_lite_bn_act_pool_fwd(const float* z, const float* mean, const float* rstd, const float* gamma,
                            const float* beta, float* y, int B, int C, int T, float slope, void* stream);
int tl_lite_bn_act_pool_bwd(const float* dy, const float* z, const float* mean, const float* rstd,
                            const float* gamma, const float* beta, float* dz, float* dgamma, float* dbeta,
                            float* work, int B, int C, int T, float slope, int training, void* stream);
int tl_lite_conv_bwd(const float* dz, const float* x, const float* w, float* dx, float* dwpart, float* dbpart,
                     int B, int Cin, int Cout, int T, int k, int pad, void* stream);
int tl_lite_lstm_fwd(const float* xl, const float* w_ih, const float* w_hh, const float* b_ih, const float* b_hh,
                     float* act, float* cs, float* hs, int B, int L, int H, int in_dim, void* stream);
int tl_lite_lstm_bwd(const float* dh_last, const float* w_hh, const float* act, const float* cs, float* dgates,
                     int B, int L, int H, int ld_dh, void* stream);
int tl_lite_cat(const float* y2, const float* hs, float* feat, int B, int F, int H, int L, int ldf,
                float p_drop, uint64_t seed, void* stream);
int tl_lite_uncat(const float* dfeat, float* dy2, float* dh, int B, int F, int H, int ldf, float p_drop,
                  uint64_t seed, void* stream);
int tl_lite_cat_dev(const float* y2, const float* hs, float* feat, int B, int F, int H, int L, int ldf,
                    float p_drop, const uint64_t* seed_dev, void* stream);
int tl_lite_uncat_dev(const float* dfeat, float* dy2, float* dh, int B, int F, int H, int ldf, float p_drop,
                      const uint64_t* seed_dev, void* stream);

int tl_gauss_envelope(const void* x, int x_is_f64, const double* taps, double* y, int C, int64_t T,
                      int nb, int ntap, int half, int envelope, void* stream);
int tl_gauss_envelope_sym(const void* x, int x_is_f64, const double* taps, double* y, int C, int64_t T, int nb, int half,
                          int envelope, void* stream);
int tl_hilbert_ols(const void* x, int x_is_f64, const double* G, const double* tw, double* y, int C, int64_t T, int nb,
                   int half, int nfft, int envelope, void* stream);
int tl_hilbert_ols_bl(const void* x, int x_is_f64, const double* Gp, const int* k0, const double* tw, double* y, int C,
                      int64_t T, int nb, int half, int nfft, int envelope, void* stream);
// ... 50 lines not shown
```

Measured before the change: 1295 mel-frames/s.

## Run conv2 input gradient on Y2 instead of Vd2, dropping Vd2 production

```diff
diff --git a/decode_tonal_langauge_amd/_conv_stack.py b/decode_tonal_langauge_amd/_conv_stack.py
--- a/decode_tonal_langauge_amd/_conv_stack.py
+++ b/decode_tonal_langauge_amd/_conv_stack.py
@@ -326,25 +326,32 @@
         S = self.S
         rows_in = S * st.tp_in
         if self._vd_ready.get(st.idx) != self.generation:
-            raise RuntimeError("F(6,3) input gradient: the stage's weight-gradient pass (which writes Vd) must run first")
+            raise RuntimeError("F(6,3) input gradient: its operand (Vd from the stage's weight-gradient pass, or Y2 from the "
+                               "input gradient of stage 3) must be written first")
         self._vd_ready[st.idx] = -1
-        Vd = self.Vd[st.idx]
-        wd = self._pack_wino63(w, False)
+        on_y = st.idx == 2 and self.f63_yprod
+        Vd = self.Yt[2] if on_y else self.Vd[st.idx]
+        if on_y:
+            wd = torch.empty(8, st.cin, st.cout, dtype=torch.float32, device=w.device)
+            check(self.lib.tl_wino63_weights_y(ptr(w), ptr(wd), st.cout, st.cin, st.cout, self._stream()), "tl_wino63_weights_y")
+        else:
+            wd = self._pack_wino63(w, False)
         kw = dict(A=ptr(Vd), A_rows=Vd.shape[0], lda=Vd.shape[2], loader=LOAD_V, Bw=ptr(wd), M=rows_in, N=st.cin,
-                  K=st.cout, ldb=st.cout, ldo=st.cin, J=3, row_shift=-2, Tp=st.tp_in, slope=self.slope,
+                  K=st.cout, ldb=st.cout, ldo=st.cin, J=3, row_shift=0 if on_y else -2, Tp=st.tp_in, slope=self.slope,
                   auxbits=ptr(self.sbits[st.idx - 1]), ld_auxbits=self.sbits[st.idx - 1].shape[1])
         if st.idx == 3 and self.f63_yprod:
             below = self.stages[0]
             rows2 = S * below.tp_in
             Y2 = self._v_hex_buffer(self.Yt, 2, rows2, below.cout)
-            Vd2 = self._v_hex_buffer(self.Vd, 2, rows2, below.cout)
+            Vd2 = self._v_hex_buffer(self.Vd, 2, rows2, below.cout) if self.store_p1 else None
             ntm = -(-rows_in // self._nt63_rows())
-            halo = self._halo_buffer("d2", ntm, below.cout)
+            halo = self._halo_buffer("d2", ntm, below.cout) if self.store_p1 else None
             self._nt(tag="conv3_dgrad", fn="tl_conv3_wino63v_nt", epilogue=EPI_MASKY, out=None, vout=ptr(Y2), vout2=ptr(Vd2),
                      vhalo=ptr(halo), vout_quads=Y2.shape[0], ld_vout=Y2.shape[2], abits=ptr(self.bits[2]),
                      ld_abits=below.cout // 32, Tvalid_in=2 * below.tout, **kw)
-            check(self.lib.tl_wino63_vd_fixup(ptr(Vd2), ptr(halo), rows_in // 3, ntm, below.tp_in // 6, below.cout, Vd2.shape[2],
-                                              self._stream()), "tl_wino63_vd_fixup")
+            if Vd2 is not None:
+                check(self.lib.tl_wino63_vd_fixup(ptr(Vd2), ptr(halo), rows_in // 3, ntm, below.tp_in // 6, below.cout,
+                                                  Vd2.shape[2], self._stream()), "tl_wino63_vd_fixup")
             self._y_ready[2] = self.generation
             self._vd_ready[2] = self.generation
             return None
@@ -429,7 +436,8 @@
             else:
                 fams[f"{tn} (conv3 weight gradient, {f6}; also writes Vd)"] = ["conv3_wgrad"]
             if self.f63_yprod:
-                fams[f"wino63v_nt_kernel<MASKY> (conv3 input gradient, {f6}; writes Y and Vd of conv2 instead of the gradient rows)"] = ["conv3_dgrad"]
+                both = "Y and Vd" if self.store_p1 else "Y"
+                fams[f"wino63v_nt_kernel<MASKY> (conv3 input gradient, {f6}; writes {both} of conv2 instead of the gradient rows)"] = ["conv3_dgrad"]
                 fams[f"wino63v_tn4y_kernel (conv2 weight gradient, {f6}: both operands by LDS-DMA, no transform in the kernel)"] = ["conv2_wgrad"]
             else:
                 fams[f"wino63v_nt_kernel<MASK> (conv3 input gradient, {f6})"] = ["conv3_dgrad"]
diff --git a/decode_tonal_langauge_amd/_kernels.py b/decode_tonal_langauge_amd/_kernels.py
--- a/decode_tonal_langauge_amd/_kernels.py
+++ b/decode_tonal_langauge_amd/_kernels.py
@@ -20,13 +20,13 @@
     "wino": ("TONAL_WINO", frozenset({"6", "4", "0"}), "6",
              "conv2 / conv3: 6 Winograd F(6,3) on pre-transformed operands (F(4,3) V form where the stack does not allow it), "
              "4 the F(4,3) V form, 0 direct MFMA kernels (also the fallback for every shape neither form covers)"),
-    "f63_yprod": ("TONAL_F63_YPROD", _B, "1", "F(6,3): the backward operands Y / Vd of stages 2 and 3 come pre-transformed out of the "
-                                              "input-gradient epilogue of the stage above (0: the weight-gradient kernels un-pool and "
-                                              "transform the gradient rows themselves)"),
+    "f63_yprod": ("TONAL_F63_YPROD", _B, "1", "F(6,3): the backward operands of stages 2 and 3 (Y2 for both passes of stage 2; Y3 / Vd3) come "
+                                              "pre-transformed out of the input-gradient epilogue of the stage above (0: the weight-gradient "
+                                              "kernels un-pool and transform the gradient rows themselves and write Vd)"),
     "conv4_dgrad": ("TONAL_CONV4_DGRAD", frozenset({"nt63", "gemm"}), "nt63",
                     "F(6,3): the one-tap stage behind conv3 - nt63: its input gradient on the NT63 kernel, writing Y3 / Vd3 "
                     "(no gradient rows, no tl_wino63_unpool_yvd); gemm: one-tap GEMM + tl_wino63_unpool_yvd"),
-    "store_p1": ("TONAL_STORE_P1", _B, "0", "keep the raw pooled rows of stages 1 / 2 beside V (tests)"),
+    "store_p1": ("TONAL_STORE_P1", _B, "0", "keep the raw pooled rows of stages 1 / 2 beside V, and Vd2 beside Y2 (tests)"),
     "conv7": ("TONAL_CONV7", frozenset({"wino63", "direct"}), "wino63", "the CNN-RNN classifier's 7-tap convolutions"),
     "whh_dh": ("TONAL_WHH_DH", _B, "1", "single process: the W_hh NAdam pass also produces the last BPTT product dh_1 = dgates_2 . W_hh "
                                         "(0: a W_hh stream of its own for it)"),
diff --git a/decode_tonal_langauge_amd/_lib.py b/decode_tonal_langauge_amd/_lib.py
--- a/decode_tonal_langauge_amd/_lib.py
+++ b/decode_tonal_langauge_amd/_lib.py
@@ -78,6 +78,7 @@
     "tl_wino43_unpool_transform": (_I, [_P, _P, _P, _L, _L, _I, _I, _I, _I, _I, _I, _P]),
     "tl_conv3_wino43v_tn": (_I, [C.POINTER(TnParams), _P]),
     "tl_wino63_weights": (_I, [_P, _P, _P, _I, _I, _I, _I, _P]),
+    "tl_wino63_weights_y": (_I, [_P, _P, _I, _I, _I, _P]),
     "tl_conv3_wino63v_nt": (_I, [C.POINTER(NtParams), _P]),
     "tl_wino63_nt_tile_rows": (_I, []),
     "tl_wino63_v_fixup": (_I, [_P, _P, _L, _L, _I, _I, _I, _P]),
diff --git a/decode_tonal_langauge_amd/csrc/tonal_wino63.hip b/decode_tonal_langauge_amd/csrc/tonal_wino63.hip
--- a/decode_tonal_langauge_amd/csrc/tonal_wino63.hip
+++ b/decode_tonal_langauge_amd/csrc/tonal_wino63.hip
@@ -24,7 +24,7 @@
 }
 
 __global__ void wino63_weights_kernel(const float* __restrict__ w, float* __restrict__ fwd, float* __restrict__ dgr, int O,
-                                      int I, int ld_f, int ld_d) {
+                                      int I, int ld_f, int ld_d, int flip) {
   const long long n_f = (long long)O * ld_f, n_d = (long long)I * ld_d;
   const long long idx = (long long)blockIdx.x * blockDim.x + threadIdx.x;
   auto emit = [](float* dst, int R, int r, int k, float g0, float g1, float g2) {
@@ -56,7 +56,8 @@
     float g0 = 0.f, g1 = 0.f, g2 = 0.f;
     if (o < O) {
       const float* s = w + ((long long)o * I + i) * 3;
-      g0 = s[2], g1 = s[1], g2 = s[0];
+      if (flip) g0 = s[2], g1 = s[1], g2 = s[0];
+      else g0 = s[0], g1 = s[1], g2 = s[2];
     }
     emit(dgr, I, i, o, g0, g1, g2);
   }
@@ -186,7 +187,7 @@
 
 template <int EPI>
 __global__ __launch_bounds__(512, 2) void wino63v_nt_kernel(const tl_nt_params p) {
-  __shared__ __attribute__((aligned(1024))) char lds[3 * V6_STAGE + ((EPI == W_EPI_POOLV || EPI == W_EPI_MASKY || EPI == W_EPI_GY) ? 4096 : EPI == W_EPI_C1W ? 16384 : 0)];
+  __shared__ __attribute__((aligned(1024))) char lds[3 * V6_STAGE + ((EPI == W_EPI_POOLV || EPI == W_EPI_MASKY || EPI == W_EPI_GY) ? 4096 : (EPI == W_EPI_C1W || EPI == W6_EPI_C1W_Y) ? 16384 : 0)];
   const int tid = threadIdx.x;
   const int lane = tid & 63;
   const int wave = __builtin_amdgcn_readfirstlane(tid >> 6);
@@ -318,7 +319,7 @@
     const dma_src src_ = src_of(tl_, step);
     asm volatile(V6K_ISSUE : : V6K_INPUTS(src_, dst, 0) : "memory", "scc", "m0");
   };
-  constexpr bool early = EPI == W_EPI_POOLV || EPI == W_EPI_C1W;
+  constexpr bool early = EPI == W_EPI_POOLV || EPI == W_EPI_C1W || EPI == W6_EPI_C1W_Y;
   constexpr int NST = v6_stores<EPI>();
   constexpr int first_n = NST + 6 > 63 ? 63 : NST + 6;
   constexpr int first_wait = (first_n & 15) | (7 << 4) | (0 << 8) | ((first_n >> 4) << 14);
@@ -332,7 +333,7 @@
     auto prefetch = [&] {
       if constexpr (EPI == W_EPI_POOL || EPI == W_EPI_POOLV || EPI == W_EPI_LRELU) return v5_prefetch_pool(p, cur.n0, wn, lr);
       else if constexpr (EPI == W_EPI_MASK) return v6_prefetch_mask(p, cur.R0, cur.n0, wm, wn, lr, lh);
-      else if constexpr (EPI == W_EPI_MASKY) return v6_prefetch_masky(p, cur.R0, cur.n0, wm, wn, lr, lh);
+      else if constexpr (EPI == W_EPI_MASKY || EPI == W6_EPI_MASKY_Y) return v6_prefetch_masky(p, cur.R0, cur.n0, wm, wn, lr, lh);
       else if constexpr (EPI == W_EPI_GY) return v6_prefetch_masky<true>(p, cur.R0, cur.n0, wm, wn, lr, lh);
       else return v6_prefetch_c1w(p, cur.R0, cur.n0, wm, wn, lr, lh);
     };
@@ -392,13 +393,16 @@
       float* xch = reinterpret_cast<float*>(lds + 3 * V6_STAGE);
       if (full) v6_epilogue_masky<true>(p, acc, pre, xch, done.R0, done.n0, wm, wn, lr, lh, done.tm);
       else v6_epilogue_masky<false>(p, acc, pre, xch, done.R0, done.n0, wm, wn, lr, lh, done.tm);
+    } else if constexpr (EPI == W6_EPI_MASKY_Y) {
+      if (full) v6_epilogue_masky<true, false, false>(p, acc, pre, nullptr, done.R0, done.n0, wm, wn, lr, lh, done.tm);
+      else v6_epilogue_masky<false, false, false>(p, acc, pre, nullptr, done.R0, done.n0, wm, wn, lr, lh, done.tm);
     } else if constexpr (EPI == W_EPI_GY) {
       float* xch = reinterpret_cast<float*>(lds + 3 * V6_STAGE);
       if (full) v6_epilogue_masky<true, true>(p, acc, pre, xch, done.R0, done.n0, wm, wn, lr, lh, done.tm);
       else v6_epilogue_masky<false, true>(p, acc, pre, xch, done.R0, done.n0, wm, wn, lr, lh, done.tm);
     } else {
-      v6_epilogue_c1w(p, acc, pre, reinterpret_cast<float*>(lds + 3 * V6_STAGE) + wave * 512, scratch, done.R0, done.n0, wm, wn,
-                      lr, lh, done.tm);
+      v6_epilogue_c1w<EPI == W6_EPI_C1W_Y>(p, acc, pre, reinterpret_cast<float*>(lds + 3 * V6_STAGE) + wave * 512, scratch, done.R0,
+                                           done.n0, wm, wn, lr, lh, done.tm);
     }
     {
       constexpr int n = NST + 6 > 63 ? 63 : NST + 6;
@@ -1497,8 +1501,19 @@
   const long long n = nf > nd ? nf : nd;
   TL_REQUIRE((n + 255) / 256 < (1LL << 31), "wino63_weights: too large");
   hipLaunchKernelGGL(wino63_weights_kernel, dim3((unsigned)((n + 255) / 256)), dim3(256), 0, (hipStream_t)stream, w, fwd, dgr, O,
-                     I, ld_f, ld_d);
+                     I, ld_f, ld_d, 1);
   return check_launch("wino63_weights");
+}
+
+extern "C" int tl_wino63_weights_y(const float* w, float* dgy, int O, int I, int ld_d, void* stream) {
+  using namespace tl;
+  TL_REQUIRE(w != nullptr && dgy != nullptr, "wino63_weights_y: null pointer");
+  TL_REQUIRE(O > 0 && I > 0 && ld_d >= O && ld_d % 8 == 0, "wino63_weights_y: O, I > 0 and ld_d %% 8 == 0, ld_d >= O needed");
+  const long long n = (long long)I * ld_d;
+  TL_REQUIRE((n + 255) / 256 < (1LL << 31), "wino63_weights_y: too large");
+  hipLaunchKernelGGL(wino63_weights_kernel, dim3((unsigned)((n + 255) / 256)), dim3(256), 0, (hipStream_t)stream, w,
+                     (float*)nullptr, dgy, O, I, 0, ld_d, 0);
+  return check_launch("wino63_weights_y");
 }
 
 extern "C" int tl_wino63_wgrad_finalize(const float* red, float* gw, int O, int I, int ld, void* stream) {
@@ -1644,15 +1659,19 @@
   } else if (p.epilogue == W_EPI_MASKY) {
     TL_REQUIRE(p.row_shift == -2 && p.auxbits != nullptr && p.abits != nullptr, "wino63v_nt: epilogue 6 needs row_shift -2, auxbits and abits");
     TL_REQUIRE(p.ld_abits * 32 >= p.N && p.Tvalid_in % 2 == 0 && p.Tvalid_in <= 2 * p.Tp, "wino63v_nt: epilogue 6: bad abits / Tvalid_in");
-    TL_REQUIRE(p.vout && p.vout2 && p.vhalo && p.ld_vout >= p.N && p.ld_vout % 8 == 0 && p.vout_quads >= p.M / 3 && p.vout_quads % 2 == 0,
-               "wino63v_nt: epilogue 6 needs vout / vout2 (>= M / 3 hexes, whole pairs, ld_vout %% 8 == 0) and vhalo");
+    TL_REQUIRE(p.vout && p.ld_vout >= p.N && p.ld_vout % 8 == 0 && p.vout_quads >= p.M / 3 && p.vout_quads % 2 == 0,
+               "wino63v_nt: epilogue 6 needs vout (>= M / 3 hexes, whole pairs, ld_vout %% 8 == 0)");
+    TL_REQUIRE((p.vout2 == nullptr) == (p.vhalo == nullptr), "wino63v_nt: epilogue 6 takes vout2 and vhalo together (Y and Vd) or neither (Y only)");
     TL_REQUIRE(128LL * 8 * p.ld_vout * 4 < (1LL << 31), "wino63v_nt: ld_vout too large");
-    hipLaunchKernelGGL((wino63v_nt_kernel<W_EPI_MASKY>), dim3((unsigned)ngrid), dim3(512), 0, st, p);
+    if (p.vout2 != nullptr) hipLaunchKernelGGL((wino63v_nt_kernel<W_EPI_MASKY>), dim3((unsigned)ngrid), dim3(512), 0, st, p);
+    else hipLaunchKernelGGL((wino63v_nt_kernel<W6_EPI_MASKY_Y>), dim3((unsigned)ngrid), dim3(512), 0, st, p);
   } else if (p.epilogue == W_EPI_C1W) {
-    TL_REQUIRE(p.row_shift == -2, "wino63v_nt: input gradient needs row_shift -2");
+    TL_REQUIRE(p.row_shift == -2 || p.row_shift == 0, "wino63v_nt: epilogue 4 needs row_shift -2 (operand Vd) or 0 (operand Y)");
     TL_REQUIRE(p.auxbits && p.c1x && p.c1bits && p.c1partial, "wino63v_nt: epilogue 4 needs auxbits, c1x, c1bits, c1partial");
     TL_REQUIRE(p.c1kt >= 1 && p.c1kt <= 3 && p.c1T >= 2 * p.Tvalid + 2, "wino63v_nt: epilogue 4: 1..3 taps, c1T >= 2*Tvalid + 2");
-    hipLaunchKernelGGL((wino63v_nt_kernel<W_EPI_C1W>), dim3((unsigned)ngrid), dim3(512), 0, st, p);
+    TL_REQUIRE(p.Tvalid >= 0 && p.Tvalid <= p.Tp, "wino63v_nt: epilogue 4: Tvalid must lie in [0, Tp]");
+    if (p.row_shift == -2) hipLaunchKernelGGL((wino63v_nt_kernel<W_EPI_C1W>), dim3((unsigned)ngrid), dim3(512), 0, st, p);
+    else hipLaunchKernelGGL((wino63v_nt_kernel<W6_EPI_C1W_Y>), dim3((unsigned)ngrid), dim3(512), 0, st, p);
   } else {
     set_error("wino63v_nt: unsupported epilogue %d", p.epilogue);
     return TL_EINVAL;
diff --git a/decode_tonal_langauge_amd/csrc/tonal_wino63_epi.h b/decode_tonal_langauge_amd/csrc/tonal_wino63_epi.h
--- a/decode_tonal_langauge_amd/csrc/tonal_wino63_epi.h
+++ b/decode_tonal_langauge_amd/csrc/tonal_wino63_epi.h
@@ -4,6 +4,8 @@
 #include "tonal_wino43v_epi.h"
 
 namespace tl {
+
+enum { W6_EPI_MASKY_Y = 8, W6_EPI_C1W_Y = 9 };
 
 constexpr unsigned V6_DROP = 0x80000000u;
 constexpr unsigned long long V6_HI = 0xffffffff00000000ull;
@@ -65,6 +67,17 @@
   v[5] = e3 + o3;
   v[6] = e3 - o3;
   v[7] = fmaf(5.25f, d[3] - d[5], d[7] - d[1]);
+}
+__device__ __forceinline__ void wino63_b(const float (&m)[8], float (&d)[8]) {
+  const float a12 = m[1] + m[2], s12 = m[1] - m[2], a34 = m[3] + m[4], s34 = m[3] - m[4], a56 = m[5] + m[6], s56 = m[5] - m[6];
+  d[0] = -m[0];
+  d[1] = fmaf(2.f, s56, fmaf(0.5f, s34, s12)) - m[7];
+  d[2] = fmaf(5.25f, m[0], fmaf(4.f, a56, fmaf(0.25f, a34, a12)));
+  d[3] = fmaf(5.25f, m[7], fmaf(-2.5f, s34 + s56, -4.25f * s12));
+  d[4] = fmaf(-5.25f, m[0], fmaf(-5.f, a56, fmaf(-1.25f, a34, -4.25f * a12)));
+  d[5] = fmaf(-5.25f, m[7], fmaf(0.5f, s56, fmaf(2.f, s34, s12)));
+  d[6] = ((m[0] + a12) + a34) + a56;
+  d[7] = m[7];
 }
 
 __device__ __forceinline__ float selbit(uint32_t w, int j, float a, float b) {
@@ -284,7 +297,8 @@
 
 template <int EPI>
 constexpr int v6_stores() {
-  return EPI == W_EPI_POOL ? 52 : EPI == W_EPI_POOLV ? 70 : (EPI == W_EPI_MASK || EPI == W_EPI_LRELU) ? 96 : (EPI == W_EPI_MASKY || EPI == W_EPI_GY) ? 63 : 0;
+  return EPI == W_EPI_POOL ? 52 : EPI == W_EPI_POOLV ? 70 : (EPI == W_EPI_MASK || EPI == W_EPI_LRELU) ? 96
+         : (EPI == W_EPI_MASKY || EPI == W6_EPI_MASKY_Y || EPI == W_EPI_GY) ? 63 : 0;
 }
 
 struct v6_pre_mask {
@@ -392,7 +406,7 @@
   }
   return r;
 }
-template <bool FULL, bool DIRECT = false>
+template <bool FULL, bool DIRECT = false, bool VD = true>
 __device__ __forceinline__ void v6_epilogue_masky(const tl_nt_params& p, const f32x16 (&acc)[8], const v6_pre_masky& pre, float* xch,
                                                   long long R0, int n0, int wm, int wn, int lr_in, int lh, long long tm) {
   int lr = lr_in;
@@ -404,20 +418,23 @@
   const int Tp = p.Tp, hps = Tp / 3;
   const v6_rows rw = v6_rows_of(tm * 128 + wm * 32, Tp);
   uint32_t we[3], wo[3], sT[3], firstw = 0;
+  (void)hps;
   {
     const bits96 okA = v6_valid_bits96(rw.tA, Tp, p.Tvalid_in >> 1, Rw, p.M);
     const bits96 okB = v6_valid_bits96(rw.tB, Tp, p.Tvalid_in >> 1, Rw + 96, p.M);
     const uint32_t okw[3] = {lh ? (uint32_t)okB.lo : (uint32_t)okA.lo, lh ? (uint32_t)(okB.lo >> 32) : (uint32_t)(okA.lo >> 32),
                              lh ? okB.hi : okA.hi};
-    uint32_t fA = 0, fB = 0;
-    int ha = rw.tA / 3, hb = rw.tB / 3;
-    for (int k = 0; k < 32; ++k) {
-      fA |= (uint32_t)(ha == 0) << k;
-      fB |= (uint32_t)(hb == 0) << k;
-      ha = ha + 1 == hps ? 0 : ha + 1;
-      hb = hb + 1 == hps ? 0 : hb + 1;
-    }
-    firstw = lh ? fB : fA;
+    if constexpr (VD) {
+      uint32_t fA = 0, fB = 0;
+      int ha = rw.tA / 3, hb = rw.tB / 3;
+      for (int k = 0; k < 32; ++k) {
+        fA |= (uint32_t)(ha == 0) << k;
+        fB |= (uint32_t)(hb == 0) << k;
+        ha = ha + 1 == hps ? 0 : ha + 1;
+        hb = hb + 1 == hps ? 0 : hb + 1;
+      }
+      firstw = lh ? fB : fA;
+    }
 #pragma unroll
     for (int k = 0; k < 3; ++k) {
       sT[k] = bit_transpose32(pre.s[k], lr);
@@ -429,7 +446,8 @@
   const long long Hb = Rw / 3;
   const unsigned pair4 = (unsigned)p.ld_vout * 64u;
   const __amdgpu_buffer_rsrc_t rsY = rsrc_of(p.vout + Hb * 8 * (long long)p.ld_vout, (p.vout_quads - Hb) * 8 * (long long)p.ld_vout * 4);
-  const __amdgpu_buffer_rsrc_t rsD = rsrc_of(p.vout2 + Hb * 8 * (long long)p.ld_vout, (p.vout_quads - Hb) * 8 * (long long)p.ld_vout * 4);
+  const __amdgpu_buffer_rsrc_t rsD = rsrc_of(VD ? p.vout2 + Hb * 8 * (long long)p.ld_vout : nullptr,
+                                            VD ? (p.vout_quads - Hb) * 8 * (long long)p.ld_vout * 4 : 0);
   const unsigned offP = v6_pair_offset(colbase, lr, lh);
   const unsigned vvA = colok ? offP : V6_DROP, vvB = colok ? 16u * pair4 + offP : V6_DROP;
   const int nexA = (int)(p.M / 3 - Hb < 64 ? p.M / 3 - Hb : 64) - lh, nexB = nexA - 32;
@@ -473,7 +491,8 @@
       Yp[hh][5] = ev3 + od3;
       Yp[hh][6] = ev3 - od3;
       Yp[hh][7] = d6[5];
-      if (j == 0) {
+      if constexpr (!VD) {
+      } else if (j == 0) {
 #pragma unroll
         for (int k = 0; k < 6; ++k) first_d[k] = d6[k];
       } else {
@@ -493,7 +512,8 @@
       const unsigned so = (unsigned)e * pair4;
       const unsigned voA = FULL ? vvA : (j < nexA ? vvA : V6_DROP), voB = FULL ? vvB : (j < nexB ? vvB : V6_DROP);
       v6_store_hex_pair<FULL>(Yp[0], Yp[1], rsY, voA, voA + 1024u, voB, voB + 1024u, so);
-      if (e == 0) {
+      if constexpr (!VD) {
+      } else if (e == 0) {
 #pragma unroll
         for (int i = 0; i < 8; ++i) v1keep[i] = Vp[1][i];
       } else {
@@ -502,6 +522,7 @@
     }
     __builtin_amdgcn_sched_barrier(0);
   }
+  if constexpr (VD) {
   const int slot = wm * 2 + lh;
   {
     float2 v2 = {pe, po};
@@ -536,6 +557,7 @@
     const unsigned ho = (colok && lh == 1) ? (unsigned)col * 4u : V5_OOB;
     __builtin_amdgcn_raw_buffer_store_b32(__builtin_bit_cast(unsigned, pe), rsH, ho, 0u, 0);
     __builtin_amdgcn_raw_buffer_store_b32(__builtin_bit_cast(unsigned, po), rsH, ho, (unsigned)p.N * 4u, 0);
+  }
   }
 }
 
@@ -567,6 +589,7 @@
   r.x[1] = __builtin_bit_cast(f32x4, (v4u)__builtin_amdgcn_raw_buffer_load_b128(rsX, xo + 16u, 0u, 0));
   return r;
 }
+template <bool YFORM = false>
 __device__ __forceinline__ void v6_epilogue_c1w(const tl_nt_params& p, const f32x16 (&acc)[8], const v6_pre_c1w& pre, float* xw,
                                                 float* red, long long R0, int n0, int wm, int wn, int lr_in, int lh, long long tm) {
   int lr = lr_in;
@@ -583,6 +606,46 @@
   float* xh = xw + lh * 256;
   *reinterpret_cast<f32x4*>(xh + 8 * lr) = pre.x[0];
   *reinterpret_cast<f32x4*>(xh + 8 * lr + 4) = pre.x[1];
+  uint32_t keepw = ~0u;
+  uint32_t okx0 = 0, okx1 = 0, sx0 = 0, sx1 = 0, cx0 = 0, cx1 = 0;
+  f32x4 xx = {0.f, 0.f, 0.f, 0.f};
+  float2 xy = {0.f, 0.f};
+  if constexpr (YFORM) {
+    const int hps = Tp / 6;
+    auto starts = [hps](int t0) {
+      uint32_t w = 0;
+      for (int e = t0 == 0 ? 0 : hps - t0 / 6; e < 17; e += hps) w |= 1u << e;
+      return w;
+    };
+    keepw = ~(lh ? starts(rw.tB) : starts(rw.tA));
+    long long seqC = rw.seqB;
+    int tC = rw.tB + 96;
+    while (tC >= Tp) {
+      tC -= Tp;
+      ++seqC;
+    }
+    const int tx = lh ? tC : rw.tB;
+    const long long sqx = lh ? seqC : rw.seqB;
+    const long long Rx = Rw + 96 + 96 * lh;
+    const bool inx = colok && Rx < p.M && tx != 0;
+    okx0 = (inx && tx < p.Tvalid) ? ~0u : 0u;
+    okx1 = (inx && tx + 1 < p.Tvalid) ? ~0u : 0u;
+    if (okx0) {
+      const long long w0 = Rx * (long long)p.ld_auxbits + (colbase >> 5);
+      sx0 = p.auxbits[w0];
+      sx1 = p.auxbits[w0 + p.ld_auxbits];
+      cx0 = p.c1bits[w0];
+      cx1 = p.c1bits[w0 + p.ld_auxbits];
+      const unsigned s0 = (unsigned)(R0 / Tp);
+      const long long nseq = p.M / Tp;
+      const __amdgpu_buffer_rsrc_t rsX = rsrc_of(p.c1x + (long long)s0 * p.c1T, (nseq - s0) * (long long)p.c1T * 4);
+      typedef unsigned v4u __attribute__((ext_vector_type(4)));
+      typedef unsigned v2u __attribute__((ext_vector_type(2)));
+      const unsigned xo = ((unsigned)(sqx - s0) * (unsigned)p.c1T + 2u * (unsigned)tx) * 4u;
+      xx = __builtin_bit_cast(f32x4, (v4u)__builtin_amdgcn_raw_buffer_load_b128(rsX, xo, 0u, 0));
+      xy = __builtin_bit_cast(float2, (v2u)__builtin_amdgcn_raw_buffer_load_b64(rsX, xo + 16u, 0u, 0));
+    }
+  }
   c1w_acc ca;
   ca.clear();
   uint32_t sT[3], cT[3];
@@ -592,10 +655,36 @@
     cT[k] = bit_transpose32(pre.c[k], lr);
   }
   asm volatile("" ::: "memory");
+  auto andf = [](float x, uint32_t m) { return __uint_as_float(__float_as_uint(x) & m); };
+  auto contract = [&ca](float dz, uint32_t am, float x0, float x1, float x2, float x3) {
+    auto pick = [am](float a, float b) { return __uint_as_float((__float_as_uint(a) & am) | (__float_as_uint(b) & ~am)); };
+    ca.s[0] = fmaf(dz, pick(x1, x0), ca.s[0]);
+    ca.s[1] = fmaf(dz, pick(x2, x1), ca.s[1]);
+    ca.s[2] = fmaf(dz, pick(x3, x2), ca.s[2]);
+    ca.b += dz;
+  };
+  float c6 = 0.f, c7 = 0.f;
 #pragma unroll
   for (int e = 0; e < 16; ++e) {
-    float y[6];
-    wino63_rows(acc, e, y);
+    float y[8];
+    if constexpr (YFORM) {
+      float m[8];
+#pragma unroll
+      for (int i = 0; i < 8; ++i) m[i] = acc[i][e];
+      wino63_b(m, y);
+      if (e > 0) {
+        const float kf = __uint_as_float(0x3f800000u & (uint32_t)__builtin_amdgcn_sbfe((int)keepw, e, 1));
+        y[0] = fmaf(c6, kf, y[0]);
+        y[1] = fmaf(c7, kf, y[1]);
+      }
+      c6 = y[6];
+      c7 = y[7];
+    } else {
+      float y6[6];
+      wino63_rows(acc, e, y6);
+#pragma unroll
+      for (int h = 0; h < 6; ++h) y[h] = y6[h];
+    }
 #pragma unroll
     for (int h = 0; h < 6; ++h) {
       const int r = 6 * e + h;
@@ -603,13 +692,14 @@
       const float2 xb = *reinterpret_cast<const float2*>(xh + 8 * (r / 3) + 2 * (r % 3) + 2);
       const float dz = selm0(mask96(okA, okB, r), y[h] * selbit(sT[r >> 5], r & 31, 1.f, p.slope));
       const uint32_t am = (uint32_t)__builtin_amdgcn_sbfe((int)cT[r >> 5], r & 31, 1);
-      auto pick = [am](float a, float b) { return __uint_as_float((__float_as_uint(a) & am) | (__float_as_uint(b) & ~am)); };
-      ca.s[0] = fmaf(dz, pick(xa.y, xa.x), ca.s[0]);
-      ca.s[1] = fmaf(dz, pick(xb.x, xa.y), ca.s[1]);
-      ca.s[2] = fmaf(dz, pick(xb.y, xb.x), ca.s[2]);
-      ca.b += dz;
+      contract(dz, am, xa.x, xa.y, xb.x, xb.y);
     }
     __builtin_amdgcn_sched_barrier(0);
+  }
+  if constexpr (YFORM) {
+    const float d0 = andf(c6 * selbit(sx0, lr, 1.f, p.slope), okx0), d1 = andf(c7 * selbit(sx1, lr, 1.f, p.slope), okx1);
+    contract(d0, (uint32_t)__builtin_amdgcn_sbfe((int)cx0, lr, 1), xx[0], xx[1], xx[2], xx[3]);
+    contract(d1, (uint32_t)__builtin_amdgcn_sbfe((int)cx1, lr, 1), xx[2], xx[3], xy.x, xy.y);
   }
   __syncthreads();
   c1w_reduce_store<4, 64>(p, red, ca, wm, wn * 32 + lr, lh, tm, col, colok);
diff --git a/include/tonal_hip.h b/include/tonal_hip.h
--- a/include/tonal_hip.h
+++ b/include/tonal_hip.h
@@ -64,6 +64,7 @@
                                int Tvalid, int C, int ldg, int ld_bits, int ldv, void* stream);
 int tl_conv3_wino43v_tn(const tl_tn_params* p, void* stream);
 int tl_wino63_weights(const float* w, float* fwd, float* dgr, int O, int I, int ld_f, int ld_d, void* stream);
+int tl_wino63_weights_y(const float* w, float* dgy, int O, int I, int ld_d, void* stream);
 int tl_conv3_wino63v_nt(const tl_nt_params* p, void* stream);
 int tl_wino63_nt_tile_rows(void);
 int tl_wino63_v_fixup(float* V, const float* vhalo, int64_t hexes, int64_t tiles, int Tq, int C, int ldv, void* stream);
```

New measurement: 1311 mel-frames/s (median of 6 runs). 1.01x the previous value.
